# gisbi-kim/navtech-radar-slam

Measured on AMD Instinct MI355X. Metric: sc_loop_queries_per_sec_vs_10k_scan_db, higher is better.
Workload: dtype f16 filter + f64 exact

## Files before the change

navtech-radar-slam_amd/csrc/sc_api.cpp:

```cpp
#include <cmath>
#include <cstdio>
#include <cstdlib>
#include <cstring>
#include <mutex>
#include <new>
#include <string>
#include <vector>

#include "rsx_common.h"
#include "sc_kernels.h"
#include "sc_plan.h"
#include "sc_kdtree.h"
#include "loopverify.h"
#include "radarsc.h"
#include "voxelgrid.h"

namespace rsx {
std::string &last_error() {
  static thread_local std::string e;
  return e;
}
}

using namespace rsx;
using namespace rsx::sc;

struct rsx_sc {
  rsx_sc_params p;
  std::mutex mu;
  Stream stream;
  int64_t n_global = 0, n_local = 0, cap = 0;
  DevBuf desc, vkey, norm, rkey;
  DevBuf hn, cmask;
  DevBuf sp, sp_aux;
  DevBuf hnr, vk16, vk_n;
  int tree_counter = 0;
  int64_t tree_size = 0;
  bool batch_made = false;
  int64_t batch_size = 0;
  struct KdTreeDev {
    DevBuf nodes, vind;
    float low[KD_DIM], high[KD_DIM];
    int64_t n = 0;
    int32_t n_nodes = 0;
    int depth = 0;
  } tree, tree_batch;
  DevBuf pts_ws, q_desc, topk, knn_ws, small, pair_out, q_elig;
  struct QueryWs {
    DevBuf q_vkey, q_norm, q_rkey, partial;
    DevBuf f_qimg, f_lb, f_cand, f_cnt, f_thr, f_plan;
    DevBuf f_wimg, f_win;
  } ws[2];
  QueryWs *w = &ws[0];
  PairProfiler prof;
  const char *prof_kernel = "sc_pair_kernel";
  struct {
    bool valid = false, filtered = false;
    int32_t nq = 0, k = 0;
    int64_t n_items = 0, n_eligible = 0;
    const int64_t *q_elig = nullptr;
    QueryView qv{};
  } st;
  DevBuf st_partial;
  DevBuf q1_ws, q1_ticket;
  DevBuf helper_ws;
  DevBuf stats;
  PinnedBuf pinned;
  static constexpr int kMaxPieces = 8;
  static constexpr int kInsSlots = 8;
  struct InsSlot {
    PinnedBuf host;
    Event done;
    bool used = false;
  } ins[kInsSlots];
  int ins_next = 0;
  hipEvent_t last_insert = nullptr;
  StreamOrder order;
  Event legacy_ev;
  Stream up_stream, stream_b;
  Event up_ev[kMaxPieces], lane_ev;
};

namespace {

constexpr size_t kStatBytes = (size_t)RESCORE_STAT_COPIES * RESCORE_STAT_WORDS * sizeof(unsigned long long);

int set_device(rsx_sc *h) {
  RSX_HIP(hipSetDevice(h->p.device));
  return RSX_OK;
}

int use_stream(rsx_sc *h, void *stream, hipStream_t *s) {
  *s = stream ? static_cast<hipStream_t>(stream) : h->stream;
  if (!stream) {
    if (!h->legacy_ev) RSX_HIP(h->legacy_ev.create());
    RSX_HIP(hipEventRecord(h->legacy_ev, nullptr));
    RSX_HIP(hipStreamWaitEvent(h->stream, h->legacy_ev, 0));
  }
  if (*s != h->stream && h->last_insert) RSX_HIP(hipStreamWaitEvent(*s, h->last_insert, 0));
  return h->order.enter(*s);
}

int own_stream(rsx_sc *h) {
  RSX_TRY(set_device(h));
  return h->order.enter(h->stream);
}

int insert_cloud(rsx_sc *h, const void *d_pts, int64_t n_pts, int64_t stride, int64_t slot, hipStream_t s) {
  return launch_insert(d_pts, nullptr, n_pts, 1, stride, h->p.lidar_height, h->p.max_radius, slot, h->desc.as<float>(),
                       h->vkey.as<double>(), h->norm.as<double>(), h->rkey.as<float>(), h->hn.p, h->hnr.p,
                       h->cmask.as<uint64_t>(), h->sp.p, h->sp_aux.as<float>(), h->vk16.p, h->vk_n.as<float>(), s, h->p.sum_order);
}

int ensure_capacity(rsx_sc *h, int64_t want_local) {
  if (want_local <= h->cap) return RSX_OK;
  int64_t nc = h->cap ? h->cap : 1024;
  while (nc < want_local) nc *= 2;
  RSX_TRY(h->desc.reserve((size_t)nc * DS * sizeof(float), h->stream, true));
  RSX_TRY(h->vkey.reserve((size_t)nc * NS * sizeof(double), h->stream, true));
  RSX_TRY(h->norm.reserve((size_t)nc * NS * sizeof(double), h->stream, true));
  RSX_TRY(h->rkey.reserve((size_t)nc * NR * sizeof(float), h->stream, true));
  RSX_TRY(h->hn.reserve((size_t)nc * FILTER_DB_BYTES_PER_ENTRY, h->stream, true));
  RSX_TRY(h->cmask.reserve((size_t)nc * sizeof(uint64_t), h->stream, true));
  RSX_TRY(h->sp.reserve((size_t)nc * SPEC_DB_BYTES_PER_ENTRY, h->stream, true));
  RSX_TRY(h->sp_aux.reserve((size_t)nc * sizeof(float), h->stream, true));
  RSX_TRY(h->hnr.reserve((size_t)nc * FILTER_DB_BYTES_PER_ENTRY, h->stream, true));
  RSX_TRY(h->vk16.reserve((size_t)nc * 256, h->stream, true));
  RSX_TRY(h->vk_n.reserve((size_t)nc * 2 * sizeof(float), h->stream, true));
  h->cap = nc;
  return RSX_OK;
}

DbView db_view(const rsx_sc *h) {
  DbView v;
  v.desc = h->desc.as<float>();
  v.vkey = h->vkey.as<double>();
  v.norm = h->norm.as<double>();
  v.rkey = h->rkey.as<float>();
  v.hnT = h->hn.p;
  v.cmask = h->cmask.as<uint64_t>();
  v.spT = h->sp.p;
  v.sp_aux = h->sp_aux.as<float>();
  v.hnR = h->hnr.p;
  v.vk16 = h->vk16.p;
  v.vk_n = h->vk_n.as<float>();
  v.n_local = h->n_local;
  v.idx_base = h->p.shard_rank;
  v.idx_stride = h->p.shard_world;
  v.sum_order = h->p.sum_order;
  return v;
}

int build_db_images(rsx_sc *h, int64_t slot, int64_t count, hipStream_t s) {
  RSX_TRY(launch_db_images(h->desc.as<float>(), h->norm.as<double>(), slot, count, h->hn.p, h->hnr.p, h->cmask.as<uint64_t>(), s));
  RSX_TRY(launch_window_db_keys(h->vkey.as<double>(), slot, count, h->vk16.p, h->vk_n.as<float>(), s));
  RSX_TRY(launch_spec_db_images(h->desc.as<float>(), h->norm.as<double>(), slot, count, h->sp.p, h->sp_aux.as<float>(), s));
  RSX_HIP(hipStreamSynchronize(s));
  return RSX_OK;
}

bool owns(const rsx_sc *h, int64_t g) { return (g % h->p.shard_world) == h->p.shard_rank; }

int64_t local_count_below(const rsx_sc *h, int64_t n_eligible) {
  if (n_eligible < 0 || n_eligible > h->n_global) n_eligible = h->n_global;
  const int64_t w = h->p.shard_world, r = h->p.shard_rank;
  if (n_eligible <= r) return 0;
  int64_t c = (n_eligible - r + w - 1) / w;
  return c < h->n_local ? c : h->n_local;
}

float yaw_from_shift(int shift) {
  const double unit = 360.0 / (double)NS;
  const float deg = (float)(shift * unit);
  return (float)((double)deg * M_PI / 180.0);
}

int ensure_pinned(rsx_sc *h, size_t bytes) {
  if (bytes <= h->pinned.bytes) return RSX_OK;
  size_t nb = 4096;
  while (nb < bytes) nb *= 2;
  return h->pinned.reserve(nb);
}

int prepare_queries(rsx_sc *h, const float *d_q, int32_t nq, hipStream_t s, QueryView *qv) {
  h->st.valid = false;
  RSX_TRY(h->w->q_vkey.reserve((size_t)nq * NS * sizeof(double), s, false));
  RSX_TRY(h->w->q_norm.reserve((size_t)nq * NS * sizeof(double), s, false));
  RSX_TRY(h->w->q_rkey.reserve((size_t)nq * NR * sizeof(float), s, false));
  RSX_TRY(launch_keys(d_q, nq, h->w->q_vkey.as<double>(), h->w->q_norm.as<double>(), h->w->q_rkey.as<float>(), s, h->p.sum_order));
  qv->desc = d_q;
  qv->vkey = h->w->q_vkey.as<double>();
  qv->norm = h->w->q_norm.as<double>();
  qv->nq = nq;
  return RSX_OK;
}

int filter_mode_of(const rsx_sc *h) {
  static const int env = [] {
    const char *e = rsx::exp_env("RSX_SC_FILTER");
    if (!e || !*e) return -1;
    return atoi(e) ? 2 : 1;
  }();
  if (h->p.filter_mode) return h->p.filter_mode;
  return env >= 0 ? env : 0;
}

bool use_filter(const rsx_sc *h, int32_t nq, int64_t n_items) {
  const int m = filter_mode_of(h);
  if (m == 1 || n_items <= 0) return false;
  if (m == 2) return true;
  if (n_items >= 50000) return true;
  return (int64_t)nq * n_items >= (1ll << 17);
}

struct ProfScope {
  PairProfiler *pp;
  hipStream_t s;
  bool armed = false;
  ProfScope(PairProfiler *p, hipStream_t st) : pp(p), s(st) {
    if (pp && pp->on && pp->ev && pp->used < PairProfiler::kMax) armed = hipEventRecord(pp->ev[2 * pp->used], s) == hipSuccess;
  }
  void stop() {
    if (armed && hipEventRecord(pp->ev[2 * pp->used + 1], s) == hipSuccess) pp->used++;
    armed = false;
  }
};

constexpr int kDefaultFilterKind = 2;
int filter_kind_of(const rsx_sc *h) {
  static const int env = [] {
    const char *e = rsx::exp_env("RSX_SC_FILTER_KIND");
    if (!e || !*e) return -1;
    if (e[0] == '2' || (e[0] == 's' && std::strstr(e, "2"))) return 2;
    return (e[0] == 's' || e[0] == '1') ? 1 : 0;
  }();
  if (h->p.filter_kind) return h->p.filter_kind - 1;
  return env >= 0 ? env : kDefaultFilterKind;
}

size_t any_qimg_bytes(int32_t nq) {
  const size_t a = filter_qimg_bytes(nq), b = spec_qimg_bytes(nq);
  return a > b ? a : b;
}

int run_filter(rsx_sc *h, const QueryView &q, int64_t n_items, lb_t *lb, int64_t ld, const FilterPlanInput *plan,
               hipStream_t s, int64_t first = 0) {
  DbView db = db_view(h);
  if (first) {
    db.hnT = static_cast<const char *>(db.hnT) + first * FILTER_DB_BYTES_PER_ENTRY;
    db.spT = static_cast<const char *>(db.spT) + first * SPEC_DB_BYTES_PER_ENTRY;
    db.cmask += first;
    db.sp_aux += first;
  }
  if (plan) RSX_TRY(h->w->f_plan.reserve(filter_plan_bytes(n_items), s, false));
  if (filter_kind_of(h) >= 1) {
    const bool two_waves = filter_kind_of(h) == 2;
    h->prof_kernel = two_waves ? spec2_filter_kernel_name() : spec_filter_kernel_name();
    RSX_TRY(launch_spec_query_images(q.desc, q.norm, q.nq, h->w->f_qimg.p, s));
    const int32_t *qmin = nullptr;
    const int64_t *cum = nullptr;
    if (plan) RSX_TRY(launch_filter_plan(db, *plan, q.nq, n_items, 4, h->w->f_plan.p, &qmin, &cum, s));
    ProfScope ps(&h->prof, s);
    RSX_TRY(launch_spec_filter(db, h->w->f_qimg.p, q.nq, n_items, lb, ld, qmin, cum, s, two_waves));
    ps.stop();
    return RSX_OK;
  }
  h->prof_kernel = filter_kernel_name();
  RSX_TRY(launch_query_images(q.desc, q.norm, q.nq, h->w->f_qimg.p, s));
  ProfScope ps(&h->prof, s);
  RSX_TRY(launch_filter(db, h->w->f_qimg.p, q.nq, n_items, lb, ld, plan, plan ? h->w->f_plan.p : nullptr, s));
  ps.stop();
  return RSX_OK;
}

int64_t filter_batch(int64_t n_items, int64_t nq) { return plan::filter_batch(n_items, nq); }

int filter_reserve(rsx_sc *h, int64_t n_items, int64_t qb, hipStream_t s) {
  h->st.valid = false;
  const int64_t ld = (n_items + 31) / 32 * 32;
  RSX_TRY(h->w->f_qimg.reserve(any_qimg_bytes((int32_t)qb), s, false));
  RSX_TRY(h->w->f_lb.reserve((size_t)qb * ld * sizeof(lb_t), s, false));
  RSX_TRY(h->w->f_cand.reserve((size_t)qb * RESCORE_SHORTLIST_CAP * sizeof(RescoreEntry), s, false));
  RSX_TRY(h->w->f_cnt.reserve((size_t)qb * sizeof(int32_t), s, false));
  RSX_TRY(h->w->f_thr.reserve((size_t)qb * RESCORE_THR_STRIDE * sizeof(float), s, false));
  RSX_TRY(h->w->f_wimg.reserve(window_qimg_bytes((int32_t)qb), s, false));
  RSX_TRY(h->w->f_win.reserve((size_t)qb * WINDOW_P * sizeof(WindowPreview), s, false));
  return RSX_OK;
}

int filter_and_select(rsx_sc *h, const QueryView &q, int64_t n_items, int64_t n_eligible, const int64_t *elig,
                      int32_t first_target, int32_t k, hipStream_t s, bool elig_monotone = false) {
  const DbView db = db_view(h);
  const int64_t ld = (n_items + 31) / 32 * 32;
  lb_t *lb = h->w->f_lb.as<lb_t>();
  {
    FilterPlanInput plan{n_eligible, elig};
    const bool planned = elig_monotone && elig != nullptr;
    RSX_TRY(run_filter(h, q, n_items, lb, ld, planned ? &plan : nullptr, s));
  }
  RSX_TRY(launch_select(db, lb, ld, n_items, q.nq, n_eligible, elig, first_target, h->w->f_cand.as<RescoreEntry>(),
                        h->w->f_cnt.as<int32_t>(), h->w->f_thr.as<float>(), s));
  return launch_window(db, q, h->w->f_wimg.p, h->w->f_cand.as<RescoreEntry>(), h->w->f_cnt.as<int32_t>(), k, filter_eps(),
                       h->w->f_win.as<WindowPreview>(), s);
}

int rescore(rsx_sc *h, const QueryView &q, int64_t n_items, int64_t n_eligible, const int64_t *elig, int32_t round_begin,
            int32_t round_end, const rsx_sc_hit *tau_src, const rsx_sc_hit *seed, int32_t k, rsx_sc_hit *d_out,
            hipStream_t s) {
  const int64_t ld = (n_items + 31) / 32 * 32;
  return launch_rescore(db_view(h), q, h->w->f_lb.as<lb_t>(), ld, n_items, n_eligible, elig, h->w->f_cand.as<RescoreEntry>(),
                        h->w->f_cnt.as<int32_t>(), h->w->f_thr.as<float>(), filter_eps(), round_begin, round_end, tau_src,
                        seed, d_out, k, s, (h->prof.on && h->stats.p) ? h->stats.as<unsigned long long>() : nullptr,
                        h->w->f_win.as<WindowPreview>());
}

int32_t first_round_target() {
  static const int32_t v = [] {
    const char *e = rsx::exp_env("RSX_SC_FIRST_TARGET");
    const int x = e ? atoi(e) : 0;
    return (x >= 1 && x <= 128) ? x : 128;
  }();
  return v;
}

int run_topk_filtered(rsx_sc *h, const QueryView &qv, int64_t n_items, int64_t n_eligible, const int64_t *d_q_elig,
                      int32_t k, rsx_sc_hit *d_out, hipStream_t s, bool elig_monotone) {
  const int64_t qb = filter_batch(n_items, qv.nq);
  RSX_TRY(filter_reserve(h, n_items, qb, s));
  for (int64_t b0 = 0; b0 < qv.nq; b0 += qb) {
    const int32_t bn = (int32_t)((qv.nq - b0 < qb) ? (qv.nq - b0) : qb);
    QueryView q = qv;
    q.desc = qv.desc + b0 * DS;
    q.vkey = qv.vkey + b0 * NS;
    q.norm = qv.norm + b0 * NS;
    q.nq = bn;
    const int64_t *elig = d_q_elig ? d_q_elig + b0 : nullptr;
    RSX_TRY(filter_and_select(h, q, n_items, n_eligible, elig, first_round_target(), k, s, elig_monotone));
    RSX_TRY(rescore(h, q, n_items, n_eligible, elig, 0, RESCORE_ALL_ROUNDS, nullptr, nullptr, k, d_out + b0 * k, s));
  }
  return RSX_OK;
}

bool use_q1(const rsx_sc *h, int32_t nq, int64_t n_items) {
  static const bool off = [] {
    const char *e = rsx::exp_env("RSX_SC_Q1");
    return e && e[0] == '0';
  }();
  const int m = filter_mode_of(h);
  if (off || nq < 1 || nq > Q1_MAX_NQ || !(m == 0 || m == 3)) return false;
  return m == 3 || nq == 1 || (int64_t)nq * n_items <= (nq <= 8 ? 800000 : 400000);
}

int run_q1(rsx_sc *h, const float *d_q, int32_t nq, int64_t n_items, int64_t n_eligible, const int64_t *d_q_elig, int32_t k,
           rsx_sc_hit *d_out, hipStream_t s) {
  if (n_items < 0) n_items = 0;
  if (!h->q1_ticket.p) {
    RSX_TRY(h->q1_ticket.reserve(q1_ticket_bytes(), s, false));
    RSX_HIP(hipMemsetAsync(h->q1_ticket.p, 0, q1_ticket_bytes(), s));
  }
  RSX_TRY(h->q1_ws.reserve(q1_workspace_bytes(n_items, nq, k), s, false));
  h->prof_kernel = q1_kernel_name();
  ProfScope ps(&h->prof, s);
  RSX_TRY(launch_q1(db_view(h), d_q, nq, n_items, n_eligible, d_q_elig, k, d_out, h->q1_ws.p, h->q1_ticket.as<unsigned>(),
                    (h->prof.on && h->stats.p) ? h->stats.as<unsigned long long>() : nullptr, s));
  ps.stop();
  return RSX_OK;
}

int run_topk(rsx_sc *h, const QueryView &qv, int64_t n_items, int64_t n_eligible, const int64_t *d_q_elig,
             int32_t k, rsx_sc_hit *d_out, hipStream_t s, bool elig_monotone = false) {
  if (use_q1(h, qv.nq, n_items)) return run_q1(h, qv.desc, qv.nq, n_items, n_eligible, d_q_elig, k, d_out, s);
  if (use_filter(h, qv.nq, n_items)) return run_topk_filtered(h, qv, n_items, n_eligible, d_q_elig, k, d_out, s, elig_monotone);
  h->prof_kernel = pair_kernel_name();
  RSX_TRY(h->w->partial.reserve(pair_partial_bytes(n_items > 0 ? n_items : 1, qv.nq, k), s, false));
  struct Hook {
    explicit Hook(PairProfiler *p) { set_pair_profiler(p); }
    ~Hook() { set_pair_profiler(nullptr); }
  } hook(&h->prof);
  return launch_pairs(db_view(h), qv, nullptr, 0, n_items, n_eligible, d_q_elig, nullptr, nullptr,
                      h->w->partial.as<rsx_sc_hit>(), d_out, k, s);
}

struct PreparedTree {
  int64_t n = 0;
  std::vector<KdNode16> n16;
  std::vector<int32_t> vind;
  float low[KD_DIM], high[KD_DIM];
  int depth = 0;
};

int prepare_tree_host(const float *keys, int64_t n, PreparedTree *out) {
  KdTreeHost host;
  RSX_TRY(kdtree_build_host(keys, n, &host));
  std::vector<KdNode16> &n16 = out->n16;
  n16.resize(host.nodes.size());
  for (size_t i = 0; i < host.nodes.size(); i++) {
    const KdNode &nd = host.nodes[i];
    if (nd.child1 < 0) {
      n16[i] = KdNode16{nd.left, -1 - (nd.right - nd.left), 0.0f, 0.0f};
    } else {
      if (nd.child1 != (int32_t)i + 1) return fail(RSX_ERR_RANGE, "kd-tree nodes are not in preorder");
      n16[i] = KdNode16{nd.child2, nd.divfeat, nd.divlow, nd.divhigh};
    }
  }
  {
    std::vector<int32_t> lo(host.nodes.size());
    for (size_t i = host.nodes.size(); i-- > 0;) {
      const KdNode &nd = host.nodes[i];
      lo[i] = nd.child1 < 0 ? nd.left : lo[(size_t)nd.child1];
      if (nd.child1 >= 0) {
        if (lo[(size_t)nd.child2] >= (1 << 26)) return fail(RSX_ERR_RANGE, "ring-key tree over more than 2^26 keys");
        n16[i].b |= lo[(size_t)nd.child2] << 5;
      }
    }
  }
  out->vind.swap(host.vind);
  std::memcpy(out->low, host.low, sizeof(out->low));
  std::memcpy(out->high, host.high, sizeof(out->high));
  out->depth = host.depth;
  out->n = n;
  return RSX_OK;
}

int upload_tree(rsx_sc *h, rsx_sc::KdTreeDev *t, const PreparedTree &p) {
  hipStream_t s = h->stream;
  t->n = 0;
  t->n_nodes = (int32_t)p.n16.size();
  RSX_TRY(t->nodes.reserve(p.n16.size() * sizeof(KdNode16), s, false));
  RSX_TRY(t->vind.reserve(p.vind.size() * sizeof(int32_t), s, false));
  RSX_HIP(hipMemcpyAsync(t->nodes.p, p.n16.data(), p.n16.size() * sizeof(KdNode16), hipMemcpyHostToDevice, s));
  RSX_HIP(hipMemcpyAsync(t->vind.p, p.vind.data(), p.vind.size() * sizeof(int32_t), hipMemcpyHostToDevice, s));
  RSX_HIP(hipStreamSynchronize(s));
  std::memcpy(t->low, p.low, sizeof(t->low));
  std::memcpy(t->high, p.high, sizeof(t->high));
  t->depth = p.depth;
  t->n = p.n;
  return RSX_OK;
}

int ensure_tree(rsx_sc *h, rsx_sc::KdTreeDev *t, int64_t n, std::unique_lock<std::mutex> &lk) {
  if (t->n == n) return RSX_OK;
  hipStream_t s = h->stream;
  std::vector<float> keys((size_t)n * NR);
  RSX_HIP(hipMemcpyAsync(keys.data(), h->rkey.p, keys.size() * sizeof(float), hipMemcpyDeviceToHost, s));
  RSX_HIP(hipStreamSynchronize(s));
  PreparedTree p;
  lk.unlock();
  const int st = prepare_tree_host(keys.data(), n, &p);
  const std::string err = st == RSX_OK ? std::string() : last_error();
  lk.lock();
  if (st != RSX_OK) {
    last_error() = err;
    return st;
  }
  RSX_TRY(set_device(h));
  if (t->n == n) return RSX_OK;
  if (n > h->n_local) return fail(RSX_ERR_RANGE, "the database shrank while the ring-key tree was being built");
  return upload_tree(h, t, p);
}

int score_candidates_and_finish(rsx_sc *h, const QueryView &qv, const float *d_qkey, int64_t n_search, rsx_sc::KdTreeDev *tree,
                                int mode, int32_t *loop_id, float *yaw, double *min_dist, int32_t *nn_idx) {
  hipStream_t s = h->stream;
  const int k = h->p.num_candidates;
  double best_d = 10000000;
  int best_align = 0, best_idx = 0;
  if (mode == RSX_SC_MODE_CANDIDATE) {
    RSX_TRY(h->small.reserve(4096, s, false));
    int32_t *d_idx = h->small.as<int32_t>();
    float *d_kd = reinterpret_cast<float *>(d_idx + 64);
    int32_t *d_found = d_idx + 128;
    if (n_search > 0) {
      if (tree->n != n_search) return fail(RSX_ERR_INTERNAL, "ring-key tree over %lld keys was not prepared", (long long)n_search);
      int32_t *b_idx = d_idx + 192;
      float *b_kd = reinterpret_cast<float *>(d_idx + 256);
      int32_t *b_found = d_idx + 320;
      RSX_TRY(h->knn_ws.reserve((size_t)n_search * 2 * sizeof(float), s, false));
      float *dist_all = h->knn_ws.as<float>(), *dist_tree = dist_all + n_search;
      RSX_TRY(launch_knn(h->rkey.as<float>(), n_search, d_qkey, k, dist_all, b_idx, b_kd, b_found, s));
      int32_t *cand_pos = d_idx + 384, *cand_count = d_idx + 384 + 64;
      RSX_TRY(launch_knn_tree_order(dist_all, tree->vind.as<int32_t>(), n_search, dist_tree, k, b_kd, b_found, cand_pos, cand_count, s));
      KdSearchArgs ka;
      ka.bound_dist = b_kd;
      ka.bound_found = b_found;
      ka.dist_tree = dist_tree;
      ka.cand_pos = cand_pos;
      ka.cand_count = cand_count;
      ka.nodes = tree->nodes.as<KdNode16>();
      ka.n_nodes = tree->n_nodes;
      ka.n = n_search;
      ka.vind = tree->vind.as<int32_t>();
      ka.keys = h->rkey.as<float>();
      ka.qkey = d_qkey;
      std::memcpy(ka.low, tree->low, sizeof(ka.low));
      std::memcpy(ka.high, tree->high, sizeof(ka.high));
      ka.k = k;
      ka.out_idx = d_idx;
      ka.out_dist = d_kd;
      ka.out_found = d_found;
      RSX_TRY(launch_knn_tree(ka, s));
    } else {
      RSX_TRY(h->knn_ws.reserve(sizeof(float), s, false));
      RSX_TRY(launch_knn(h->rkey.as<float>(), 0, d_qkey, k, h->knn_ws.as<float>(), d_idx, d_kd, d_found, s));
    }
    double *d_dist = reinterpret_cast<double *>(h->small.as<char>() + 1024);
    int32_t *d_shift = reinterpret_cast<int32_t *>(h->small.as<char>() + 2048);
    RSX_TRY(launch_pairs(db_view(h), qv, d_idx, 0, k, -1, nullptr, d_dist, d_shift, nullptr, nullptr, 0, s));
    RSX_TRY(ensure_pinned(h, 4096));
    char *hp = static_cast<char *>(h->pinned.p);
    RSX_HIP(hipMemcpyAsync(hp, h->small.p, 2048 + 256, hipMemcpyDeviceToHost, s));
    RSX_HIP(hipStreamSynchronize(s));
    const int32_t *ci = reinterpret_cast<const int32_t *>(hp);
    const double *cd = reinterpret_cast<const double *>(hp + 1024);
    const int32_t *cs = reinterpret_cast<const int32_t *>(hp + 2048);
    for (int c = 0; c < k; c++) {
      if (cd[c] < best_d) {
        best_d = cd[c];
        best_align = cs[c];
        best_idx = ci[c];
      }
    }
  } else {
    RSX_TRY(ensure_pinned(h, 4096));
    RSX_TRY(run_topk(h, qv, n_search, n_search, nullptr, 1, static_cast<rsx_sc_hit *>(h->pinned.p), s));
    RSX_HIP(hipStreamSynchronize(s));
    const rsx_sc_hit *r = static_cast<const rsx_sc_hit *>(h->pinned.p);
    if (r->dist < best_d) {
      best_d = r->dist;
      best_align = r->shift;
      best_idx = r->index;
    }
  }
  int lid = -1;
  if (best_d < h->p.dist_thres) lid = best_idx;
  if (loop_id) *loop_id = lid;
  if (yaw) *yaw = yaw_from_shift(best_align);
  if (min_dist) *min_dist = best_d;
  if (nn_idx) *nn_idx = best_idx;
  return RSX_OK;
}

}

extern "C" {

const char *rsx_last_error_string(void) { return rsx::last_error().c_str(); }

const char *rsx_version(void) {
#ifdef RSX_EXPERIMENTS
  return "rsx 0.3 (gfx950, HIP; ScanContext + ORORA hot path) +experiments";
#else
  return "rsx 0.3 (gfx950, HIP; ScanContext + ORORA hot path)";
#endif
}

int rsx_device_count(void) try {
  int n = 0;
  if (hipGetDeviceCount(&n) != hipSuccess) return 0;
  return n;
} RSX_CATCH_ALL

const char *rsx_sc_dominant_kernel_name(void) { return pair_kernel_name(); }

const char *rsx_sc_profiled_kernel_name(rsx_sc *h) {
  if (!h) return "";
  std::lock_guard<std::mutex> lk(h->mu);
  return h->prof_kernel;
}

int rsx_sc_default_params(rsx_sc_params *p) try {
  if (!p) return fail(RSX_ERR_BAD_ARG, "null params");
  p->lidar_height = 2.0;
  p->max_radius = 80.0;
  p->num_exclude_recent = 30;
  p->num_candidates = 3;
  p->search_ratio = 0.1;
  p->dist_thres = 0.2;
  p->tree_making_period = 30;
  p->device = 0;
  p->shard_rank = 0;
  p->shard_world = 1;
  p->capacity_hint = 1024;
  p->filter_mode = 0;
  p->filter_kind = 0;
  p->sum_order = RSX_SC_SUM_EIGEN_SSE2;
  return RSX_OK;
} RSX_CATCH_ALL

int rsx_sc_create(const rsx_sc_params *p, rsx_sc **out) try {
  if (!out) return fail(RSX_ERR_BAD_ARG, "null out");
  *out = nullptr;
  rsx_sc_params d;
  rsx_sc_default_params(&d);
  if (p) d = *p;
  if (d.shard_world < 1 || d.shard_rank < 0 || d.shard_rank >= d.shard_world)
    return fail(RSX_ERR_BAD_ARG, "bad shard %d/%d", d.shard_rank, d.shard_world);
  if (d.num_candidates < 1 || d.num_candidates > RSX_SC_MAX_TOPK)
    return fail(RSX_ERR_BAD_ARG, "num_candidates must be in [1,%d]", RSX_SC_MAX_TOPK);
  if ((int)std::lround(0.5 * d.search_ratio * NS) != 3)
    return fail(RSX_ERR_BAD_ARG, "kernels are specialised for SEARCH_RADIUS 3 (search_ratio 0.1, SC.h:96)");
  if (d.tree_making_period < 1 || d.num_exclude_recent < 0) return fail(RSX_ERR_BAD_ARG, "bad detector params");
  if (d.filter_mode < 0 || d.filter_mode > 3) return fail(RSX_ERR_BAD_ARG, "filter_mode must be 0 (auto), 1 (off), 2 (force) or 3 (single-query path)");
  if (d.sum_order < 0 || d.sum_order > RSX_SC_SUM_EIGEN34_AVX_FMA) return fail(RSX_ERR_BAD_ARG, "sum_order must be RSX_SC_SUM_EIGEN_SSE2, _SEQ, _EIGEN_AVX_FMA or _EIGEN34_AVX_FMA");
  if (d.filter_kind < 0 || d.filter_kind > 3)
    return fail(RSX_ERR_BAD_ARG, "filter_kind must be 0 (auto), 1 (direct), 2 (spectral) or 3 (spectral, two waves per SIMD)");
  RSX_TRY(check_device(d.device));
  std::unique_ptr<rsx_sc> h(new (std::nothrow) rsx_sc());
  if (!h) return fail(RSX_ERR_OOM, "host alloc");
  h->p = d;
  RSX_TRY(set_device(h.get()));
  hipError_t e = h->stream.create();
  if (e != hipSuccess) return fail(RSX_ERR_HIP, "hipStreamCreate: %s", hipGetErrorString(e));
  RSX_TRY(ensure_capacity(h.get(), d.capacity_hint > 0 ? d.capacity_hint : 1024));
  *out = h.release();
  return RSX_OK;
} RSX_CATCH_ALL

int rsx_sc_destroy(rsx_sc *h) try {
  if (!h) return RSX_OK;
  (void)hipSetDevice(h->p.device);
  for (hipStream_t s : {h->stream.s, h->up_stream.s, h->stream_b.s})
    if (s) (void)hipStreamSynchronize(s);
  delete h;
  return RSX_OK;
} RSX_CATCH_ALL

int rsx_sc_set_dist_thres(rsx_sc *h, double thres) try {
  if (!h) return fail(RSX_ERR_BAD_ARG, "null handle");
  std::lock_guard<std::mutex> lk(h->mu);
  h->p.dist_thres = thres;
  return RSX_OK;
} RSX_CATCH_ALL

int rsx_sc_size(rsx_sc *h, int64_t *n) try {
  if (!h || !n) return fail(RSX_ERR_BAD_ARG, "null arg");
  std::lock_guard<std::mutex> lk(h->mu);
  *n = h->n_global;
  return RSX_OK;
} RSX_CATCH_ALL

int rsx_sc_local_size(rsx_sc *h, int64_t *n) try {
  if (!h || !n) return fail(RSX_ERR_BAD_ARG, "null arg");
  std::lock_guard<std::mutex> lk(h->mu);
  *n = h->n_local;
  return RSX_OK;
} RSX_CATCH_ALL

int rsx_sc_ringkey_tree_layout(const float *keys20, int64_t n, int32_t *out_vind, int32_t *out_n_nodes, int32_t *out_depth) try {
  if (!keys20 || !out_vind || n < 1) return fail(RSX_ERR_BAD_ARG, "bad arg");
  KdTreeHost host;
  RSX_TRY(kdtree_build_host(keys20, n, &host));
  std::memcpy(out_vind, host.vind.data(), host.vind.size() * sizeof(int32_t));
  if (out_n_nodes) *out_n_nodes = (int32_t)host.nodes.size();
  if (out_depth) *out_depth = host.depth;
  return RSX_OK;
} RSX_CATCH_ALL

int rsx_sc_tree_size(rsx_sc *h, int64_t *n) try {
  if (!h || !n) return fail(RSX_ERR_BAD_ARG, "null arg");
  std::lock_guard<std::mutex> lk(h->mu);
  *n = h->tree_size;
  return RSX_OK;
} RSX_CATCH_ALL

int rsx_sc_add_points(rsx_sc *h, const void *pts, size_t n, size_t stride_bytes, int32_t *out_index) try {
  if (!h || (!pts && n)) return fail(RSX_ERR_BAD_ARG, "null arg");
  if (stride_bytes < 12 || (stride_bytes & 3)) return fail(RSX_ERR_BAD_ARG, "stride_bytes must be >= 12 and a multiple of 4");
  std::lock_guard<std::mutex> lk(h->mu);
  RSX_TRY(own_stream(h));
  const int64_t g = h->n_global;
  if (owns(h, g)) {
    const int64_t slot = h->n_local;
    RSX_TRY(ensure_capacity(h, slot + 1));
    const size_t bytes = n * stride_bytes;
    rsx_sc::InsSlot &sl = h->ins[h->ins_next];
    h->ins_next = (h->ins_next + 1) % rsx_sc::kInsSlots;
    if (sl.used) RSX_HIP(hipEventSynchronize(sl.done));
    if (bytes > sl.host.bytes) {
      size_t cap = 32768;
      while (cap < bytes) cap *= 2;
      RSX_TRY(sl.host.reserve(cap));
    }
    if (!sl.done) RSX_HIP(sl.done.create());
    if (bytes) std::memcpy(sl.host.p, pts, bytes);
    RSX_TRY(insert_cloud(h, sl.host.p, (int64_t)n, (int64_t)stride_bytes, slot, h->stream));
    RSX_HIP(hipEventRecord(sl.done, h->stream));
    sl.used = true;
    h->last_insert = sl.done;
    h->n_local = slot + 1;
  }
  h->n_global = g + 1;
  if (out_index) *out_index = (int32_t)g;
  return RSX_OK;
} RSX_CATCH_ALL

int rsx_sc_add_points_downsampled(rsx_sc *h, rsx_voxelgrid *vg, const void *pts, size_t n, size_t stride_bytes, float leaf,
                                  int32_t *out_index) try {
  if (!h || !vg || (!pts && n)) return fail(RSX_ERR_BAD_ARG, "null arg");
  if (stride_bytes < 12 || (stride_bytes & 3)) return fail(RSX_ERR_BAD_ARG, "stride_bytes must be >= 12 and a multiple of 4");
  if (!(leaf > 0.0f)) return fail(RSX_ERR_BAD_ARG, "leaf must be positive");
  if (rsx::vg::device_of(vg) != h->p.device) return fail(RSX_ERR_BAD_ARG, "voxel grid and ScanContext handles are on different devices");
  std::lock_guard<std::mutex> lk(h->mu);
  std::lock_guard<std::mutex> lkv(rsx::vg::mutex_of(vg));
  RSX_TRY(own_stream(h));
  const int64_t g = h->n_global;
  if (owns(h, g)) {
    const float *d_ds = nullptr;
    int64_t nds = 0;
    RSX_TRY(rsx::vg::upload_and_filter(vg, pts, (int64_t)n, (int64_t)stride_bytes, -1, leaf, (int64_t)(n ? n : 1), &d_ds, &nds));
    const int64_t slot = h->n_local;
    RSX_TRY(ensure_capacity(h, slot + 1));
    RSX_TRY(insert_cloud(h, d_ds ? static_cast<const void *>(d_ds) : h->desc.p, nds, 16, slot, h->stream));
    RSX_HIP(hipStreamSynchronize(h->stream));
    h->n_local = slot + 1;
  }
  h->n_global = g + 1;
  if (out_index) *out_index = (int32_t)g;
  return RSX_OK;
} RSX_CATCH_ALL

int rsx_sc_add_keyframe(rsx_sc *h, rsx_voxelgrid *vg, rsx_kfstore *kf, const void *pts, size_t n, size_t stride_bytes,
                        int32_t intensity_offset, float leaf, int32_t *out_index) try {
  if (!h || !vg || !kf || (!pts && n)) return fail(RSX_ERR_BAD_ARG, "null arg");
  if (stride_bytes < 12 || (stride_bytes & 3)) return fail(RSX_ERR_BAD_ARG, "stride_bytes must be >= 12 and a multiple of 4");
  if (intensity_offset >= 0 && ((intensity_offset & 3) || (size_t)intensity_offset + 4 > stride_bytes))
    return fail(RSX_ERR_BAD_ARG, "intensity_offset outside the point");
  if (!(leaf > 0.0f)) return fail(RSX_ERR_BAD_ARG, "leaf must be positive");
  if (rsx::vg::device_of(vg) != h->p.device || rsx::kf::device_of(kf) != h->p.device)
    return fail(RSX_ERR_BAD_ARG, "voxel grid, keyframe store and ScanContext handles are on different devices");
  std::lock_guard<std::mutex> lk(h->mu);
  std::lock_guard<std::mutex> lkv(rsx::vg::mutex_of(vg));
  std::lock_guard<std::mutex> lkk(rsx::kf::mutex_of(kf));
  RSX_TRY(own_stream(h));
  const int64_t g = h->n_global;
  const float *d_ds = nullptr;
  int64_t nds = 0;
  RSX_TRY(rsx::vg::upload_and_filter(vg, pts, (int64_t)n, (int64_t)stride_bytes, intensity_offset, leaf, (int64_t)(n ? n : 1), &d_ds, &nds));
  const bool mine = owns(h, g);
  if (mine) {
    const int64_t slot = h->n_local;
    RSX_TRY(ensure_capacity(h, slot + 1));
    RSX_TRY(insert_cloud(h, d_ds ? static_cast<const void *>(d_ds) : h->desc.p, nds, 16, slot, h->stream));
    RSX_HIP(hipStreamSynchronize(h->stream));
  }
  int32_t kf_index = -1;
  RSX_TRY(rsx::kf::append_device_locked(kf, d_ds, nds, &kf_index));
  if (mine) h->n_local = h->n_local + 1;
  h->n_global = g + 1;
  if (out_index) *out_index = (int32_t)g;
  return RSX_OK;
} RSX_CATCH_ALL

static int add_f32_locked(rsx_sc *h, const float *src, int64_t n, bool src_is_device, hipStream_t s) {
  const int64_t g0 = h->n_global;
  const int64_t w = h->p.shard_world, r = h->p.shard_rank;
  int64_t first = g0 + (((r - g0) % w) + w) % w;
  int64_t count = first < g0 + n ? (g0 + n - first + w - 1) / w : 0;
  if (count > 0) {
    const int64_t slot = h->n_local;
    RSX_TRY(ensure_capacity(h, slot + count));
    float *dst = h->desc.as<float>() + slot * DS;
    RSX_HIP(hipMemcpy2DAsync(dst, DS * sizeof(float), src + (first - g0) * DS, (size_t)w * DS * sizeof(float),
                             DS * sizeof(float), (size_t)count,
                             src_is_device ? hipMemcpyDeviceToDevice : hipMemcpyHostToDevice, s));
    RSX_TRY(launch_keys(dst, count, h->vkey.as<double>() + slot * NS, h->norm.as<double>() + slot * NS,
                        h->rkey.as<float>() + slot * NR, s, h->p.sum_order));
    RSX_TRY(build_db_images(h, slot, count, s));
    h->n_local = slot + count;
  }
  h->n_global = g0 + n;
  return RSX_OK;
}

static int add_descriptor_f64(rsx_sc *h, const double *desc, bool allow_rounding, int32_t *out_index, double *max_err) {
  if (!h || !desc) return fail(RSX_ERR_BAD_ARG, "null arg");
  float f[DS];
  double worst = 0.0;
  for (int i = 0; i < DS; i++) {
    f[i] = (float)desc[i];
    if (!((double)f[i] == desc[i])) {
      if (!allow_rounding || !(desc[i] == desc[i]))
        return fail(RSX_ERR_NOT_FP32_EXACT, "descriptor element %d (%.17g) is not exactly representable in fp32", i, desc[i]);
      const double e = std::fabs((double)f[i] - desc[i]);
      if (e > worst) worst = e;
    }
  }
  if (max_err) *max_err = worst;
  std::lock_guard<std::mutex> lk(h->mu);
  RSX_TRY(own_stream(h));
  const int64_t g = h->n_global;
  RSX_TRY(add_f32_locked(h, f, 1, false, h->stream));
  if (out_index) *out_index = (int32_t)g;
  return RSX_OK;
}

int rsx_sc_add_descriptor(rsx_sc *h, const double *desc, int32_t *out_index) try {
  return add_descriptor_f64(h, desc, false, out_index, nullptr);
} RSX_CATCH_ALL

int rsx_sc_add_descriptor_rounded(rsx_sc *h, const double *desc, int32_t *out_index, double *max_abs_rounding) try {
  return add_descriptor_f64(h, desc, true, out_index, max_abs_rounding);
} RSX_CATCH_ALL

int rsx_sc_add_descriptors_f32(rsx_sc *h, const float *descs, int64_t n) try {
  if (!h || (!descs && n) || n < 0) return fail(RSX_ERR_BAD_ARG, "bad arg");
  if (n == 0) return RSX_OK;
  std::lock_guard<std::mutex> lk(h->mu);
  RSX_TRY(own_stream(h));
  return add_f32_locked(h, descs, n, false, h->stream);
} RSX_CATCH_ALL

int rsx_sc_add_descriptors_f32_device(rsx_sc *h, const float *d_descs, int64_t n, void *stream) try {
  if (!h || (!d_descs && n) || n < 0) return fail(RSX_ERR_BAD_ARG, "bad arg");
  if (n == 0) return RSX_OK;
  std::lock_guard<std::mutex> lk(h->mu);
  RSX_TRY(set_device(h));
  hipStream_t s;
  RSX_TRY(use_stream(h, stream, &s));
  return add_f32_locked(h, d_descs, n, true, s);
} RSX_CATCH_ALL

int rsx_sc_add_polar_batch_device(rsx_sc *h, rsx_radarsc *rc, const uint8_t *d_imgs, int32_t n_images, int64_t image_stride_bytes,
                                  int32_t row_stride, int32_t col_offset, const float *d_azimuths, int32_t azimuths_per_image, void *stream) try {
  if (!h || !rc || n_images < 0 || (n_images && (!d_imgs || !d_azimuths))) return fail(RSX_ERR_BAD_ARG, "bad arg");
  if (rsx::rc::device_of(rc) != h->p.device) return fail(RSX_ERR_BAD_ARG, "radar scan-context and ScanContext handles are on different devices");
  if (n_images == 0) return RSX_OK;
  std::lock_guard<std::mutex> lk(h->mu);
  std::lock_guard<std::mutex> lkr(rsx::rc::mutex_of(rc));
  RSX_TRY(set_device(h));
  hipStream_t s;
  RSX_TRY(use_stream(h, stream, &s));
  const float *d_descs = nullptr;
  RSX_TRY(rsx::rc::build_scratch_device(rc, d_imgs, n_images, image_stride_bytes, row_stride, col_offset, d_azimuths, azimuths_per_image, s, &d_descs));
  return add_f32_locked(h, d_descs, n_images, true, s);
} RSX_CATCH_ALL

int rsx_sc_add_polar(rsx_sc *h, rsx_radarsc *rc, const uint8_t *img, int32_t row_stride, int32_t col_offset, const float *azimuths,
                     int32_t *out_index) try {
  if (!h || !rc || !img || !azimuths) return fail(RSX_ERR_BAD_ARG, "null arg");
  if (rsx::rc::device_of(rc) != h->p.device) return fail(RSX_ERR_BAD_ARG, "radar scan-context and ScanContext handles are on different devices");
  std::lock_guard<std::mutex> lk(h->mu);
  std::lock_guard<std::mutex> lkr(rsx::rc::mutex_of(rc));
  RSX_TRY(own_stream(h));
  const int64_t g = h->n_global;
  if (owns(h, g)) {
    const float *d_desc = nullptr;
    RSX_TRY(rsx::rc::upload_and_build(rc, img, row_stride, col_offset, azimuths, h->stream, &d_desc));
    RSX_TRY(add_f32_locked(h, d_desc, 1, true, h->stream));
  } else {
    h->n_global = g + 1;
  }
  if (out_index) *out_index = (int32_t)g;
  return RSX_OK;
} RSX_CATCH_ALL

int rsx_sc_export_descriptors_f32(rsx_sc *h, int64_t first_slot, int64_t count, float *out) try {
  if (!h || (!out && count)) return fail(RSX_ERR_BAD_ARG, "null arg");
  std::lock_guard<std::mutex> lk(h->mu);
  if (first_slot < 0 || count < 0 || first_slot + count > h->n_local) return fail(RSX_ERR_RANGE, "slot range out of bounds");
  if (count == 0) return RSX_OK;
  RSX_TRY(own_stream(h));
  RSX_HIP(hipMemcpyAsync(out, h->desc.as<float>() + first_slot * DS, (size_t)count * DS * sizeof(float), hipMemcpyDeviceToHost,
                         h->stream));
  RSX_HIP(hipStreamSynchronize(h->stream));
  return RSX_OK;
} RSX_CATCH_ALL

namespace {
struct DbFileHeader {
  char magic[8];
  uint32_t version;
  uint32_t num_ring;
  uint32_t num_sector;
  uint32_t dtype;
  int64_t n_global;
  int64_t n_local;
  int32_t shard_rank, shard_world;
  uint8_t reserved[16];
};
static_assert(sizeof(DbFileHeader) == 64, "header layout");
}

int rsx_sc_save(rsx_sc *h, const char *path) try {
  if (!h || !path) return fail(RSX_ERR_BAD_ARG, "null arg");
  std::lock_guard<std::mutex> lk(h->mu);
  RSX_TRY(own_stream(h));
  std::vector<float> buf((size_t)h->n_local * DS);
  if (h->n_local) {
    RSX_HIP(hipMemcpyAsync(buf.data(), h->desc.p, buf.size() * sizeof(float), hipMemcpyDeviceToHost, h->stream));
    RSX_HIP(hipStreamSynchronize(h->stream));
  }
  DbFileHeader hd{};
  std::memcpy(hd.magic, "RSXSCDB1", 8);
  hd.version = 1;
  hd.num_ring = NR;
  hd.num_sector = NS;
  hd.dtype = 0;
  hd.n_global = h->n_global;
  hd.n_local = h->n_local;
  hd.shard_rank = h->p.shard_rank;
  hd.shard_world = h->p.shard_world;
  FILE *f = std::fopen(path, "wb");
  if (!f) return fail(RSX_ERR_BAD_ARG, "cannot open %s for writing", path);
  bool ok = std::fwrite(&hd, sizeof(hd), 1, f) == 1;
  ok = ok && (buf.empty() || std::fwrite(buf.data(), sizeof(float), buf.size(), f) == buf.size());
  ok = (std::fclose(f) == 0) && ok;
  if (!ok) return fail(RSX_ERR_INTERNAL, "short write to %s", path);
  return RSX_OK;
} RSX_CATCH_ALL

int rsx_sc_load(rsx_sc *h, const char *path, int64_t *n_loaded) try {
  if (!h || !path) return fail(RSX_ERR_BAD_ARG, "null arg");
  FILE *f = std::fopen(path, "rb");
  if (!f) return fail(RSX_ERR_BAD_ARG, "cannot open %s", path);
  DbFileHeader hd{};
  std::vector<float> buf;
  bool ok = std::fread(&hd, sizeof(hd), 1, f) == 1 && std::memcmp(hd.magic, "RSXSCDB1", 8) == 0 && hd.version == 1 &&
            hd.num_ring == (uint32_t)NR && hd.num_sector == (uint32_t)NS && hd.dtype == 0 && hd.n_local >= 0 && hd.n_global >= 0 &&
            hd.n_local <= hd.n_global && hd.shard_world >= 1 && hd.shard_rank >= 0 && hd.shard_rank < hd.shard_world;
  if (ok) {
    const int64_t expect = hd.n_global > hd.shard_rank ? (hd.n_global - hd.shard_rank + hd.shard_world - 1) / hd.shard_world : 0;
    ok = hd.n_local == expect;
  }
  if (ok) {
    const long here = std::ftell(f);
    ok = here == (long)sizeof(hd) && std::fseek(f, 0, SEEK_END) == 0;
    const long end = ok ? std::ftell(f) : -1;
    ok = ok && end >= 0 && (uint64_t)end == (uint64_t)sizeof(hd) + (uint64_t)hd.n_local * DS * sizeof(float) &&
         std::fseek(f, here, SEEK_SET) == 0;
  }
  if (ok) {
    try {
      buf.resize((size_t)hd.n_local * DS);
    } catch (const std::bad_alloc &) {
      std::fclose(f);
      return fail(RSX_ERR_OOM, "%s: %lld descriptors do not fit in host memory", path, (long long)hd.n_local);
    }
    ok = buf.empty() || std::fread(buf.data(), sizeof(float), buf.size(), f) == buf.size();
  }
  std::fclose(f);
  if (!ok) return fail(RSX_ERR_BAD_ARG, "%s is not a complete, consistent RSXSCDB1 file for 20 x 60 fp32 descriptors", path);
  std::lock_guard<std::mutex> lk(h->mu);
  if (hd.shard_world != 1) {
    if (hd.shard_world != h->p.shard_world || hd.shard_rank != h->p.shard_rank || h->n_global != 0)
      return fail(RSX_ERR_BAD_ARG, "%s holds shard %d/%d: load it into an empty handle of the same shard", path, hd.shard_rank,
                  hd.shard_world);
    RSX_TRY(own_stream(h));
    if (hd.n_local) {
      RSX_TRY(ensure_capacity(h, hd.n_local));
      RSX_HIP(hipMemcpyAsync(h->desc.p, buf.data(), buf.size() * sizeof(float), hipMemcpyHostToDevice, h->stream));
      RSX_TRY(launch_keys(h->desc.as<float>(), hd.n_local, h->vkey.as<double>(), h->norm.as<double>(), h->rkey.as<float>(), h->stream, h->p.sum_order));
      RSX_TRY(build_db_images(h, 0, hd.n_local, h->stream));
    }
    h->n_local = hd.n_local;
    h->n_global = hd.n_global;
  } else {
    RSX_TRY(own_stream(h));
    if (hd.n_local) RSX_TRY(add_f32_locked(h, buf.data(), hd.n_local, false, h->stream));
  }
  if (n_loaded) *n_loaded = hd.n_local;
  return RSX_OK;
} RSX_CATCH_ALL

static int local_slot_of(rsx_sc *h, int64_t index, int64_t *slot) {
  if (index < 0 || index >= h->n_global) return fail(RSX_ERR_RANGE, "index %lld out of range [0,%lld)", (long long)index, (long long)h->n_global);
  if (!owns(h, index)) return fail(RSX_ERR_RANGE, "index %lld is not stored on shard %d/%d", (long long)index, h->p.shard_rank, h->p.shard_world);
  *slot = index / h->p.shard_world;
  if (*slot >= h->n_local) return fail(RSX_ERR_INTERNAL, "index %lld maps to slot %lld but the shard holds %lld", (long long)index, (long long)*slot, (long long)h->n_local);
  return RSX_OK;
}

int rsx_sc_get_descriptor(rsx_sc *h, int64_t index, double *out) try {
  if (!h || !out) return fail(RSX_ERR_BAD_ARG, "null arg");
  std::lock_guard<std::mutex> lk(h->mu);
  RSX_TRY(own_stream(h));
  int64_t slot;
  RSX_TRY(local_slot_of(h, index, &slot));
  float f[DS];
  RSX_HIP(hipMemcpyAsync(f, h->desc.as<float>() + slot * DS, sizeof(f), hipMemcpyDeviceToHost, h->stream));
  RSX_HIP(hipStreamSynchronize(h->stream));
  for (int i = 0; i < DS; i++) out[i] = (double)f[i];
  return RSX_OK;
} RSX_CATCH_ALL

int rsx_sc_get_ringkey(rsx_sc *h, int64_t index, float *out20) try {
  if (!h || !out20) return fail(RSX_ERR_BAD_ARG, "null arg");
  std::lock_guard<std::mutex> lk(h->mu);
  RSX_TRY(own_stream(h));
  int64_t slot;
  RSX_TRY(local_slot_of(h, index, &slot));
  RSX_HIP(hipMemcpyAsync(out20, h->rkey.as<float>() + slot * NR, NR * sizeof(float), hipMemcpyDeviceToHost, h->stream));
  RSX_HIP(hipStreamSynchronize(h->stream));
  return RSX_OK;
} RSX_CATCH_ALL

int rsx_sc_get_sectorkey(rsx_sc *h, int64_t index, double *out60) try {
  if (!h || !out60) return fail(RSX_ERR_BAD_ARG, "null arg");
  std::lock_guard<std::mutex> lk(h->mu);
  RSX_TRY(own_stream(h));
  int64_t slot;
  RSX_TRY(local_slot_of(h, index, &slot));
  RSX_HIP(hipMemcpyAsync(out60, h->vkey.as<double>() + slot * NS, NS * sizeof(double), hipMemcpyDeviceToHost, h->stream));
  RSX_HIP(hipStreamSynchronize(h->stream));
  return RSX_OK;
} RSX_CATCH_ALL

int rsx_sc_detect_loop_closure_ex(rsx_sc *h, int mode, rsx_sc_detection *out) try {
  if (!h || !out) return fail(RSX_ERR_BAD_ARG, "null arg");
  if (mode != RSX_SC_MODE_CANDIDATE && mode != RSX_SC_MODE_EXHAUSTIVE) return fail(RSX_ERR_BAD_ARG, "bad mode %d", mode);
  std::unique_lock<std::mutex> lk(h->mu);
  if (h->p.shard_world != 1) return fail(RSX_ERR_BAD_ARG, "detect_loop_closure needs an unsharded handle; use rsx_scs_* or rsx_sc_query_device + merge");
  RSX_TRY(own_stream(h));
  const int64_t N = h->n_global;
  out->loop_id = -1;
  out->yaw_diff_rad = 0.0f;
  out->min_dist = 10000000;
  out->nn_idx = 0;
  out->query_idx = (int32_t)(N - 1);
  out->searched = 0;
  out->reserved = 0;
  out->dist_thres = h->p.dist_thres;
  if (N == 0 || N < h->p.num_exclude_recent + 1) return RSX_OK;
  int64_t n_search = h->tree_size;
  if (h->tree_counter % h->p.tree_making_period == 0)
    n_search = N - h->p.num_exclude_recent;
  if (mode == RSX_SC_MODE_CANDIDATE && n_search >= 1) RSX_TRY(ensure_tree(h, &h->tree, n_search, lk));
  if (N > h->n_global || n_search > h->n_global)
    return fail(RSX_ERR_RANGE, "the database was replaced while the ring-key tree was being built");
  h->tree_size = n_search;
  h->tree_counter = h->tree_counter + 1;
  QueryView qv;
  qv.desc = h->desc.as<float>() + (N - 1) * DS;
  qv.vkey = h->vkey.as<double>() + (N - 1) * NS;
  qv.norm = h->norm.as<double>() + (N - 1) * NS;
  qv.nq = 1;
  out->searched = 1;
  return score_candidates_and_finish(h, qv, h->rkey.as<float>() + (N - 1) * NR , n_search, &h->tree, mode,
                                     &out->loop_id, &out->yaw_diff_rad, &out->min_dist, &out->nn_idx);
} RSX_CATCH_ALL

int rsx_sc_detect_loop_closure(rsx_sc *h, int mode, int32_t *loop_id, float *yaw, double *min_dist, int32_t *nn_idx) try {
  rsx_sc_detection d;
  RSX_TRY(rsx_sc_detect_loop_closure_ex(h, mode, &d));
  if (loop_id) *loop_id = d.loop_id;
  if (yaw) *yaw = d.yaw_diff_rad;
  if (min_dist) *min_dist = d.min_dist;
  if (nn_idx) *nn_idx = d.nn_idx;
  return RSX_OK;
} RSX_CATCH_ALL

static int helper_call(rsx_sc *h, int op, const double *a, size_t na, const double *b, size_t nb, double *out_d, size_t nd,
                       int32_t *out_i) {
  std::lock_guard<std::mutex> lk(h->mu);
  RSX_TRY(own_stream(h));
  hipStream_t s = h->stream;
  RSX_TRY(h->helper_ws.reserve((2 * DS + 128) * sizeof(double), s, false));
  double *d_a = h->helper_ws.as<double>(), *d_b = d_a + DS, *d_o = d_b + DS;
  int32_t *d_i = reinterpret_cast<int32_t *>(d_o + 96);
  RSX_HIP(hipMemcpyAsync(d_a, a, na * sizeof(double), hipMemcpyHostToDevice, s));
  if (b) RSX_HIP(hipMemcpyAsync(d_b, b, nb * sizeof(double), hipMemcpyHostToDevice, s));
  RSX_TRY(launch_helper(op, d_a, b ? d_b : nullptr, d_o, d_i, s, h->p.sum_order));
  if (out_d) RSX_HIP(hipMemcpyAsync(out_d, d_o, nd * sizeof(double), hipMemcpyDeviceToHost, s));
  if (out_i) RSX_HIP(hipMemcpyAsync(out_i, d_i, sizeof(int32_t), hipMemcpyDeviceToHost, s));
  RSX_HIP(hipStreamSynchronize(s));
  return RSX_OK;
}

int rsx_sc_make_keys(rsx_sc *h, const double *desc, double *out_ringkey20, double *out_sectorkey60) try {
  if (!h || !desc) return fail(RSX_ERR_BAD_ARG, "null arg");
  double o[NR + NS];
  RSX_TRY(helper_call(h, 0, desc, DS, nullptr, 0, o, NR + NS, nullptr));
  if (out_ringkey20) std::memcpy(out_ringkey20, o, NR * sizeof(double));
  if (out_sectorkey60) std::memcpy(out_sectorkey60, o + NR, NS * sizeof(double));
  return RSX_OK;
} RSX_CATCH_ALL

int rsx_sc_dist_direct(rsx_sc *h, const double *sc1, const double *sc2, double *out_dist) try {
  if (!h || !sc1 || !sc2 || !out_dist) return fail(RSX_ERR_BAD_ARG, "null arg");
  return helper_call(h, 1, sc1, DS, sc2, DS, out_dist, 1, nullptr);
} RSX_CATCH_ALL

int rsx_sc_fast_align(rsx_sc *h, const double *vkey1, const double *vkey2, int32_t *out_shift) try {
  if (!h || !vkey1 || !vkey2 || !out_shift) return fail(RSX_ERR_BAD_ARG, "null arg");
  return helper_call(h, 2, vkey1, NS, vkey2, NS, nullptr, 0, out_shift);
} RSX_CATCH_ALL

int rsx_sc_distance(rsx_sc *h, const double *sc1, const double *sc2, double *out_dist, int32_t *out_shift) try {
  if (!h || !sc1 || !sc2 || !out_dist || !out_shift) return fail(RSX_ERR_BAD_ARG, "null arg");
  return helper_call(h, 3, sc1, DS, sc2, DS, out_dist, 1, out_shift);
} RSX_CATCH_ALL

int rsx_sc_make_scancontext(rsx_sc *h, const void *pts, size_t n, size_t stride_bytes, double *out_desc) try {
  if (!h || (!pts && n) || !out_desc) return fail(RSX_ERR_BAD_ARG, "null arg");
  if (stride_bytes < 12 || (stride_bytes & 3)) return fail(RSX_ERR_BAD_ARG, "stride_bytes must be >= 12 and a multiple of 4");
  std::lock_guard<std::mutex> lk(h->mu);
  RSX_TRY(own_stream(h));
  hipStream_t s = h->stream;
  const size_t bytes = n * stride_bytes;
  RSX_TRY(h->pts_ws.reserve(bytes ? bytes : 16, s, false));
  if (bytes) RSX_HIP(hipMemcpyAsync(h->pts_ws.p, pts, bytes, hipMemcpyHostToDevice, s));
  RSX_TRY(h->helper_ws.reserve((2 * DS + 128) * sizeof(double), s, false));
  float *d_desc = h->helper_ws.as<float>();
  double *d_vk = reinterpret_cast<double *>(d_desc + DS);
  RSX_TRY(launch_build(h->pts_ws.p, (int64_t)n, (int64_t)stride_bytes, h->p.lidar_height, h->p.max_radius, d_desc, d_vk,
                       d_vk + NS, reinterpret_cast<float *>(d_vk + 2 * NS), s, h->p.sum_order));
  float f[DS];
  RSX_HIP(hipMemcpyAsync(f, d_desc, sizeof(f), hipMemcpyDeviceToHost, s));
  RSX_HIP(hipStreamSynchronize(s));
  for (int i = 0; i < DS; i++) out_desc[i] = (double)f[i];
  return RSX_OK;
} RSX_CATCH_ALL

int rsx_sc_detect_between_session(rsx_sc *h, const float *curr_key20, const double *curr_desc, int32_t *loop_id,
                                  float *yaw, double *min_dist, int32_t *nn_idx) try {
  if (!h || !curr_key20 || !curr_desc) return fail(RSX_ERR_BAD_ARG, "null arg");
  float f[DS];
  for (int i = 0; i < DS; i++) {
    f[i] = (float)curr_desc[i];
    if (!((double)f[i] == curr_desc[i])) return fail(RSX_ERR_NOT_FP32_EXACT, "query descriptor element %d is not fp32-exact", i);
  }
  std::unique_lock<std::mutex> lk(h->mu);
  if (h->p.shard_world != 1) return fail(RSX_ERR_BAD_ARG, "unsharded handles only");
  if (h->n_global == 0) return fail(RSX_ERR_RANGE, "empty database");
  RSX_TRY(own_stream(h));
  const int64_t batch = h->batch_made ? h->batch_size : h->n_global;
  RSX_TRY(ensure_tree(h, &h->tree_batch, batch, lk));
  if (batch > h->n_global) return fail(RSX_ERR_RANGE, "the database was replaced while the ring-key tree was being built");
  if (!h->batch_made) {
    h->batch_size = batch;
    h->batch_made = true;
  }
  hipStream_t s = h->stream;
  RSX_TRY(h->q_desc.reserve(sizeof(f) + 128, s, false));
  RSX_HIP(hipMemcpyAsync(h->q_desc.p, f, sizeof(f), hipMemcpyHostToDevice, s));
  float *d_key = reinterpret_cast<float *>(static_cast<char *>(h->q_desc.p) + sizeof(f));
  RSX_HIP(hipMemcpyAsync(d_key, curr_key20, NR * sizeof(float), hipMemcpyHostToDevice, s));
  QueryView qv;
  RSX_TRY(prepare_queries(h, h->q_desc.as<float>(), 1, s, &qv));
  return score_candidates_and_finish(h, qv, d_key, h->batch_size, &h->tree_batch, RSX_SC_MODE_CANDIDATE, loop_id, yaw, min_dist, nn_idx);
} RSX_CATCH_ALL

static int query_device_locked(rsx_sc *h, const float *d_q, int32_t nq, int32_t k, int64_t n_eligible, rsx_sc_hit *d_out,
                               hipStream_t s) {
  const int64_t items = local_count_below(h, n_eligible);
  if (use_q1(h, nq, items))
    return run_q1(h, d_q, nq, items, n_eligible < 0 ? h->n_global : n_eligible, nullptr, k, d_out, s);
  QueryView qv;
  RSX_TRY(prepare_queries(h, d_q, nq, s, &qv));
  return run_topk(h, qv, items, n_eligible < 0 ? h->n_global : n_eligible, nullptr, k, d_out, s);
}

int rsx_sc_query_device(rsx_sc *h, const float *d_q, int32_t nq, int32_t k, int64_t n_eligible, rsx_sc_hit *d_out, void *stream) try {
  if (!h || !d_q || !d_out || nq < 1) return fail(RSX_ERR_BAD_ARG, "bad arg");
  if (k < 1 || k > RSX_SC_MAX_TOPK) return fail(RSX_ERR_BAD_ARG, "k must be in [1,%d]", RSX_SC_MAX_TOPK);
  std::lock_guard<std::mutex> lk(h->mu);
  RSX_TRY(set_device(h));
  hipStream_t s;
  RSX_TRY(use_stream(h, stream, &s));
  return query_device_locked(h, d_q, nq, k, n_eligible, d_out, s);
} RSX_CATCH_ALL

int host_pieces(int32_t nq, int32_t *sizes) {
  static const std::pair<int, int> cfg = [] {
    const char *e = rsx::exp_env("RSX_SC_HOST_PIECES");
    std::pair<int, int> r{512, 25};
    if (e && *e) {
      r.first = atoi(e);
      const char *c = strchr(e, ':');
      if (c) r.second = atoi(c + 1);
    }
    return r;
  }();
  return plan::host_pieces(nq, cfg.first, cfg.second, rsx_sc::kMaxPieces, sizes);
}

int rsx_sc_query(rsx_sc *h, const float *q, int32_t nq, int32_t k, int64_t n_eligible, rsx_sc_hit *out) try {
  if (!h || !q || !out || nq < 1) return fail(RSX_ERR_BAD_ARG, "bad arg");
  if (k < 1 || k > RSX_SC_MAX_TOPK) return fail(RSX_ERR_BAD_ARG, "k must be in [1,%d]", RSX_SC_MAX_TOPK);
  std::lock_guard<std::mutex> lk(h->mu);
  RSX_TRY(own_stream(h));
  RSX_TRY(h->q_desc.reserve((size_t)nq * DS * sizeof(float), h->stream, false));
  RSX_TRY(h->topk.reserve((size_t)nq * k * sizeof(rsx_sc_hit), h->stream, false));
  int32_t sizes[rsx_sc::kMaxPieces];
  const int np = host_pieces(nq, sizes);
  static const bool two_lanes = [] {
    const char *e = rsx::exp_env("RSX_SC_HOST_LANES");
    return !(e && e[0] == '1');
  }();
  const size_t out_bytes = (size_t)nq * k * sizeof(rsx_sc_hit);
  if (np == 1 && out_bytes <= 4096) {
    const size_t q_bytes = (size_t)nq * DS * sizeof(float);
    const bool small_q = q_bytes <= 8 * DS * sizeof(float);
    RSX_TRY(ensure_pinned(h, 4096 + (small_q ? q_bytes : 0)));
    const void *src = q;
    if (small_q) {
      std::memcpy(static_cast<char *>(h->pinned.p) + 4096, q, q_bytes);
      src = static_cast<char *>(h->pinned.p) + 4096;
    }
    RSX_HIP(hipMemcpyAsync(h->q_desc.p, src, q_bytes, hipMemcpyHostToDevice, h->stream));
    RSX_TRY(query_device_locked(h, h->q_desc.as<float>(), nq, k, n_eligible, static_cast<rsx_sc_hit *>(h->pinned.p), h->stream));
    RSX_HIP(hipStreamSynchronize(h->stream));
    std::memcpy(out, h->pinned.p, out_bytes);
    return RSX_OK;
  }
  if (np == 1) {
    RSX_HIP(hipMemcpyAsync(h->q_desc.p, q, (size_t)nq * DS * sizeof(float), hipMemcpyHostToDevice, h->stream));
    RSX_TRY(query_device_locked(h, h->q_desc.as<float>(), nq, k, n_eligible, h->topk.as<rsx_sc_hit>(), h->stream));
  } else {
    if (!h->up_stream) {
      RSX_HIP(h->up_stream.create());
      RSX_HIP(h->stream_b.create());
      for (Event &e : h->up_ev) RSX_HIP(e.create());
      RSX_HIP(h->lane_ev.create());
    }
    auto upload = [&](int c, int64_t q0) -> int {
      RSX_HIP(hipMemcpyAsync(h->q_desc.as<float>() + q0 * DS, q + q0 * DS, (size_t)sizes[c] * DS * sizeof(float),
                             hipMemcpyHostToDevice, h->up_stream));
      RSX_HIP(hipEventRecord(h->up_ev[c], h->up_stream));
      return RSX_OK;
    };
    const int64_t items = local_count_below(h, n_eligible), elig_all = n_eligible < 0 ? h->n_global : n_eligible;
    const bool one_tail = !use_q1(h, nq, items) && use_filter(h, nq, items) && filter_batch(items, nq) >= nq;
    auto filter_pieces_one_tail = [&]() -> int {
      hipStream_t s = h->stream;
      h->w = &h->ws[0];
      RSX_TRY(filter_reserve(h, items, nq, s));
      QueryView all;
      {
        h->st.valid = false;
        RSX_TRY(h->w->q_vkey.reserve((size_t)nq * NS * sizeof(double), s, false));
        RSX_TRY(h->w->q_norm.reserve((size_t)nq * NS * sizeof(double), s, false));
        RSX_TRY(h->w->q_rkey.reserve((size_t)nq * NR * sizeof(float), s, false));
        all.desc = h->q_desc.as<float>();
        all.vkey = h->w->q_vkey.as<double>();
        all.norm = h->w->q_norm.as<double>();
        all.nq = nq;
      }
      const int64_t ld = (items + 31) / 32 * 32;
      lb_t *lb = h->w->f_lb.as<lb_t>();
      RSX_TRY(upload(0, 0));
      int64_t q0 = 0;
      for (int c = 0; c < np; c++) {
        RSX_HIP(hipStreamWaitEvent(s, h->up_ev[c], 0));
        RSX_TRY(launch_keys(all.desc + q0 * DS, sizes[c], h->w->q_vkey.as<double>() + q0 * NS, h->w->q_norm.as<double>() + q0 * NS,
                            h->w->q_rkey.as<float>() + q0 * NR, s, h->p.sum_order));
        QueryView piece = all;
        piece.desc = all.desc + q0 * DS;
        piece.vkey = all.vkey + q0 * NS;
        piece.norm = all.norm + q0 * NS;
        piece.nq = sizes[c];
        RSX_TRY(run_filter(h, piece, items, lb + q0 * ld, ld, nullptr, s));
        q0 += sizes[c];
        if (c + 1 < np) RSX_TRY(upload(c + 1, q0));
      }
      const DbView db = db_view(h);
      RSX_TRY(launch_select(db, lb, ld, items, nq, elig_all, nullptr, first_round_target(), h->w->f_cand.as<RescoreEntry>(),
                            h->w->f_cnt.as<int32_t>(), h->w->f_thr.as<float>(), s));
      RSX_TRY(launch_window(db, all, h->w->f_wimg.p, h->w->f_cand.as<RescoreEntry>(), h->w->f_cnt.as<int32_t>(), k, filter_eps(),
                            h->w->f_win.as<WindowPreview>(), s));
      return rescore(h, all, items, elig_all, nullptr, 0, RESCORE_ALL_ROUNDS, nullptr, nullptr, k, h->topk.as<rsx_sc_hit>(), s);
    };
    auto all_pieces = [&]() -> int {
      if (one_tail) return filter_pieces_one_tail();
      RSX_HIP(hipEventRecord(h->lane_ev, h->stream));
      RSX_HIP(hipStreamWaitEvent(h->stream_b, h->lane_ev, 0));
      RSX_TRY(upload(0, 0));
      int64_t q0 = 0;
      for (int c = 0; c < np; c++) {
        hipStream_t lane = two_lanes && (c & 1) ? h->stream_b : h->stream;
        h->w = &h->ws[two_lanes ? (c & 1) : 0];
        RSX_HIP(hipStreamWaitEvent(lane, h->up_ev[c], 0));
        RSX_TRY(query_device_locked(h, h->q_desc.as<float>() + q0 * DS, sizes[c], k, n_eligible,
                                    h->topk.as<rsx_sc_hit>() + q0 * k, lane));
        q0 += sizes[c];
        if (c + 1 < np) RSX_TRY(upload(c + 1, q0));
      }
      RSX_HIP(hipEventRecord(h->lane_ev, h->stream_b));
      RSX_HIP(hipStreamWaitEvent(h->stream, h->lane_ev, 0));
      return RSX_OK;
    };
    struct BackToSetZero {
      rsx_sc *h;
      ~BackToSetZero() { h->w = &h->ws[0]; }
    } back{h};
    const int st = all_pieces();
    h->w = &h->ws[0];
    if (st != RSX_OK) {
      (void)hipStreamSynchronize(h->up_stream);
      (void)hipStreamSynchronize(h->stream_b);
      (void)hipStreamSynchronize(h->stream);
      return st;
    }
  }
  RSX_HIP(hipMemcpyAsync(out, h->topk.p, (size_t)nq * k * sizeof(rsx_sc_hit), hipMemcpyDeviceToHost, h->stream));
  RSX_HIP(hipStreamSynchronize(h->stream));
  return RSX_OK;
} RSX_CATCH_ALL

int rsx_sc_filter_range_device(rsx_sc *h, const float *d_q, int32_t nq, int64_t first_slot, int64_t n_slots, rsx_f16 *d_lb,
                               int64_t ld, void *stream) try {
  if (!h || !d_q || !d_lb || nq < 1) return fail(RSX_ERR_BAD_ARG, "bad arg");
  if (first_slot < 0 || first_slot % 32 || n_slots < 0) return fail(RSX_ERR_BAD_ARG, "the range must start at a multiple of 32 slots");
  if (ld < (n_slots + 31) / 32 * 32 || ld % 8) return fail(RSX_ERR_BAD_ARG, "ld must cover the range rounded up to 32 slots");
  if ((reinterpret_cast<uintptr_t>(d_lb) & 15u) != 0) return fail(RSX_ERR_BAD_ARG, "d_lb must be 16-byte aligned");
  if (n_slots == 0) return RSX_OK;
  std::lock_guard<std::mutex> lk(h->mu);
  RSX_TRY(set_device(h));
  if (first_slot + n_slots > h->n_local) return fail(RSX_ERR_RANGE, "slots [%lld, %lld) of %lld", (long long)first_slot,
                                                     (long long)(first_slot + n_slots), (long long)h->n_local);
  hipStream_t s;
  RSX_TRY(use_stream(h, stream, &s));
  QueryView qv;
  RSX_TRY(prepare_queries(h, d_q, nq, s, &qv));
  RSX_TRY(h->w->f_qimg.reserve(any_qimg_bytes(nq), s, false));
  return run_filter(h, qv, n_slots, reinterpret_cast<lb_t *>(d_lb), ld, nullptr, s, first_slot);
} RSX_CATCH_ALL

int rsx_sc_query_bounds_device(rsx_sc *h, const float *d_q, int32_t nq, int32_t k, int64_t n_eligible, const rsx_f16 *d_lb_blocks,
                               int32_t n_blocks, int64_t block_ld, int64_t block_stride, rsx_sc_hit *d_out, void *stream) try {
  if (!h || !d_q || !d_lb_blocks || !d_out || nq < 1 || n_blocks < 1) return fail(RSX_ERR_BAD_ARG, "bad arg");
  if (k < 1 || k > RSX_SC_MAX_TOPK) return fail(RSX_ERR_BAD_ARG, "k must be in [1,%d]", RSX_SC_MAX_TOPK);
  if ((reinterpret_cast<uintptr_t>(d_lb_blocks) & 15u) != 0)
    return fail(RSX_ERR_BAD_ARG, "d_lb_blocks must be 16-byte aligned");
  std::lock_guard<std::mutex> lk(h->mu);
  RSX_TRY(set_device(h));
  if (h->p.shard_world != 1) return fail(RSX_ERR_BAD_ARG, "bounds from filter shards need the whole database in this handle (shard_world 1)");
  hipStream_t s;
  RSX_TRY(use_stream(h, stream, &s));
  QueryView qv;
  RSX_TRY(prepare_queries(h, d_q, nq, s, &qv));
  const int64_t n_elig = n_eligible < 0 ? h->n_global : n_eligible;
  const int64_t n_items = local_count_below(h, n_eligible);
  if (n_items <= 0) return launch_pairs(db_view(h), qv, nullptr, 0, 0, n_elig, nullptr, nullptr, nullptr, nullptr, d_out, k, s);
  const int64_t ld = (n_items + 31) / 32 * 32;
  if (block_ld < 32 || block_ld % 32 || (int64_t)n_blocks * block_ld < ld || block_stride < (int64_t)nq * block_ld || block_stride % 8)
    return fail(RSX_ERR_BAD_ARG, "%d blocks of %lld columns do not cover %lld eligible entries", n_blocks, (long long)block_ld,
                (long long)n_items);
  const int64_t qb = filter_batch(n_items, nq);
  RSX_TRY(filter_reserve(h, n_items, qb, s));
  const DbView db = db_view(h);
  for (int64_t b0 = 0; b0 < nq; b0 += qb) {
    QueryView q = qv;
    q.desc = qv.desc + b0 * DS;
    q.vkey = qv.vkey + b0 * NS;
    q.norm = qv.norm + b0 * NS;
    q.nq = (int32_t)((nq - b0 < qb) ? (nq - b0) : qb);
    RSX_TRY(launch_gather_bounds(reinterpret_cast<const lb_t *>(d_lb_blocks), block_ld, block_stride, b0, q.nq, h->w->f_lb.as<lb_t>(), ld, s));
    RSX_TRY(launch_select(db, h->w->f_lb.as<lb_t>(), ld, n_items, q.nq, n_elig, nullptr, first_round_target(), h->w->f_cand.as<RescoreEntry>(),
                          h->w->f_cnt.as<int32_t>(), h->w->f_thr.as<float>(), s));
    RSX_TRY(launch_window(db, q, h->w->f_wimg.p, h->w->f_cand.as<RescoreEntry>(), h->w->f_cnt.as<int32_t>(), k, filter_eps(),
                          h->w->f_win.as<WindowPreview>(), s));
    RSX_TRY(rescore(h, q, n_items, n_elig, nullptr, 0, RESCORE_ALL_ROUNDS, nullptr, nullptr, k, d_out + b0 * k, s));
  }
  return RSX_OK;
} RSX_CATCH_ALL

int rsx_sc_query_stage1_device(rsx_sc *h, const float *d_q, int32_t nq, int32_t k, int64_t n_eligible,
                               rsx_sc_hit *d_partial, void *stream) try {
  return rsx_sc_query_stage1_elig_device(h, d_q, nq, k, n_eligible, nullptr, 0, d_partial, stream);
} RSX_CATCH_ALL

int rsx_sc_query_stage1_elig_device(rsx_sc *h, const float *d_q, int32_t nq, int32_t k, int64_t n_eligible,
                                    const int64_t *d_q_elig, int32_t elig_monotone, rsx_sc_hit *d_partial, void *stream) try {
  if (!h || !d_q || !d_partial || nq < 1) return fail(RSX_ERR_BAD_ARG, "bad arg");
  if (k < 1 || k > RSX_SC_MAX_TOPK) return fail(RSX_ERR_BAD_ARG, "k must be in [1,%d]", RSX_SC_MAX_TOPK);
  std::lock_guard<std::mutex> lk(h->mu);
  RSX_TRY(set_device(h));
  hipStream_t s;
  RSX_TRY(use_stream(h, stream, &s));
  h->st.valid = false;
  QueryView qv;
  RSX_TRY(prepare_queries(h, d_q, nq, s, &qv));
  const int64_t items = local_count_below(h, n_eligible);
  const int64_t n_elig = n_eligible < 0 ? h->n_global : n_eligible;
  RSX_TRY(h->st_partial.reserve((size_t)nq * k * sizeof(rsx_sc_hit), s, false));
  const bool filtered = use_filter(h, nq, items) && filter_batch(items, nq) >= nq;
  if (filtered) {
    static const int stage1_total = [] {
      const char *e = rsx::exp_env("RSX_SC_STAGE1_TOTAL");
      const int v = (e && *e) ? atoi(e) : 0;
      return v > 0 ? v : 160;
    }();
    int32_t first = (stage1_total + h->p.shard_world - 1) / h->p.shard_world;
    if (first < 8) first = 8;
    if (first > 128) first = 128;
    RSX_TRY(filter_reserve(h, items, nq, s));
    RSX_TRY(filter_and_select(h, qv, items, n_elig, d_q_elig, first, k, s, elig_monotone != 0));
    RSX_TRY(rescore(h, qv, items, n_elig, d_q_elig, 0, 1, nullptr, nullptr, k, h->st_partial.as<rsx_sc_hit>(), s));
  } else {
    RSX_TRY(run_topk(h, qv, items, n_elig, d_q_elig, k, h->st_partial.as<rsx_sc_hit>(), s, elig_monotone != 0));
  }
  RSX_HIP(hipMemcpyAsync(d_partial, h->st_partial.p, (size_t)nq * k * sizeof(rsx_sc_hit), hipMemcpyDeviceToDevice, s));
  h->st.valid = true;
  h->st.filtered = filtered;
  h->st.nq = nq;
  h->st.k = k;
  h->st.n_items = items;
  h->st.n_eligible = n_elig;
  h->st.q_elig = d_q_elig;
  h->st.qv = qv;
  return RSX_OK;
} RSX_CATCH_ALL

int rsx_sc_query_stage2_device(rsx_sc *h, int32_t nq, int32_t k, const rsx_sc_hit *d_global, rsx_sc_hit *d_out,
                               void *stream) try {
  if (!h || !d_global || !d_out) return fail(RSX_ERR_BAD_ARG, "null arg");
  std::lock_guard<std::mutex> lk(h->mu);
  if (!h->st.valid || h->st.nq != nq || h->st.k != k)
    return fail(RSX_ERR_BAD_ARG, "stage 2 without a matching stage 1 (nq=%d k=%d)", nq, k);
  RSX_TRY(set_device(h));
  hipStream_t s;
  RSX_TRY(use_stream(h, stream, &s));
  h->st.valid = false;
  if (h->st.filtered)
    return rescore(h, h->st.qv, h->st.n_items, h->st.n_eligible, h->st.q_elig, 1, RESCORE_ALL_ROUNDS, d_global,
                   h->st_partial.as<rsx_sc_hit>(), k, d_out, s);
  RSX_HIP(hipMemcpyAsync(d_out, h->st_partial.p, (size_t)nq * k * sizeof(rsx_sc_hit), hipMemcpyDeviceToDevice, s));
  return RSX_OK;
} RSX_CATCH_ALL

int rsx_sc_query_self_device(rsx_sc *h, int64_t q_first, int32_t nq, int32_t k, int64_t n_eligible, int32_t exclude_recent,
                             rsx_sc_hit *d_out, void *stream) try {
  if (!h || !d_out || nq < 1) return fail(RSX_ERR_BAD_ARG, "bad arg");
  if (k < 1 || k > RSX_SC_MAX_TOPK) return fail(RSX_ERR_BAD_ARG, "k must be in [1,%d]", RSX_SC_MAX_TOPK);
  std::lock_guard<std::mutex> lk(h->mu);
  if (h->p.shard_world != 1) return fail(RSX_ERR_BAD_ARG, "query_self needs an unsharded handle (queries must be local)");
  if (q_first < 0 || q_first + nq > h->n_global) return fail(RSX_ERR_RANGE, "query range out of bounds");
  RSX_TRY(set_device(h));
  hipStream_t s;
  RSX_TRY(use_stream(h, stream, &s));
  QueryView qv;
  qv.desc = h->desc.as<float>() + q_first * DS;
  qv.vkey = h->vkey.as<double>() + q_first * NS;
  qv.norm = h->norm.as<double>() + q_first * NS;
  qv.nq = nq;
  if (n_eligible < 0 || n_eligible > h->n_global) n_eligible = h->n_global;
  const int64_t *d_elig = nullptr;
  if (exclude_recent >= 0) {
    std::vector<int64_t> e((size_t)nq);
    for (int i = 0; i < nq; i++) {
      int64_t v = q_first + i - exclude_recent;
      e[(size_t)i] = v < 0 ? 0 : v;
    }
    RSX_TRY(h->q_elig.reserve((size_t)nq * sizeof(int64_t), s, false));
    RSX_HIP(hipMemcpyAsync(h->q_elig.p, e.data(), (size_t)nq * sizeof(int64_t), hipMemcpyHostToDevice, s));
    RSX_HIP(hipStreamSynchronize(s));
    d_elig = h->q_elig.as<int64_t>();
  }
  return run_topk(h, qv, local_count_below(h, n_eligible), n_eligible, d_elig, k, d_out, s, true);
} RSX_CATCH_ALL

int rsx_sc_pair_distances(rsx_sc *h, const float *q_desc, int64_t first, int64_t count, double *out_dist, int32_t *out_shift) try {
  if (!h || !q_desc || !out_dist || !out_shift) return fail(RSX_ERR_BAD_ARG, "null arg");
  std::lock_guard<std::mutex> lk(h->mu);
  if (first < 0 || count < 0 || first + count > h->n_local) return fail(RSX_ERR_RANGE, "range out of bounds");
  if (count == 0) return RSX_OK;
  RSX_TRY(own_stream(h));
  hipStream_t s = h->stream;
  RSX_TRY(h->q_desc.reserve(DS * sizeof(float), s, false));
  RSX_HIP(hipMemcpyAsync(h->q_desc.p, q_desc, DS * sizeof(float), hipMemcpyHostToDevice, s));
  QueryView qv;
  RSX_TRY(prepare_queries(h, h->q_desc.as<float>(), 1, s, &qv));
  RSX_TRY(h->pair_out.reserve((size_t)count * (sizeof(double) + sizeof(int32_t)), s, false));
  double *d_dist = h->pair_out.as<double>();
  int32_t *d_shift = reinterpret_cast<int32_t *>(d_dist + count);
  RSX_TRY(launch_pairs(db_view(h), qv, nullptr, first, count, -1, nullptr, d_dist, d_shift, nullptr, nullptr, 0, s));
  RSX_HIP(hipMemcpyAsync(out_dist, d_dist, (size_t)count * sizeof(double), hipMemcpyDeviceToHost, s));
  RSX_HIP(hipMemcpyAsync(out_shift, d_shift, (size_t)count * sizeof(int32_t), hipMemcpyDeviceToHost, s));
  RSX_HIP(hipStreamSynchronize(s));
  return RSX_OK;
} RSX_CATCH_ALL

int rsx_sc_filter_bounds(rsx_sc *h, const float *q_descs, int32_t nq, float *out_lb) try {
  if (!h || !q_descs || !out_lb || nq < 1) return fail(RSX_ERR_BAD_ARG, "bad arg");
  std::lock_guard<std::mutex> lk(h->mu);
  RSX_TRY(own_stream(h));
  hipStream_t s = h->stream;
  const int64_t n = h->n_local;
  if (n == 0) return RSX_OK;
  const int64_t ld = (n + 31) / 32 * 32;
  RSX_TRY(h->q_desc.reserve((size_t)nq * DS * sizeof(float), s, false));
  RSX_HIP(hipMemcpyAsync(h->q_desc.p, q_descs, (size_t)nq * DS * sizeof(float), hipMemcpyHostToDevice, s));
  QueryView qv;
  RSX_TRY(prepare_queries(h, h->q_desc.as<float>(), nq, s, &qv));
  RSX_TRY(h->w->f_qimg.reserve(any_qimg_bytes(nq), s, false));
  RSX_TRY(h->w->f_lb.reserve((size_t)nq * ld * sizeof(lb_t), s, false));
  RSX_TRY(run_filter(h, qv, n, h->w->f_lb.as<lb_t>(), ld, nullptr, s));
  std::vector<lb_t> host((size_t)nq * (size_t)n);
  RSX_HIP(hipMemcpy2DAsync(host.data(), (size_t)n * sizeof(lb_t), h->w->f_lb.p, (size_t)ld * sizeof(lb_t), (size_t)n * sizeof(lb_t),
                           (size_t)nq, hipMemcpyDeviceToHost, s));
  RSX_HIP(hipStreamSynchronize(s));
  for (size_t i = 0; i < host.size(); i++) out_lb[i] = (float)host[i];
  return RSX_OK;
} RSX_CATCH_ALL

double rsx_sc_filter_eps(void) { return filter_eps(); }

int rsx_sc_window_previews(rsx_sc *h, const float *q_descs, int32_t nq, int32_t k, int32_t *out_slots, float *out_pv,
                           int32_t *out_kstar, int32_t *out_shift_mask, int32_t *out_counts) try {
  if (!h || !q_descs || !out_slots || !out_pv || !out_kstar || !out_shift_mask || !out_counts || nq < 1)
    return fail(RSX_ERR_BAD_ARG, "bad arg");
  if (k < 1 || k > RSX_SC_MAX_TOPK) return fail(RSX_ERR_BAD_ARG, "k=%d out of range [1,%d]", k, RSX_SC_MAX_TOPK);
  std::lock_guard<std::mutex> lk(h->mu);
  RSX_TRY(own_stream(h));
  hipStream_t s = h->stream;
  const int64_t n = h->n_local;
  for (int32_t q = 0; q < nq; q++) out_counts[q] = 0;
  if (n == 0) return RSX_OK;
  RSX_TRY(h->q_desc.reserve((size_t)nq * DS * sizeof(float), s, false));
  RSX_HIP(hipMemcpyAsync(h->q_desc.p, q_descs, (size_t)nq * DS * sizeof(float), hipMemcpyHostToDevice, s));
  QueryView qv;
  RSX_TRY(prepare_queries(h, h->q_desc.as<float>(), nq, s, &qv));
  RSX_TRY(filter_reserve(h, n, nq, s));
  RSX_HIP(hipMemsetAsync(h->w->f_win.p, 0xff, (size_t)nq * WINDOW_P * sizeof(WindowPreview), s));
  RSX_TRY(filter_and_select(h, qv, n, h->n_global, nullptr, 128, k, s));
  std::vector<RescoreEntry> sl((size_t)nq * RESCORE_SHORTLIST_CAP);
  std::vector<WindowPreview> wp((size_t)nq * WINDOW_P);
  std::vector<int32_t> cnt((size_t)nq);
  RSX_HIP(hipMemcpyAsync(sl.data(), h->w->f_cand.p, sl.size() * sizeof(RescoreEntry), hipMemcpyDeviceToHost, s));
  RSX_HIP(hipMemcpyAsync(wp.data(), h->w->f_win.p, wp.size() * sizeof(WindowPreview), hipMemcpyDeviceToHost, s));
  RSX_HIP(hipMemcpyAsync(cnt.data(), h->w->f_cnt.p, cnt.size() * sizeof(int32_t), hipMemcpyDeviceToHost, s));
  RSX_HIP(hipStreamSynchronize(s));
  for (int32_t q = 0; q < nq; q++) {
    const int32_t c = cnt[(size_t)q] < WINDOW_P ? cnt[(size_t)q] : WINDOW_P;
    out_counts[q] = c;
    for (int32_t i = 0; i < WINDOW_P; i++) {
      const size_t o = (size_t)q * WINDOW_P + i;
      out_slots[o] = i < c ? sl[(size_t)q * RESCORE_SHORTLIST_CAP + i].slot : -1;
      out_pv[o] = wp[o].pv;
      out_kstar[o] = wp[o].ks >= 0 ? (wp[o].ks & 63) : wp[o].ks;
      out_shift_mask[o] = wp[o].ks >= 0 ? ((wp[o].ks >> 8) & 0x7f) : 0;
    }
  }
  return RSX_OK;
} RSX_CATCH_ALL

int rsx_selftest_firewall(int kind) try {
  if (kind == 0) {
    std::vector<double> v;
    v.reserve(v.max_size() + 1);
  } else if (kind == 1) {
    throw std::bad_alloc();
  } else if (kind == 2) {
    throw std::runtime_error("KDTreeSingleIndexAdaptor: selftest");
  } else if (kind == 3) {
    throw 42;
  }
  return RSX_OK;
} RSX_CATCH_ALL

int rsx_sc_merge_topk(const rsx_sc_hit *parts, int32_t nparts, int32_t nq, int32_t k, rsx_sc_hit *out) try {
  if (!parts || !out || nparts < 1 || nq < 1 || k < 1) return fail(RSX_ERR_BAD_ARG, "bad arg");
  for (int q = 0; q < nq; q++) {
    rsx_sc_hit *o = out + (size_t)q * k;
    int count = 0;
    for (int p = 0; p < nparts; p++)
      for (int i = 0; i < k; i++) {
        const rsx_sc_hit &r = parts[((size_t)p * nq + q) * k + i];
        if (!(r.dist < 10000000)) continue;
        int pos = count < k ? count : k;
        while (pos > 0 && ((r.dist < o[pos - 1].dist) || (r.dist == o[pos - 1].dist && r.index < o[pos - 1].index))) pos--;
        if (pos >= k) continue;
        int last = count < k ? count : k - 1;
        for (int j = last; j > pos; j--) o[j] = o[j - 1];
        o[pos] = r;
        if (count < k) count++;
      }
    for (int i = count; i < k; i++) {
      o[i].dist = 10000000;
      o[i].index = 0;
      o[i].shift = 0;
    }
  }
  return RSX_OK;
} RSX_CATCH_ALL

int rsx_sc_merge_topk_device(rsx_sc *h, const rsx_sc_hit *d_parts, int32_t nparts, int32_t nq, int32_t k,
                             rsx_sc_hit *d_out, void *stream) try {
  if (!h || !d_parts || !d_out || nparts < 1 || nq < 1 || k < 1 || k > RSX_SC_MAX_TOPK) return fail(RSX_ERR_BAD_ARG, "bad arg");
  std::lock_guard<std::mutex> lk(h->mu);
  RSX_TRY(set_device(h));
  hipStream_t s;
  RSX_TRY(use_stream(h, stream, &s));
  return launch_merge(d_parts, nparts, nq, k, d_out, s);
} RSX_CATCH_ALL

int rsx_sc_profile_enable(rsx_sc *h, int on) try {
  if (!h) return fail(RSX_ERR_BAD_ARG, "null handle");
  std::lock_guard<std::mutex> lk(h->mu);
  RSX_TRY(own_stream(h));
  if (on && !h->prof.ev) {
    h->prof.ev.reset(new (std::nothrow) Event[2 * PairProfiler::kMax]);
    if (!h->prof.ev) return fail(RSX_ERR_OOM, "host alloc");
    for (int i = 0; i < 2 * PairProfiler::kMax; i++) RSX_HIP(h->prof.ev[i].create(true));
  }
  if (on) {
    RSX_TRY(h->stats.reserve(kStatBytes, h->stream, false));
    RSX_HIP(hipMemsetAsync(h->stats.p, 0, kStatBytes, h->stream));
    RSX_HIP(hipStreamSynchronize(h->stream));
  }
  h->prof.on = on != 0;
  h->prof.used = 0;
  return RSX_OK;
} RSX_CATCH_ALL

int rsx_sc_profile_read_rescoring(rsx_sc *h, rsx_sc_rescoring_stats *out) try {
  if (!h || !out || out->struct_size < offsetof(rsx_sc_rescoring_stats, candidates)) return fail(RSX_ERR_BAD_ARG, "null arg / struct_size not set");
  int64_t out6[8];
  int64_t *const out5 = out6;
  int64_t *candidates = out5, *exact_evals = out5 + 1, *queries_rescored = out5 + 2;
  struct Publish {
    rsx_sc_rescoring_stats *o;
    const int64_t *v;
    ~Publish() {
      int64_t *dst = &o->candidates;
      const size_t n = (o->struct_size - offsetof(rsx_sc_rescoring_stats, candidates)) / sizeof(int64_t);
      for (size_t i = 0; i < n && i < 8; i++) dst[i] = v[i];
    }
  } publish{out, out6};
  std::lock_guard<std::mutex> lk(h->mu);
  RSX_TRY(set_device(h));
  for (int i = 0; i < 8; i++) out6[i] = 0;
  if (!h->stats.p) return RSX_OK;
  RSX_HIP(hipDeviceSynchronize());
  unsigned long long v[RESCORE_STAT_WORDS] = {0};
  {
    std::vector<unsigned long long> all((size_t)RESCORE_STAT_COPIES * RESCORE_STAT_WORDS);
    RSX_HIP(hipMemcpy(all.data(), h->stats.p, kStatBytes, hipMemcpyDeviceToHost));
    RSX_HIP(hipMemset(h->stats.p, 0, kStatBytes));
    for (int c = 0; c < RESCORE_STAT_COPIES; c++)
      for (int i = 0; i < RESCORE_STAT_WORDS; i++) v[i] += all[(size_t)c * RESCORE_STAT_WORDS + i];
  }
  if (rsx::exp_env("RSX_RESCORE_PROF") && v[1])
    fprintf(stderr, "[sc_rescore prof] per query (cycles of wave 0): load %.0f  phaseA %.0f  mergeA %.0f  phaseB %.0f  mergeX %.0f  gather %.0f  total %.0f\n",
            (double)v[4] / v[1], (double)v[5] / v[1], (double)v[6] / v[1], (double)v[7] / v[1], (double)v[8] / v[1], (double)v[9] / v[1],
            (double)v[10] / v[1]);
  if (rsx::exp_env("RSX_RESCORE_PROF") && v[1] && v[13])
    fprintf(stderr, "[sc_rescore prof] wave kernel: header %.0f  records %.0f (then tau_ub = the 'phaseA' figure)\n", (double)v[13] / v[1], (double)v[14] / v[1]);
  *candidates = (int64_t)v[0];
  *exact_evals = v[2] ? (int64_t)v[2] : (int64_t)v[0];
  *queries_rescored = (int64_t)v[1];
  out5[3] = (int64_t)v[3];
  out5[4] = (int64_t)v[11];
  out6[5] = v[12] ? (int64_t)v[12] : 7 * *exact_evals;
  out6[6] = (int64_t)v[15];
  out6[7] = (int64_t)v[16];
  return RSX_OK;
} RSX_CATCH_ALL

int rsx_sc_profile_read(rsx_sc *h, int64_t *launches, double *total_ms) try {
  if (!h || !launches || !total_ms) return fail(RSX_ERR_BAD_ARG, "null arg");
  std::lock_guard<std::mutex> lk(h->mu);
  RSX_TRY(set_device(h));
  *launches = 0;
  *total_ms = 0.0;
  for (int i = 0; i < h->prof.used; i++) {
    RSX_HIP(hipEventSynchronize(h->prof.ev[2 * i + 1]));
    float ms = 0.f;
    RSX_HIP(hipEventElapsedTime(&ms, h->prof.ev[2 * i], h->prof.ev[2 * i + 1]));
    *total_ms += ms;
    (*launches)++;
  }
  h->prof.used = 0;
  return RSX_OK;
} RSX_CATCH_ALL

int rsx_sc_hit_to_loop(rsx_sc *h, const rsx_sc_hit *hit, int32_t *loop_id, float *yaw) try {
  if (!h || !hit) return fail(RSX_ERR_BAD_ARG, "null arg");
  std::lock_guard<std::mutex> lk(h->mu);
  if (loop_id) *loop_id = (hit->dist < h->p.dist_thres) ? hit->index : -1;
  if (yaw) *yaw = yaw_from_shift(hit->shift);
  return RSX_OK;
} RSX_CATCH_ALL

}
```

navtech-radar-slam_amd/csrc/sc_kernels.h:

```cpp
#pragma once
#include <hip/hip_runtime.h>

#include <cstdint>

#include "rsx_common.h"

namespace rsx {
namespace sc {

constexpr int NR = RSX_SC_NUM_RING;
constexpr int NS = RSX_SC_NUM_SECTOR;
constexpr int DS = RSX_SC_DESC_SIZE;

struct DbView {
  const float *desc;
  const double *vkey;
  const double *norm;
  const float *rkey;
  const void *hnT;
  const uint64_t *cmask;
  const void *spT;
  const float *sp_aux;
  const void *hnR;
  const void *vk16;
  const float *vk_n;
  int64_t n_local;
  int64_t idx_base;
  int64_t idx_stride;
  int32_t sum_order;
};

using lb_t = _Float16;
typedef _Float16 lb2_t __attribute__((ext_vector_type(2)));
constexpr int RESCORE_BINS = 2048;
#ifdef __HIPCC__
__device__ __forceinline__ lb_t lb_pack(float v) {
  return __builtin_bit_cast(lb2_t, __builtin_amdgcn_cvt_pkrtz(v, 0.0f))[0];
}
__device__ __forceinline__ int lb_bin(float d) {
  if (!(d > 0.0f)) return 0;
  const float x = d * (float)RESCORE_BINS;
  return x >= (float)(RESCORE_BINS - 1) ? RESCORE_BINS - 1 : (int)x;
}
__device__ __forceinline__ float lb_bin_edge(int b) {
  return b < 0 ? -INFINITY : (b >= RESCORE_BINS - 1 ? INFINITY : (float)(b + 1) / (float)RESCORE_BINS);
}
__device__ __forceinline__ int lb_edge_bin(float edge) {
  return edge == -INFINITY ? -1 : (edge == INFINITY ? RESCORE_BINS - 1 : (int)(edge * (float)RESCORE_BINS) - 1);
}
__device__ __forceinline__ float lb_bin_lo(int b) {
  return b <= 0 ? -INFINITY : (float)b / (float)RESCORE_BINS;
}
#endif

struct QueryView {
  const float *desc;
  const double *vkey;
  const double *norm;
  int32_t nq;
};

int launch_keys(const float *desc, int64_t n, double *vkey, double *norm, float *rkey, hipStream_t s, int sum_order);

int launch_build(const void *d_pts, int64_t n_pts, int64_t stride_bytes, double lidar_height,
                 double max_radius, float *out_desc, double *out_vkey, double *out_norm,
                 float *out_rkey, hipStream_t s, int sum_order);

int pair_num_slots(int64_t n_items, int32_t nq);
size_t pair_partial_bytes(int64_t n_items, int32_t nq, int32_t k);

int launch_pairs(const DbView &db, const QueryView &q, const int32_t *gather, int64_t first,
                 int64_t n_items, int64_t n_eligible, const int64_t *q_elig, double *out_dist,
                 int32_t *out_shift, rsx_sc_hit *d_partial, rsx_sc_hit *d_topk, int32_t k,
                 hipStream_t s);

int launch_insert(const void *d_pts, const int64_t *d_offs, int64_t n_pts, int64_t n_clouds, int64_t stride_bytes,
                  double lidar_height, double max_radius, int64_t first_slot, float *desc, double *vkey, double *norm,
                  float *rkey, void *hnT, void *hnR, uint64_t *cmask, void *spT, float *aux, void *vk16, float *vk_n,
                  hipStream_t s, int sum_order);

int launch_merge(const rsx_sc_hit *d_parts, int32_t nparts, int32_t nq, int32_t k, rsx_sc_hit *d_out,
                 hipStream_t s);

int launch_gather_bounds(const lb_t *d_blocks, int64_t block_ld, int64_t block_stride, int64_t q0, int32_t nq, lb_t *d_lb,
                         int64_t ld, hipStream_t s);

int launch_knn(const float *rkeys, int64_t n_search, const float *qkey, int32_t k, float *d_dist_ws,
               int32_t *out_idx, float *out_dist, int32_t *out_found, hipStream_t s);

constexpr int RESCORE_SHORTLIST_CAP = 2048;
constexpr int RESCORE_HEAD = 512;
static_assert(RESCORE_HEAD >= RSX_SC_WINDOW_P && RESCORE_HEAD <= RESCORE_SHORTLIST_CAP,
              "the head must cover every list position sc_window_kernel may read (WINDOW_P)");
constexpr int RESCORE_NUM_THR = 6;
constexpr int RESCORE_THR_HEAD_BIN = 2 * RESCORE_NUM_THR, RESCORE_THR_HEAD_END = 2 * RESCORE_NUM_THR + 1;
constexpr int RESCORE_THR_STRIDE = 16;
static_assert(RESCORE_THR_HEAD_END < RESCORE_THR_STRIDE, "layout");
constexpr int RESCORE_STAT_WORDS = 24, RESCORE_STAT_COPIES = 64;
struct WindowPreview;
struct RescoreEntry {
  float lb;
  int32_t slot;
};
int launch_select(const DbView &db, const lb_t *lb, int64_t ld_lb, int64_t n_items, int32_t nq, int64_t n_eligible,
                  const int64_t *q_elig, int32_t first_target, RescoreEntry *slist, int32_t *sl_cnt, float *thr,
                  hipStream_t s);
constexpr int RESCORE_ALL_ROUNDS = RESCORE_NUM_THR + 1;
int launch_rescore(const DbView &db, const QueryView &q, const lb_t *lb, int64_t ld_lb, int64_t n_items,
                   int64_t n_eligible, const int64_t *q_elig, const RescoreEntry *slist, const int32_t *sl_cnt,
                   const float *thr, double eps, int32_t round_begin, int32_t round_end, const rsx_sc_hit *tau_src,
                   const rsx_sc_hit *seed, rsx_sc_hit *d_out, int32_t k, hipStream_t s, unsigned long long *d_stats,
                   const WindowPreview *win);

constexpr int FILTER_QIMG_BYTES = 9984;
constexpr int FILTER_QIMG_ODD = 4960;
constexpr int FILTER_QIMG_MASK_OFF = 4928;
constexpr float FILTER_ACC_SCALE = 1073741824.0f;
constexpr int FILTER_DB_BYTES_PER_ENTRY = 2 * DS;
double filter_eps();
size_t filter_qimg_bytes(int32_t nq);
int launch_db_images(const float *desc, const double *norm, int64_t first, int64_t count, void *hnT, void *hnR,
                     uint64_t *cmask, hipStream_t s);
int launch_query_images(const float *desc, const double *norm, int32_t nq, void *qimg, hipStream_t s);
struct FilterPlanInput {
  int64_t n_eligible;
  const int64_t *q_elig;
};
size_t filter_plan_bytes(int64_t n_items);
int launch_filter_plan(const DbView &db, const FilterPlanInput &plan, int32_t nq, int64_t n_items, int32_t qgroup,
                       void *plan_ws, const int32_t **tb_qmin, const int64_t **tb_cum, hipStream_t s);
int launch_filter(const DbView &db, const void *qimg, int32_t nq, int64_t n_items, lb_t *lb, int64_t ld_lb,
                  const FilterPlanInput *plan, void *plan_ws, hipStream_t s);
const char *pair_kernel_name();
const char *filter_kernel_name();

constexpr int SPEC_QIMG_BYTES = 4736;
constexpr int SPEC_DB_BYTES_PER_ENTRY = 2432;
size_t spec_qimg_bytes(int32_t nq);
int launch_spec_db_images(const float *desc, const double *norm, int64_t first, int64_t count, void *spT, float *aux,
                          hipStream_t s);
int launch_spec_query_images(const float *desc, const double *norm, int32_t nq, void *qimg, hipStream_t s);
int launch_spec_filter(const DbView &db, const void *qimg, int32_t nq, int64_t n_items, lb_t *lb, int64_t ld_lb,
                       const int32_t *tb_qmin, const int64_t *tb_cum, hipStream_t s, bool two_waves);
const char *spec_filter_kernel_name();
const char *spec2_filter_kernel_name();

constexpr int WINDOW_P = RSX_SC_WINDOW_P;
constexpr int WINDOW_HEAD = 128;
constexpr float WINDOW_MARGIN = RSX_SC_WINDOW_MARGIN;
constexpr int WINDOW_QK_BYTES = 4624;
static_assert(WINDOW_P % 64 == 0 && WINDOW_HEAD == 128 && WINDOW_P > WINDOW_HEAD, "layout");
struct WindowPreview {
  float pv;
  int32_t ks;
};
size_t window_qimg_bytes(int32_t nq);
int launch_window_db_keys(const double *vkey, int64_t first, int64_t count, void *vk16, float *vk_n, hipStream_t s);
int launch_window(const DbView &db, const QueryView &q, void *qimg, const RescoreEntry *slist, const int32_t *sl_cnt,
                  int32_t k, double eps, WindowPreview *out, hipStream_t s);
const char *window_kernel_name();

constexpr int Q1_MAX_NQ = 16;
int q1_grid(int64_t n_items, int32_t k, int32_t nq);
size_t q1_workspace_bytes(int64_t n_items, int32_t nq, int32_t k);
size_t q1_ticket_bytes();
int launch_q1(const DbView &db, const float *d_q, int32_t nq, int64_t n_items, int64_t n_eligible, const int64_t *q_elig,
              int32_t k, rsx_sc_hit *d_out, void *ws, unsigned *d_ticket, unsigned long long *d_stats, hipStream_t s);
const char *q1_kernel_name();

int launch_helper(int op, const double *d_a, const double *d_b, double *d_out_d, int32_t *d_out_i, hipStream_t s, int sum_order);

struct PairProfiler {
  bool on = false;
  static constexpr int kMax = 4096;
  std::unique_ptr<Event[]> ev;
  int used = 0;
};
void set_pair_profiler(PairProfiler *p);

}
}
```

navtech-radar-slam_amd/csrc/sc_kernels.hip:

```cpp
#include <hip/hip_runtime.h>

#include <cmath>
#include <cstdint>
#include <cstdio>
#include <cstdlib>

#include "rsx_common.h"
#include "sc_kernels.h"
#include "sc_entry_dev.h"
#include "sc_exact_dev.h"

namespace rsx {
namespace sc {

namespace {

using dev::wave_keys;


template <int SO>
__global__ __launch_bounds__(256) void sc_keys_kernel(const float *__restrict__ desc, int64_t n,
                                                      double *__restrict__ vkey, double *__restrict__ norm,
                                                      float *__restrict__ rkey) {
  const int lane = threadIdx.x & 63;
  int64_t i = (int64_t)blockIdx.x * 4 + (threadIdx.x >> 6);
  if (i >= n) return;
  wave_keys<SO>(desc + i * DS, vkey + i * NS, norm + i * NS, rkey + i * NR, lane);
}

template <int SO>
__global__ __launch_bounds__(256) void sc_build_kernel(const char *__restrict__ pts, int64_t n_pts,
                                                       int64_t stride, double lidar_height,
                                                       double max_radius, float *__restrict__ out_desc,
                                                       double *__restrict__ out_vkey,
                                                       double *__restrict__ out_norm,
                                                       float *__restrict__ out_rkey) {
  __shared__ __attribute__((aligned(16))) unsigned bins[DS];
  dev::build_block<SO>(pts, n_pts, stride, lidar_height, max_radius, bins, out_desc, out_vkey, out_norm, out_rkey);
}

constexpr int Q_COL_STRIDE = 176;
constexpr int OFF_QIMG = 0;
constexpr int OFF_QN1 = 60 * Q_COL_STRIDE;
constexpr int OFF_QV1 = OFF_QN1 + 512;
constexpr int OFF_WAVES = OFF_QV1 + 512;
constexpr int QP_COL_STRIDE = NR * 4;
constexpr int QP_FLAG = NS * QP_COL_STRIDE;
constexpr int QP_MASK = QP_FLAG + 8;
constexpr int QP_V1F = QP_FLAG + 16;
constexpr int QP_SIZE = QP_V1F + NS * 4;

template <int B>
struct PairLds {
  static constexpr int WAVE_SIZE = B * ENT_SIZE;
  static constexpr int SIZE = OFF_WAVES + 4 * WAVE_SIZE;
};

struct PairArgs {
  DbView db;
  QueryView q;
  const int32_t *gather;
  int64_t first, n_items, n_eligible;
  const int64_t *q_elig;
  double *out_dist;
  int32_t *out_shift;
  rsx_sc_hit *partial;
  int32_t k, nslots;
};


template <int B>
constexpr int pair_waves_per_simd() {
  constexpr int blocks = (160 * 1024) / PairLds<B>::SIZE;
  return blocks < 1 ? 1 : (blocks > 4 ? 4 : blocks);
}


constexpr float kFastAlignEps = 1.6e-5f;
__host__ __device__ constexpr int fimg_base(int j) { return (j == 0 ? 0 : j == 1 ? 37 : j == 2 ? 73 : 109) * 16; }
typedef float float2p __attribute__((ext_vector_type(2)));

constexpr float kPreviewMargin = 1e-4f;


template <int B, int SO = dev::SO_SSE2>
__device__ __forceinline__ void pair_group(const DbView &db, const char *smem, char *wsm, int lane,
                                           const int64_t (&eslot)[B], double &bd_out, int &bk_out) {
  const int cl = lane < NS ? lane : 0;
  const int kk = lane < NS ? lane : NS - 1;
  const double *v1 = reinterpret_cast<const double *>(smem + OFF_QV1);
  const double *qn1 = reinterpret_cast<const double *>(smem + OFF_QN1);
  float4 ecol[B][5];
  double en2[B], ev[B];
    wave_lds_fence();
#pragma unroll
    for (int b = 0; b < B; b++) {
      ev[b] = db.vkey[eslot[b] * NS + cl];
      const float4 *src = reinterpret_cast<const float4 *>(db.desc + eslot[b] * DS + cl * NR);
#pragma unroll
      for (int i = 0; i < 5; i++) ecol[b][i] = src[i];
      en2[b] = db.norm[eslot[b] * NS + cl];
    }

    int kstar[B];
#pragma unroll
    for (int b = 0; b < B; b++) {
      const double v = ev[b];
      double *vka = reinterpret_cast<double *>(wsm + b * ENT_SIZE + ENT_VKEY_A);
      double *vkb = reinterpret_cast<double *>(wsm + b * ENT_SIZE + ENT_VKEY_B);
      if (lane < NS) {
        vka[lane] = v;
        vka[lane + NS] = v;
        vkb[lane + 1] = v;
        vkb[lane + NS + 1] = v;
      }
    }
    wave_lds_fence();

    double acc[B][4];
#pragma unroll
    for (int b = 0; b < B; b++)
#pragma unroll
      for (int l = 0; l < 4; l++) acc[b][l] = 0.0;
    {
      const double2 *v2[B];
      const int eoff = (kk & 1) ? (ENT_VKEY_B + (NS + 1 - kk) * 8) : (ENT_VKEY_A + (NS - kk) * 8);
#pragma unroll
      for (int b = 0; b < B; b++) v2[b] = reinterpret_cast<const double2 *>(wsm + b * ENT_SIZE + eoff);
      const double2 *v1p = reinterpret_cast<const double2 *>(v1);
#pragma unroll 1
      for (int c0 = 0; c0 < NS / 2; c0 += 6) {
#pragma unroll
        for (int cc = 0; cc < 6; cc++) {
          const double2 x = v1p[c0 + cc];
#pragma unroll
          for (int b = 0; b < B; b++) {
            const double2 y = v2[b][c0 + cc];
            double d0 = x.x - y.x;
            double dd0 = d0 * d0;
            acc[b][2 * (cc & 1)] = acc[b][2 * (cc & 1)] + dd0;
            double d1 = x.y - y.y;
            double dd1 = d1 * d1;
            acc[b][2 * (cc & 1) + 1] = acc[b][2 * (cc & 1) + 1] + dd1;
          }
        }
      }
    }
#pragma unroll
    for (int b = 0; b < B; b++) {
      double nrm = sqrt((acc[b][0] + acc[b][2]) + (acc[b][1] + acc[b][3]));
      if constexpr (SO != dev::SO_SSE2) {
        const int eoff = (kk & 1) ? (ENT_VKEY_B + (NS + 1 - kk) * 8) : (ENT_VKEY_A + (NS - kk) * 8);
        const double *v2d = reinterpret_cast<const double *>(wsm + b * ENT_SIZE + eoff);
        auto d = [&](int c) { return v1[c] - v2d[c]; };
        nrm = sqrt(dev::redux_prod<SO, NS>(d, d));
      }
      bool ok = (lane < NS) && (nrm < kBig);
      double m = ok ? nrm : INFINITY;
#pragma unroll
      for (int off = 32; off >= 1; off >>= 1) m = fmin(m, __shfl_xor(m, off));
      unsigned long long bal = __ballot(ok && nrm == m);
      kstar[b] = bal ? (__ffsll((long long)bal) - 1) : 0;
    }

    wave_lds_fence();
#pragma unroll
    for (int b = 0; b < B; b++) {
      const int ks = kstar[b];
      double e[NR];
#pragma unroll
      for (int i = 0; i < 5; i++) {
        e[4 * i + 0] = ecol[b][i].x; e[4 * i + 1] = ecol[b][i].y;
        e[4 * i + 2] = ecol[b][i].z; e[4 * i + 3] = ecol[b][i].w;
      }
      const double n2 = en2[b];
      double *simp = reinterpret_cast<double *>(wsm + b * ENT_SIZE + ENT_SIM);
      int *misc = reinterpret_cast<int *>(wsm + b * ENT_SIZE + ENT_MISC);
#pragma unroll
      for (int t = 0; t < 7; t++) {
        int k = ks + t - 3;
        k += (k < 0) ? NS : 0;
        k -= (k >= NS) ? NS : 0;
        int c = cl + k;
        c -= (c >= NS) ? NS : 0;
        const double2 *qp = reinterpret_cast<const double2 *>(smem + OFF_QIMG + c * Q_COL_STRIDE);
        double da[4] = {0.0, 0.0, 0.0, 0.0};
#pragma unroll
        for (int i = 0; i < 10; i++) {
          double2 q2 = qp[i];
          da[2 * (i & 1)] = fma(q2.x, e[2 * i + 0], da[2 * (i & 1)]);
          da[2 * (i & 1) + 1] = fma(q2.y, e[2 * i + 1], da[2 * (i & 1) + 1]);
        }
        double dot = (da[0] + da[2]) + (da[1] + da[3]);
        if constexpr (SO != dev::SO_SSE2) {
          const double *qd = reinterpret_cast<const double *>(qp);
          dot = dev::redux_prod<SO, NR>([&](int r) { return qd[r]; }, [&](int r) { return e[r]; });
        }
        const double n1 = qn1[c];
        const bool valid = (lane < NS) && !((n1 == 0.0) | (n2 == 0.0));
        const double s = dot / (n1 * n2);
        if (lane < NS) simp[t * NS + c] = valid ? s : 0.0;
        const int ne = __popcll(__ballot(valid));
        if (lane == 0) misc[t] = ne;
      }
      if (lane == 0) misc[7] = ks;
    }
    wave_lds_fence();

    const int bb = lane >> 3, tt = lane & 7;
    double bd = INFINITY;
    int bk = 0x7fffffff;
    if (bb < B && tt < 7) {
      const double2 *sp = reinterpret_cast<const double2 *>(wsm + bb * ENT_SIZE + ENT_SIM + tt * (NS * 8));
      const int *misc = reinterpret_cast<const int *>(wsm + bb * ENT_SIZE + ENT_MISC);
      double s = 0.0;
#pragma unroll 1
      for (int c0 = 0; c0 < NS / 2; c0 += 6) {
#pragma unroll
        for (int cc = 0; cc < 6; cc++) {
          const double2 v = sp[c0 + cc];
          s = s + v.x;
          s = s + v.y;
        }
      }
      const int ne = misc[tt];
      const double d = 1.0 - s / (double)ne;
      int k = misc[7] + tt - 3;
      k += (k < 0) ? NS : 0;
      k -= (k >= NS) ? NS : 0;
      if (d < kBig) {
        bd = d;
        bk = k;
      }
    }
#pragma unroll
    for (int off = 1; off <= 4; off <<= 1) {
      double od = __shfl_xor(bd, off);
      int ok = __shfl_xor(bk, off);
      if (hit_before(od, ok, bd, bk)) {
        bd = od;
        bk = ok;
      }
    }
    if (bd == INFINITY) {
      bd = kBig;
      bk = 0;
    }

    bd_out = bd;
    bk_out = bk;
}


template <int SO = dev::SO_SSE2>
__device__ __forceinline__ int phase_a(const char *smem, char *wsm, int lane, const EntryRegs &er, int off_preview,
                                       float e1, float &pv) {
  const int cl = lane < NS ? lane : 0;
  const int kk = lane < NS ? lane : NS - 1;
  const double *v1 = reinterpret_cast<const double *>(smem + OFF_QV1);
  wave_lds_fence();
  const double ev = er.v;
  const float4 (&ecol)[5] = er.ecol;
  const double n2 = er.n2;
  int kstar = 0;
  bool need_exact = true;
  {
    const float vf = (float)ev;
    if (lane < NS) {
#pragma unroll
      for (int j = 0; j < 4; j++) {
        float *img = reinterpret_cast<float *>(wsm + fimg_base(j));
        if (lane >= j) img[lane - j] = vf;
        img[lane + NS - j] = vf;
        if (lane < j) img[lane + 2 * NS - j] = vf;
      }
    }
    const float e2 = wave_sum_f32(lane < NS ? vf * vf : 0.0f);
    wave_lds_fence();
    const int j = (-kk) & 3;
    const float4 *yp = reinterpret_cast<const float4 *>(wsm + fimg_base(j) + (NS - kk - j) * 4);
    const float4 *xp = reinterpret_cast<const float4 *>(smem + off_preview + QP_V1F);
    float2p a0 = {0.0f, 0.0f}, a1 = {0.0f, 0.0f};
#pragma unroll 5
    for (int i = 0; i < NS / 4; i++) {
      const float4 x = xp[i], y = yp[i];
      const float2p d0 = float2p{x.x, x.y} - float2p{y.x, y.y}, d1 = float2p{x.z, x.w} - float2p{y.z, y.w};
      a0 = __builtin_elementwise_fma(d0, d0, a0);
      a1 = __builtin_elementwise_fma(d1, d1, a1);
    }
    const float D = (a0[0] + a0[1]) + (a1[0] + a1[1]);
    const float dmin = wave_min_f32(lane < NS ? D : INFINITY);
    const float thr = dmin + 2.0f * kFastAlignEps * (e1 + e2);
    const unsigned long long nan_bal = __ballot(lane < NS && !(D == D));
    const unsigned long long cand = __ballot(lane < NS && D <= thr);
    if (!nan_bal && dmin < 1e12f && thr < 3.0e38f && __popcll(cand) == 1) {
      kstar = __ffsll((long long)cand) - 1;
      need_exact = false;
    }
    wave_lds_fence();
  }
  if (need_exact) kstar = align_exact<SO>(v1, wsm, lane, ev);
  pv = __builtin_nanf("");
  if (*reinterpret_cast<const int *>(smem + off_preview + QP_FLAG)) {
    const bool n2_ok = (n2 == 0.0) || (n2 >= 1e-15 && n2 <= 1e15);
    if (!__ballot(!n2_ok && lane < NS)) {
      const float r2 = (n2 == 0.0 || lane >= NS) ? 0.0f : (float)(1.0 / n2);
      const unsigned long long me = __ballot(lane < NS && n2 != 0.0);
      const unsigned long long mq = *reinterpret_cast<const unsigned long long *>(smem + off_preview + QP_MASK);
      float p[8];
      int k0 = kstar - 3;
      k0 += (k0 < 0) ? NS : 0;
      int k = k0;
      int c = cl + k;
      c -= (c >= NS) ? NS : 0;
#pragma unroll
      for (int t = 0; t < 7; t++) {
        const float4 *qp = reinterpret_cast<const float4 *>(smem + off_preview + c * QP_COL_STRIDE);
        float2p d0 = {0.0f, 0.0f}, d1 = {0.0f, 0.0f};
#pragma unroll
        for (int i = 0; i < 5; i++) {
          const float4 q4 = qp[i];
          d0 = __builtin_elementwise_fma(float2p{q4.x, q4.y}, float2p{ecol[i].x, ecol[i].y}, d0);
          d1 = __builtin_elementwise_fma(float2p{q4.z, q4.w}, float2p{ecol[i].z, ecol[i].w}, d1);
        }
        p[t] = ((d0[0] + d0[1]) + (d1[0] + d1[1])) * r2;
        c = (c + 1 == NS) ? 0 : c + 1;
      }
      p[7] = 0.0f;
      const bool b0 = lane & 1, b1 = lane & 2, b2 = lane & 4;
      float q4v[4];
#pragma unroll
      for (int i = 0; i < 4; i++) {
        const float keep = b0 ? p[2 * i + 1] : p[2 * i], send = b0 ? p[2 * i] : p[2 * i + 1];
        q4v[i] = keep + __shfl_xor(send, 1);
      }
      float q2v[2];
#pragma unroll
      for (int i = 0; i < 2; i++) {
        const float keep = b1 ? q4v[2 * i + 1] : q4v[2 * i], send = b1 ? q4v[2 * i] : q4v[2 * i + 1];
        q2v[i] = keep + __shfl_xor(send, 2);
      }
      float sv;
      {
        const float keep = b2 ? q2v[1] : q2v[0], send = b2 ? q2v[0] : q2v[1];
        sv = keep + __shfl_xor(send, 4);
      }
      sv += __shfl_xor(sv, 8);
      sv += __shfl_xor(sv, 16);
      sv += __shfl_xor(sv, 32);
      float best = INFINITY;
      bool broken = false;
      k = k0;
#pragma unroll
      for (int t = 0; t < 7; t++) {
        const float st = __builtin_bit_cast(float, __builtin_amdgcn_readlane(__builtin_bit_cast(int, sv), t));
        const unsigned long long rq = ((mq >> k) | (mq << (NS - k))) & ((1ull << NS) - 1ull);
        const int ne = __popcll(rq & me);
        k = (k + 1 == NS) ? 0 : k + 1;
        if (ne != 0) {
          const float d = 1.0f - st * __builtin_amdgcn_rcpf((float)ne);
          if (!(d == d)) broken = true;
          best = fminf(best, d);
        }
      }
      if (!broken) pv = best;
    }
  }
  return kstar;
}

template <int SO = dev::SO_SSE2>
__device__ __forceinline__ void phase_b(const char *smem, char *wsm, int lane, const EntryRegs &er, int ks, double &bd_out,
                                        int &bk_out) {
  const int cl = lane < NS ? lane : 0;
  const double *qn1 = reinterpret_cast<const double *>(smem + OFF_QN1);
  wave_lds_fence();
  double e[NR];
#pragma unroll
  for (int i = 0; i < 5; i++) {
    const float4 v = er.ecol[i];
    e[4 * i + 0] = v.x; e[4 * i + 1] = v.y; e[4 * i + 2] = v.z; e[4 * i + 3] = v.w;
  }
  const double n2 = er.n2;
  double *simp = reinterpret_cast<double *>(wsm + ENT_SIM);
  int *misc = reinterpret_cast<int *>(wsm + ENT_MISC);
#pragma unroll
  for (int t = 0; t < 7; t++) {
    int k = ks + t - 3;
    k += (k < 0) ? NS : 0;
    k -= (k >= NS) ? NS : 0;
    int c = cl + k;
    c -= (c >= NS) ? NS : 0;
    const double2 *qp = reinterpret_cast<const double2 *>(smem + OFF_QIMG + c * Q_COL_STRIDE);
    double da[4] = {0.0, 0.0, 0.0, 0.0};
#pragma unroll
    for (int i = 0; i < 10; i++) {
      const double2 q2 = qp[i];
      da[2 * (i & 1)] = fma(q2.x, e[2 * i + 0], da[2 * (i & 1)]);
      da[2 * (i & 1) + 1] = fma(q2.y, e[2 * i + 1], da[2 * (i & 1) + 1]);
    }
    double dot = (da[0] + da[2]) + (da[1] + da[3]);
    if constexpr (SO != dev::SO_SSE2) {
      const double *qd = reinterpret_cast<const double *>(qp);
      dot = dev::redux_prod<SO, NR>([&](int r) { return qd[r]; }, [&](int r) { return e[r]; });
    }
    const double n1 = qn1[c];
    const bool valid = (lane < NS) && !((n1 == 0.0) | (n2 == 0.0));
    const double s = dot / (n1 * n2);
    if (lane < NS) simp[t * NS + c] = valid ? s : 0.0;
    const int ne = __popcll(__ballot(valid));
    if (lane == 0) misc[t] = ne;
  }
  wave_lds_fence();
  const int tt = lane & 7;
  double bd = INFINITY;
  int bk = 0x7fffffff;
  if (lane < 8 && tt < 7) {
    const double2 *sp = reinterpret_cast<const double2 *>(wsm + ENT_SIM + tt * (NS * 8));
    double s = 0.0;
#pragma unroll 1
    for (int c0 = 0; c0 < NS / 2; c0 += 6) {
#pragma unroll
      for (int cc = 0; cc < 6; cc++) {
        const double2 v = sp[c0 + cc];
        s = s + v.x;
        s = s + v.y;
      }
    }
    const int ne = misc[tt];
    const double d = 1.0 - s / (double)ne;
    int k = ks + tt - 3;
    k += (k < 0) ? NS : 0;
    k -= (k >= NS) ? NS : 0;
    if (d < kBig) {
      bd = d;
      bk = k;
    }
  }
#pragma unroll
  for (int off = 1; off <= 4; off <<= 1) {
    const double od = __shfl_xor(bd, off);
    const int ok = __shfl_xor(bk, off);
    if (hit_before(od, ok, bd, bk)) {
      bd = od;
      bk = ok;
    }
  }
  bd = __shfl(bd, 0);
  bk = __shfl(bk, 0);
  if (bd == INFINITY) {
    bd = kBig;
    bk = 0;
  }
  bd_out = bd;
  bk_out = bk;
}

__device__ __forceinline__ void load_query_to_lds(const QueryView &q, int qi, char *smem, int tid, int nthreads,
                                                  int off_preview = -1) {
  const float4 *qd4 = reinterpret_cast<const float4 *>(q.desc + (int64_t)qi * DS);
  const double *qn = q.norm + (int64_t)qi * NS, *qv = q.vkey + (int64_t)qi * NS;
  double kn = 0.0, kv = 0.0;
  if (tid < NS) {
    kn = qn[tid];
    kv = qv[tid];
  }
  for (int t = tid; t < DS / 4; t += nthreads) {
    const int c = t / (NR / 4), r0 = (t - c * (NR / 4)) * 4;
    const float4 x = qd4[t];
    const double n1 = off_preview >= 0 ? qn[c] : 1.0;
    const float xe[4] = {x.x, x.y, x.z, x.w};
    double *img = reinterpret_cast<double *>(smem + OFF_QIMG + c * Q_COL_STRIDE + r0 * 8);
#pragma unroll
    for (int e = 0; e < 4; e++) img[e] = (double)xe[e];
    if (off_preview >= 0) {
      float4 u;
      u.x = (n1 == 0.0) ? 0.0f : (float)((double)xe[0] / n1);
      u.y = (n1 == 0.0) ? 0.0f : (float)((double)xe[1] / n1);
      u.z = (n1 == 0.0) ? 0.0f : (float)((double)xe[2] / n1);
      u.w = (n1 == 0.0) ? 0.0f : (float)((double)xe[3] / n1);
      *reinterpret_cast<float4 *>(smem + off_preview + (c * NR + r0) * 4) = u;
    }
  }
  if (off_preview >= 0) {
    const bool bad = tid < NS && (kn != 0.0) && !(kn >= 1e-15 && kn <= 1e15);
    if (__ballot(bad)) *reinterpret_cast<int *>(smem + off_preview + QP_FLAG) = 0;
    if (tid < NS) reinterpret_cast<float *>(smem + off_preview + QP_V1F)[tid] = (float)kv;
    if (tid < 64) {
      const unsigned long long m = __ballot(tid < NS && kn != 0.0);
      if (tid == 0) *reinterpret_cast<unsigned long long *>(smem + off_preview + QP_MASK) = m;
    }
  }
  if (tid < NS) {
    reinterpret_cast<double *>(smem + OFF_QN1)[tid] = kn;
    reinterpret_cast<double *>(smem + OFF_QV1)[tid] = kv;
  }
}


template <int B, int W, int SO>
__global__ __launch_bounds__(256, W) void sc_pair_kernel(PairArgs a) {
  extern __shared__ __attribute__((aligned(16))) char smem[];
  const int lane = threadIdx.x & 63;
  const int wave = threadIdx.x >> 6;
  char *wsm = smem + OFF_WAVES + wave * PairLds<B>::WAVE_SIZE;
  const int qi = blockIdx.y;
  const int slot = blockIdx.x * 4 + wave;
  const int nwaves = gridDim.x * 4;

  load_query_to_lds(a.q, qi, smem, threadIdx.x, 256);
  __syncthreads();

  int64_t n_elig = a.n_eligible;
  if (a.q_elig) {
    int64_t e = a.q_elig[qi];
    n_elig = e < n_elig ? e : n_elig;
  }

  double ld = INFINITY;
  int li = 0x7fffffff, ls = 0;

  const int32_t *gath = a.gather;
  const int64_t n_items = a.n_items;
  const int64_t ngroups = (n_items + B - 1) / B;
  for (int64_t g = slot; g < ngroups; g += nwaves) {
    int64_t eslot[B];
    bool evalid[B];
#pragma unroll
    for (int b = 0; b < B; b++) {
      int64_t item = g * B + b;
      evalid[b] = item < n_items;
      int64_t it = evalid[b] ? item : (n_items - 1);
      eslot[b] = gath ? (int64_t)gath[it] : (a.first + it);
    }
    double bd;
    int bk;
    pair_group<B, SO>(a.db, smem, wsm, lane, eslot, bd, bk);

#pragma unroll
    for (int b = 0; b < B; b++) {
      const double dist = __shfl(bd, b * 8);
      const int shift = __shfl(bk, b * 8);
      if (!evalid[b]) continue;
      const int64_t item = g * B + b;
      if (a.out_dist && lane == 0) {
        a.out_dist[(int64_t)qi * n_items + item] = dist;
        a.out_shift[(int64_t)qi * n_items + item] = shift;
      }
      if (a.partial) {
        const int64_t gidx = a.db.idx_base + eslot[b] * a.db.idx_stride;
        if (gidx < n_elig && dist < kBig) {
          topk_insert(ld, li, ls, lane, a.k, dist, (int)gidx, shift);
        }
      }
    }
  }

  if (a.partial && lane < a.k) {
    rsx_sc_hit h;
    h.dist = ld;
    h.index = li;
    h.shift = ls;
    a.partial[((int64_t)qi * a.nslots + slot) * a.k + lane] = h;
  }
}

constexpr int PAIR2_OFF_QP32 = OFF_WAVES + 4 * ENT_SIZE;
constexpr int PAIR2_LDS = PAIR2_OFF_QP32 + QP_SIZE;

template <int W, int SO>
__global__ __launch_bounds__(256, W) void sc_pair2_kernel(PairArgs a) {
  extern __shared__ __attribute__((aligned(16))) char smem[];
  const int lane = threadIdx.x & 63;
  const int wave = threadIdx.x >> 6;
  char *wsm = smem + OFF_WAVES + wave * ENT_SIZE;
  const int qi = blockIdx.y;
  const int slot = blockIdx.x * 4 + wave;
  const int nwaves = gridDim.x * 4;

  if (threadIdx.x == 0) *reinterpret_cast<int *>(smem + PAIR2_OFF_QP32 + QP_FLAG) = 1;
  __syncthreads();
  load_query_to_lds(a.q, qi, smem, threadIdx.x, 256, PAIR2_OFF_QP32);
  __syncthreads();
  const float v1f = lane < NS ? reinterpret_cast<const float *>(smem + PAIR2_OFF_QP32 + QP_V1F)[lane] : 0.0f;
  const float e1 = wave_sum_f32(v1f * v1f);

  int64_t n_elig = a.n_eligible;
  if (a.q_elig) {
    const int64_t e = a.q_elig[qi];
    n_elig = e < n_elig ? e : n_elig;
  }
  double ld = INFINITY;
  int li = 0x7fffffff, ls = 0;
  const int32_t *gath = a.gather;
  EntryRegs cur;
  Touch tch;
  for (int64_t g = slot; g < a.n_items; g += nwaves) {
    const int64_t eslot = gath ? (int64_t)gath[g] : (a.first + g);
    const int64_t gidx = a.db.idx_base + eslot * a.db.idx_stride;
    if (gidx >= n_elig) continue;
    if (g + nwaves < a.n_items) touch_entry(a.db, gath ? (int64_t)gath[g + nwaves] : (a.first + g + nwaves), lane, tch);
    load_entry(a.db, eslot, lane, cur);
    float pv;
    const int ks = phase_a<SO>(smem, wsm, lane, cur, PAIR2_OFF_QP32, e1, pv);
    touch_keep(tch);
    const double kth = __shfl(ld, a.k - 1);
    if ((pv == pv) && (double)pv - (double)kPreviewMargin > kth) continue;
    double bd;
    int bk;
    phase_b<SO>(smem, wsm, lane, cur, ks, bd, bk);
    if (bd < kBig) topk_insert(ld, li, ls, lane, a.k, bd, (int)gidx, bk);
  }
  if (lane < a.k) {
    rsx_sc_hit h;
    h.dist = ld;
    h.index = li;
    h.shift = ls;
    a.partial[((int64_t)qi * a.nslots + slot) * a.k + lane] = h;
  }
}

__global__ __launch_bounds__(256) void sc_gather_bounds_kernel(const lb_t *__restrict__ blocks, int64_t block_ld,
                                                               int64_t block_stride, int64_t q0, lb_t *__restrict__ lb,
                                                               int64_t ld) {
  const int64_t c = ((int64_t)blockIdx.x * 256 + threadIdx.x) * 8;
  if (c >= ld) return;
  const int64_t q = blockIdx.y, b = c / block_ld, j = c - b * block_ld;
  const uint4 v = *reinterpret_cast<const uint4 *>(blocks + b * block_stride + (q0 + q) * block_ld + j);
  *reinterpret_cast<uint4 *>(lb + q * ld + c) = v;
}

__global__ __launch_bounds__(64) void sc_merge_kernel(const rsx_sc_hit *__restrict__ parts, int32_t nparts,
                                                      int64_t part_stride, int64_t q_stride, int32_t per_part,
                                                      int32_t k, rsx_sc_hit *__restrict__ out) {
  const int q = blockIdx.x;
  const int lane = threadIdx.x;
  double pd = -INFINITY;
  int pi = -1;
  const int64_t total = (int64_t)nparts * per_part;
  for (int r = 0; r < k; r++) {
    double bd = INFINITY;
    int bi = 0x7fffffff, bs = 0;
    for (int64_t t = lane; t < total; t += 64) {
      const int p = (int)(t / per_part), i = (int)(t % per_part);
      rsx_sc_hit h = parts[(int64_t)p * part_stride + (int64_t)q * q_stride + i];
      const bool pad = !(h.dist < kBig);
      if (pad) continue;
      if (hit_before(pd, pi, h.dist, h.index) && hit_before(h.dist, h.index, bd, bi)) {
        bd = h.dist; bi = h.index; bs = h.shift;
      }
    }
#pragma unroll
    for (int off = 32; off >= 1; off >>= 1) {
      double od = __shfl_xor(bd, off);
      int oi = __shfl_xor(bi, off), os = __shfl_xor(bs, off);
      if (hit_before(od, oi, bd, bi)) {
        bd = od; bi = oi; bs = os;
      }
    }
    if (lane == 0) {
      rsx_sc_hit h;
      if (bd == INFINITY) {
        h.dist = kBig; h.index = 0; h.shift = 0;
      } else {
        h.dist = bd; h.index = bi; h.shift = bs;
      }
      out[(int64_t)q * k + r] = h;
    }
    pd = bd;
    pi = bi;
  }
}

__global__ __launch_bounds__(1024) void sc_knn_kernel(const float *__restrict__ rkeys, int64_t n,
                                                      const float *__restrict__ qkey, int32_t k,
                                                      float *__restrict__ dist_ws, int32_t *__restrict__ out_idx,
                                                      float *__restrict__ out_dist, int32_t *__restrict__ out_found) {
  __shared__ float sq[NR];
  __shared__ float rd[16];
  __shared__ int ri[16];
  __shared__ float pick_d;
  __shared__ int pick_i;
  if (threadIdx.x < NR) sq[threadIdx.x] = qkey[threadIdx.x];
  __syncthreads();
  for (int64_t i = threadIdx.x; i < n; i += 1024) {
    const float4 *p = reinterpret_cast<const float4 *>(rkeys + i * NR);
    float result = 0.0f;
#pragma unroll
    for (int g = 0; g < 5; g++) {
      float4 v = p[g];
      float d0 = __fsub_rn(sq[4 * g + 0], v.x), d1 = __fsub_rn(sq[4 * g + 1], v.y);
      float d2 = __fsub_rn(sq[4 * g + 2], v.z), d3 = __fsub_rn(sq[4 * g + 3], v.w);
      float t = __fadd_rn(__fadd_rn(__fadd_rn(__fmul_rn(d0, d0), __fmul_rn(d1, d1)), __fmul_rn(d2, d2)),
                          __fmul_rn(d3, d3));
      result = __fadd_rn(result, t);
    }
    dist_ws[i] = result;
  }
  __syncthreads();
  float pd = -1.0f;
  int pi = -1;
  int found = 0;
  for (int r = 0; r < k; r++) {
    float bd = INFINITY;
    int bi = 0x7fffffff;
    for (int64_t i = threadIdx.x; i < n; i += 1024) {
      float d = dist_ws[i];
      bool after = (d > pd) || (d == pd && (int)i > pi);
      if (after && ((d < bd) || (d == bd && (int)i < bi))) {
        bd = d;
        bi = (int)i;
      }
    }
#pragma unroll
    for (int off = 32; off >= 1; off >>= 1) {
      float od = __shfl_xor(bd, off);
      int oi = __shfl_xor(bi, off);
      if ((od < bd) || (od == bd && oi < bi)) {
        bd = od; bi = oi;
      }
    }
    if ((threadIdx.x & 63) == 0) {
      rd[threadIdx.x >> 6] = bd;
      ri[threadIdx.x >> 6] = bi;
    }
    __syncthreads();
    if (threadIdx.x == 0) {
      float d = rd[0];
      int ix = ri[0];
      for (int w = 1; w < 16; w++)
        if ((rd[w] < d) || (rd[w] == d && ri[w] < ix)) {
          d = rd[w]; ix = ri[w];
        }
      pick_d = d;
      pick_i = ix;
    }
    __syncthreads();
    pd = pick_d;
    pi = pick_i;
    if (pi != 0x7fffffff) found++;
    if (threadIdx.x == 0) {
      out_idx[r] = (pi == 0x7fffffff) ? 0 : pi;
      out_dist[r] = pd;
    }
    __syncthreads();
  }
  if (threadIdx.x == 0) out_found[0] = found;
}


struct RescoreArgs {
  DbView db;
  QueryView q;
  const lb_t *lb;
  int64_t ld_lb, n_items, n_eligible;
  const int64_t *q_elig;
  const RescoreEntry *slist;
  const int32_t *sl_cnt;
  const float *thr;
  rsx_sc_hit *out;
  const rsx_sc_hit *tau_src;
  const rsx_sc_hit *seed;
  double eps;
  int32_t k;
  int32_t round_begin, round_end;
  unsigned long long *stats;
  const WindowPreview *win;
};

template <int B, int W, int SO>
int launch_pairs_t(const PairArgs &a, int gx, hipStream_t s) {
  static_assert(W <= pair_waves_per_simd<B>(), "LDS footprint does not allow this occupancy");
  static bool attr_set = false;
  const int lds = PairLds<B>::SIZE;
  if (!attr_set) {
    RSX_HIP(hipFuncSetAttribute(reinterpret_cast<const void *>(&sc_pair_kernel<B, W, SO>),
                                hipFuncAttributeMaxDynamicSharedMemorySize, lds));
    attr_set = true;
  }
  dim3 grid(gx, a.q.nq);
  hipLaunchKernelGGL((sc_pair_kernel<B, W, SO>), grid, dim3(256), lds, s, a);
  RSX_HIP(hipGetLastError());
  return RSX_OK;
}

constexpr int kPairB = 2, kPairW = 4;

int choose_gx(int64_t n_items, int32_t nq) {
  const int kB = kPairB;
  const int64_t ngroups = (n_items + kB - 1) / kB;
  int64_t max_gx = (ngroups + 3) / 4;
  if (max_gx < 1) max_gx = 1;
  int64_t want = (2048 + 4 * (int64_t)nq - 1) / (4 * (int64_t)nq);
  if (want < 1) want = 1;
  return (int)(want < max_gx ? want : max_gx);
}

}

const char *pair_kernel_name() { return "sc_pair_kernel"; }

static thread_local PairProfiler *g_prof = nullptr;
void set_pair_profiler(PairProfiler *p) { g_prof = p; }

int pair_num_slots(int64_t n_items, int32_t nq) { return choose_gx(n_items, nq) * 4; }

size_t pair_partial_bytes(int64_t n_items, int32_t nq, int32_t k) {
  return (size_t)pair_num_slots(n_items, nq) * (size_t)nq * (size_t)k * sizeof(rsx_sc_hit);
}

int launch_keys(const float *desc, int64_t n, double *vkey, double *norm, float *rkey, hipStream_t s, int sum_order) {
  if (n <= 0) return RSX_OK;
  RSX_SO_DISPATCH(sum_order, hipLaunchKernelGGL(sc_keys_kernel<SO>, dim3((unsigned)((n + 3) / 4)), dim3(256), 0, s, desc, n, vkey, norm, rkey));
  RSX_HIP(hipGetLastError());
  return RSX_OK;
}

int launch_build(const void *d_pts, int64_t n_pts, int64_t stride_bytes, double lidar_height,
                 double max_radius, float *out_desc, double *out_vkey, double *out_norm,
                 float *out_rkey, hipStream_t s, int sum_order) {
  RSX_SO_DISPATCH(sum_order, hipLaunchKernelGGL(sc_build_kernel<SO>, dim3(1), dim3(256), 0, s, static_cast<const char *>(d_pts), n_pts,
                                                stride_bytes, lidar_height, max_radius, out_desc, out_vkey, out_norm, out_rkey));
  RSX_HIP(hipGetLastError());
  return RSX_OK;
}

int launch_merge(const rsx_sc_hit *d_parts, int32_t nparts, int32_t nq, int32_t k, rsx_sc_hit *d_out,
                 hipStream_t s) {
  if (nq <= 0) return RSX_OK;
  hipLaunchKernelGGL(sc_merge_kernel, dim3(nq), dim3(64), 0, s, d_parts, nparts, (int64_t)nq * k, (int64_t)k, k, k, d_out);
  RSX_HIP(hipGetLastError());
  return RSX_OK;
}

int launch_gather_bounds(const lb_t *d_blocks, int64_t block_ld, int64_t block_stride, int64_t q0, int32_t nq, lb_t *d_lb,
                         int64_t ld, hipStream_t s) {
  if (nq <= 0 || ld <= 0) return RSX_OK;
  if (block_ld < 32 || block_ld % 32 || ld % 8 || block_stride % 8) return fail(RSX_ERR_BAD_ARG, "bound blocks must be a multiple of 32 columns wide");
  for (int32_t r0 = 0; r0 < nq; r0 += 65535) {
    const int32_t rows = nq - r0 < 65535 ? nq - r0 : 65535;
    hipLaunchKernelGGL(sc_gather_bounds_kernel, dim3((unsigned)((ld / 8 + 255) / 256), (unsigned)rows), dim3(256), 0, s, d_blocks,
                       block_ld, block_stride, q0 + r0, d_lb + (int64_t)r0 * ld, ld);
    RSX_HIP(hipGetLastError());
  }
  return RSX_OK;
}

int launch_pairs(const DbView &db, const QueryView &q, const int32_t *gather, int64_t first,
                 int64_t n_items, int64_t n_eligible, const int64_t *q_elig, double *out_dist,
                 int32_t *out_shift, rsx_sc_hit *d_partial, rsx_sc_hit *d_topk, int32_t k,
                 hipStream_t s) {
  if (q.nq <= 0) return RSX_OK;
  if (k < 0 || k > RSX_SC_MAX_TOPK) return fail(RSX_ERR_BAD_ARG, "k=%d out of range [0,%d]", k, RSX_SC_MAX_TOPK);
  if (n_items <= 0) {
    if (d_topk && k > 0) {
      hipLaunchKernelGGL(sc_merge_kernel, dim3(q.nq), dim3(64), 0, s, (const rsx_sc_hit *)nullptr, 0,
                         (int64_t)0, (int64_t)k, k, k, d_topk);
      RSX_HIP(hipGetLastError());
    }
    return RSX_OK;
  }
  PairArgs a;
  a.db = db;
  a.q = q;
  a.gather = gather;
  a.first = first;
  a.n_items = n_items;
  a.n_eligible = n_eligible < 0 ? INT64_MAX : n_eligible;
  a.q_elig = q_elig;
  a.out_dist = out_dist;
  a.out_shift = out_shift;
  const int gx = choose_gx(n_items, q.nq);
  a.partial = (d_topk && k > 0) ? d_partial : nullptr;
  a.k = k;
  a.nslots = gx * 4;
  PairProfiler *pp = (g_prof && g_prof->on && g_prof->ev && g_prof->used < PairProfiler::kMax) ? g_prof : nullptr;
  if (pp) RSX_HIP(hipEventRecord(pp->ev[2 * pp->used], s));
  if (a.partial && !out_dist) {
    static_assert(PAIR2_LDS <= 48 * 1024, "within the default dynamic LDS limit: no per-device opt-in needed");
    RSX_SO_DISPATCH(db.sum_order, hipLaunchKernelGGL((sc_pair2_kernel<4, SO>), dim3(gx, q.nq), dim3(256), PAIR2_LDS, s, a));
    RSX_HIP(hipGetLastError());
  } else {
    int st = RSX_OK;
    RSX_SO_DISPATCH(db.sum_order, st = (launch_pairs_t<kPairB, kPairW, SO>(a, gx, s)));
    RSX_TRY(st);
  }
  if (pp) {
    RSX_HIP(hipEventRecord(pp->ev[2 * pp->used + 1], s));
    pp->used++;
  }
  if (a.partial) {
    hipLaunchKernelGGL(sc_merge_kernel, dim3(q.nq), dim3(64), 0, s, (const rsx_sc_hit *)d_partial, 1,
                       (int64_t)0, (int64_t)a.nslots * k, a.nslots * k, k, d_topk);
    RSX_HIP(hipGetLastError());
  }
  return RSX_OK;
}


constexpr int RW_CH = (WINDOW_P + 63) / 64;


#ifndef RW_OCC
#define RW_OCC 3
#endif
template <int SO>
__global__ __launch_bounds__(64, RW_OCC) void sc_rescore_wave_kernel(RescoreArgs a) {
  extern __shared__ __attribute__((aligned(16))) char smem[];
  if (a.stats) a.stats += (blockIdx.x % RESCORE_STAT_COPIES) * RESCORE_STAT_WORDS;
  const int lane = threadIdx.x;
  const int qi = blockIdx.x;
  char *wsm = smem + WaveLds::OFF_ENT;

  int64_t n_elig = a.n_eligible;
  if (a.q_elig) {
    const int64_t e = a.q_elig[qi];
    n_elig = e < n_elig ? e : n_elig;
  }
  int64_t n_rows = 0;
  if (n_elig > a.db.idx_base) {
    n_rows = (n_elig - a.db.idx_base + a.db.idx_stride - 1) / a.db.idx_stride;
    n_rows = n_rows < a.n_items ? n_rows : a.n_items;
  }

  double ld = INFINITY;
  int li = 0x7fffffff, ls = 0;
  double tau_init = INFINITY;
  if (a.tau_src) {
    const double d = a.tau_src[(int64_t)qi * a.k + (a.k - 1)].dist;
    if (d < kBig) tau_init = d;
  }
  if (a.seed && lane < a.k) {
    const rsx_sc_hit h = a.seed[(int64_t)qi * a.k + lane];
    if (h.dist < kBig) {
      ld = h.dist; li = h.index; ls = h.shift;
    }
  }
  auto kth_of = [&](double list) {
    const double t = __shfl(list, a.k - 1);
    return t < tau_init ? t : tau_init;
  };
  double tau = kth_of(ld);
  bool query_loaded = false;
  unsigned n_exact = 0, n_looked = 0, n_aligned = 0, n_shifts = 0, n_tail = 0;
  unsigned nl_lane = 0, n_windowed = 0;
  bool walked_tail = false;

#ifdef RSX_EXPERIMENTS
  const bool timing = a.stats != nullptr;
#else
  constexpr bool timing = false;
#endif
  long long tacc[9] = {0, 0, 0, 0, 0, 0, 0, 0, 0};
  long long t_mark = timing ? clock64() : 0;
  const long long t_begin = t_mark;
  auto lap = [&](int slot_) {
    if (!timing) return;
    const long long t = clock64();
    tacc[slot_] += t - t_mark;
    t_mark = t;
  };
  auto eval = [&](int64_t slot, int ksm, const EntryRegs &er) {
    if (timing) {
      lap(2);
      asm volatile("s_waitcnt vmcnt(0)" ::: "memory");
      lap(5);
    }
    int ks = ksm;
    unsigned tmask = 0x7fu;
    if (ksm >= 0) {
      ks = ksm & 63;
      const unsigned m7 = ((unsigned)ksm >> 8) & 0x7fu;
      if (m7) tmask = m7;
    }
    if (!query_loaded) {
      const float4 *src = reinterpret_cast<const float4 *>(a.q.desc + (int64_t)qi * DS);
      float4 *dst = reinterpret_cast<float4 *>(smem + WaveLds::OFF_QF32);
      float4 x[5];
#pragma unroll
      for (int i = 0; i < 5; i++) x[i] = (lane + 64 * i < DS / 4) ? src[lane + 64 * i] : float4{0.f, 0.f, 0.f, 0.f};
      const double kn = lane < NS ? a.q.norm[(int64_t)qi * NS + lane] : 0.0;
      const double kv = lane < NS ? a.q.vkey[(int64_t)qi * NS + lane] : 0.0;
#pragma unroll
      for (int i = 0; i < 5; i++)
        if (lane + 64 * i < DS / 4) dst[lane + 64 * i] = x[i];
      if (lane < NS) {
        reinterpret_cast<double *>(smem + WaveLds::OFF_QN1)[lane] = kn;
        reinterpret_cast<double *>(smem + WaveLds::OFF_QV1)[lane] = kv;
      }
      query_loaded = true;
      wave_lds_fence();
      lap(0);
    }
    if (ks < 0) {
      ks = align_exact<SO>(reinterpret_cast<const double *>(smem + WaveLds::OFF_QV1), wsm, lane, er.v);
      n_aligned++;
      lap(4);
    }
    double bd;
    int bk;
    phase_b32<SO>(smem, wsm, lane, er, ks, tmask, bd, bk);
    if (timing) {
      asm volatile("" : "+v"(bd));
      lap(3);
    }
    n_exact++;
    n_shifts += (unsigned)__builtin_popcount(tmask);
    const int64_t gidx = a.db.idx_base + slot * a.db.idx_stride;
    if (gidx < n_elig && bd < kBig) {
      topk_insert(ld, li, ls, lane, a.k, bd, (int)gidx, bk);
      tau = kth_of(ld);
    }
  };

  const int sl_cnt = a.sl_cnt[qi];
  const RescoreEntry *sl = a.slist + (int64_t)qi * RESCORE_SHORTLIST_CAP;
  const float *thr = a.thr + (int64_t)qi * RESCORE_THR_STRIDE;
  const int32_t *rcnt = reinterpret_cast<const int32_t *>(thr) + RESCORE_NUM_THR;
  const float t_cap = thr[RESCORE_NUM_THR - 1];
  const int r_end = a.round_end < RESCORE_NUM_THR ? a.round_end : RESCORE_NUM_THR;
  auto upto = [&](int r) {
    if (r <= 0) return 0;
    const int c = rcnt[r - 1];
    return c < sl_cnt ? c : sl_cnt;
  };
  const int i0 = upto(a.round_begin), i1 = upto(r_end);
  if (timing) {
    int keep = i0 + i1;
    asm volatile("" : "+s"(keep));
    lap(7);
  }
  bool done = false;

  int pos_next = i0;
  if (a.win && i0 < WINDOW_P && i0 < i1) {
    const WindowPreview *wp = a.win + (int64_t)qi * WINDOW_P;
    const int pw = i1 < WINDOW_P ? i1 : WINDOW_P;
    float lo[RW_CH], ub[RW_CH], flb[RW_CH];
#pragma unroll
    for (int j = 0; j < RW_CH; j++) {
      const int pos = i0 + lane + 64 * j;
      lo[j] = INFINITY;
      ub[j] = INFINITY;
      flb[j] = INFINITY;
      if (pos < pw) {
        const RescoreEntry e = sl[pos];
        const WindowPreview w = wp[pos];
        const int64_t gidx = a.db.idx_base + (int64_t)e.slot * a.db.idx_stride;
        if (gidx < n_elig && !((double)e.lb - a.eps > tau)) {
          flb[j] = e.lb;
          if (!(w.pv == w.pv)) {
            lo[j] = -INFINITY;
          } else {
            lo[j] = w.pv - WINDOW_MARGIN;
            if (w.ks >= 0 && w.pv < 3.0e38f) ub[j] = w.pv + WINDOW_MARGIN;
          }
        }
      }
    }
    if (timing) {
      asm volatile("" : "+v"(lo[0]), "+v"(ub[0]));
      lap(8);
    }
    double ud = ld;
    int ui = li, us = ls;
    for (int it = 0; it < a.k; it++) {
      float m = ub[0];
#pragma unroll
      for (int j = 1; j < RW_CH; j++) m = fminf(m, ub[j]);
      const float wm = wave_min_f32(m);
      if (!((double)wm < __shfl(ud, a.k - 1))) break;
      const unsigned long long bal = __ballot(m == wm);
      const int src = __ffsll((long long)bal) - 1;
      if (lane == src) {
        bool gone = false;
#pragma unroll
        for (int j = 0; j < RW_CH; j++)
          if (!gone && ub[j] == wm) {
            ub[j] = INFINITY;
            gone = true;
          }
      }
      topk_insert(ud, ui, us, lane, a.k, (double)wm, 0x40000000 + it, 0);
    }
    const double tau_ub = kth_of(ud);
    lap(1);
#pragma unroll
    for (int j = 0; j < RW_CH; j++)
      if ((double)flb[j] - a.eps > tau_ub) lo[j] = INFINITY;
#pragma unroll
    for (int j = 0; j < RW_CH; j++) {
      nl_lane += (lo[j] < INFINITY) ? 1u : 0u;
      n_windowed += (lo[j] > -INFINITY && lo[j] < INFINITY) ? 1u : 0u;
    }
    struct Packed {
      float lo;
      int pos;
    };
    Packed *cbuf = reinterpret_cast<Packed *>(wsm);
    for (;;) {
      const double t_now = tau < tau_ub ? tau : tau_ub;
      int nsurv = 0;
#pragma unroll
      for (int j = 0; j < RW_CH; j++) {
        const bool sv = lo[j] < INFINITY && !((double)lo[j] > t_now);
        const unsigned long long bal = __ballot(sv);
        const int rank = nsurv + __popcll(bal & ((1ull << lane) - 1ull));
        if (sv && rank < 64) {
          cbuf[rank] = Packed{lo[j], i0 + lane + 64 * j};
          lo[j] = INFINITY;
        }
        nsurv += __popcll(bal);
      }
      if (nsurv == 0) break;
      nsurv = nsurv < 64 ? nsurv : 64;
      wave_lds_fence();
      float mylo = INFINITY;
      int32_t myslot = 0;
      int myks = -1;
      if (lane < nsurv) {
        const Packed c = cbuf[lane];
        mylo = c.lo;
        myslot = sl[c.pos].slot;
        const int k_ = wp[c.pos].ks;
        myks = k_ >= 0 ? k_ : -1;
      }
      wave_lds_fence();
      {
        Touch tch;
        for (int i = 0; i < nsurv; i++) touch_entry(a.db, __shfl(myslot, i), lane, tch);
        touch_wait(tch);
      }
      auto pick = [&](int32_t &slot, int &ks) -> float {
        const float wm = wave_min_f32(mylo);
        if (wm == INFINITY) return wm;
        const int src = __ffsll((long long)__ballot(mylo == wm)) - 1;
        slot = __shfl(myslot, src);
        ks = __shfl(myks, src);
        if (lane == src) mylo = INFINITY;
        return wm;
      };
      EntryRegs cur, nxt;
      int32_t cur_slot = 0, nxt_slot = 0;
      int cur_ks = -1, nxt_ks = -1;
      float cur_lo = pick(cur_slot, cur_ks);
      if (cur_lo < INFINITY) load_entry(a.db, cur_slot, lane, cur);
      while (cur_lo < INFINITY) {
        const double t_eff = tau < tau_ub ? tau : tau_ub;
        if ((double)cur_lo > t_eff) break;
        const float nxt_lo = pick(nxt_slot, nxt_ks);
        if (nxt_lo < INFINITY && !((double)nxt_lo > t_eff)) load_entry(a.db, nxt_slot, lane, nxt);
        eval(cur_slot, cur_ks, cur);
        cur_lo = nxt_lo;
        cur_slot = nxt_slot;
        cur_ks = nxt_ks;
        cur = nxt;
      }
    }
    pos_next = pw > i0 ? pw : i0;
  }

  const int head_bin = rcnt[RESCORE_THR_HEAD_BIN - RESCORE_NUM_THR], head_end = rcnt[RESCORE_THR_HEAD_END - RESCORE_NUM_THR];
  const int i1h = i1 < head_end ? i1 : head_end;
  for (int base = pos_next; base < i1h && !done; base += 64) {
    const int n_here = (i1h - base < 64) ? (i1h - base) : 64;
    RescoreEntry mine;
    mine.lb = INFINITY;
    mine.slot = 0;
    if (lane < n_here) mine = sl[base + lane];
    for (int i = 0; i < n_here; i++) {
      const float lb = __shfl(mine.lb, i);
      const int32_t slot = __shfl(mine.slot, i);
      if ((double)lb_bin_lo(lb_bin(lb)) - a.eps > tau) {
        done = true;
        break;
      }
      if ((double)lb - a.eps > tau) continue;
      const int64_t gidx = a.db.idx_base + (int64_t)slot * a.db.idx_stride;
      if (!(gidx < n_elig)) continue;
      EntryRegs er;
      load_entry(a.db, slot, lane, er);
      n_looked++;
      eval(slot, -1, er);
    }
  }

  if (!done && i1 > head_end) {
    const lb_t *row = a.lb + (int64_t)qi * a.ld_lb;
    const int b_to = lb_edge_bin(thr[r_end - 1]);
    int b = head_bin;
    if (a.round_begin > 0) {
      const int b0 = lb_edge_bin(thr[(a.round_begin < RESCORE_NUM_THR ? a.round_begin : RESCORE_NUM_THR) - 1]);
      b = b0 > b ? b0 : b;
    }
    bool take = false;
    walked_tail = b < b_to;
    while (!done && walked_tail) {
      int next = RESCORE_BINS;
      constexpr int U = 4;
      for (int64_t pos = 0; pos < n_rows && !done; pos += 64 * U) {
        float d[U];
#pragma unroll
        for (int u = 0; u < U; u++) {
          const int64_t i = pos + 64 * u + lane;
          d[u] = (i < n_rows) ? (float)row[i] : INFINITY;
        }
#pragma unroll
        for (int u = 0; u < U; u++) {
          const int bin = (d[u] != INFINITY) ? lb_bin(d[u]) : RESCORE_BINS;
          if (bin > b && bin < next) next = bin;
          unsigned long long bal = __ballot(take && bin == b);
          while (bal && !done) {
            const int l = __ffsll((long long)bal) - 1;
            bal &= bal - 1;
            if ((double)lb_bin_lo(b) - a.eps > tau) {
              done = true;
              break;
            }
            const float dl = __shfl(d[u], l);
            if ((double)dl - a.eps > tau) continue;
            const int64_t slot = pos + 64 * u + l;
            EntryRegs er;
            load_entry(a.db, slot, lane, er);
            n_looked++;
            n_tail++;
            eval(slot, -1, er);
          }
        }
      }
      if (done) break;
#pragma unroll
      for (int off = 32; off >= 1; off >>= 1) {
        const int o = __shfl_xor(next, off);
        next = o < next ? o : next;
      }
      if (next > b_to) break;
      b = next;
      take = true;
      if ((double)lb_bin_lo(b) - a.eps > tau) done = true;
    }
  }

  if (!done && a.round_end > RESCORE_NUM_THR && t_cap < INFINITY && !((double)t_cap - a.eps > tau)) {
    const lb_t *row = a.lb + (int64_t)qi * a.ld_lb;
    const bool take_all = (t_cap == -INFINITY);
    for (int64_t pos = 0; pos < n_rows; pos += 64) {
      const int64_t i = pos + lane;
      const float d = (i < n_rows) ? (float)row[i] : INFINITY;
      const bool beyond = take_all ? true : (d >= t_cap);
      unsigned long long bal = __ballot((i < n_rows) && beyond && (d != INFINITY));
      while (bal) {
        const int l = __ffsll((long long)bal) - 1;
        bal &= bal - 1;
        const float dl = __shfl(d, l);
        if ((double)dl - a.eps > tau) continue;
        EntryRegs er;
        load_entry(a.db, pos + l, lane, er);
        n_looked++;
        eval(pos + l, -1, er);
      }
    }
  }

  if (lane < a.k) {
    rsx_sc_hit h;
    if (ld == INFINITY) {
      h.dist = kBig; h.index = 0; h.shift = 0;
    } else {
      h.dist = ld; h.index = li; h.shift = ls;
    }
    a.out[(int64_t)qi * a.k + lane] = h;
  }
  if (a.stats) {
    unsigned lk = nl_lane, wd = n_windowed;
#pragma unroll
    for (int off = 32; off >= 1; off >>= 1) {
      lk += __shfl_xor(lk, off);
      wd += __shfl_xor(wd, off);
    }
    if (lane == 0) {
      atomicAdd(a.stats, (unsigned long long)(lk + n_looked));
      atomicAdd(a.stats + 3, (unsigned long long)wd);
      atomicAdd(a.stats + 2, (unsigned long long)n_exact);
      atomicAdd(a.stats + 11, (unsigned long long)n_aligned);
      atomicAdd(a.stats + 12, (unsigned long long)n_shifts);
      atomicAdd(a.stats + 15, (unsigned long long)n_tail);
      if (walked_tail) atomicAdd(a.stats + 16, 1ull);
      if (timing) {
        for (int i = 0; i < 6; i++) atomicAdd(a.stats + 4 + i, (unsigned long long)tacc[i]);
        atomicAdd(a.stats + 13, (unsigned long long)tacc[7]);
        atomicAdd(a.stats + 14, (unsigned long long)tacc[8]);
        atomicAdd(a.stats + 10, (unsigned long long)(clock64() - t_begin));
      }
      if (n_exact) atomicAdd(a.stats + 1, 1ull);
    }
  }
}

int launch_rescore(const DbView &db, const QueryView &q, const lb_t *lb, int64_t ld_lb, int64_t n_items,
                   int64_t n_eligible, const int64_t *q_elig, const RescoreEntry *slist, const int32_t *sl_cnt,
                   const float *thr, double eps, int32_t round_begin, int32_t round_end, const rsx_sc_hit *tau_src,
                   const rsx_sc_hit *seed, rsx_sc_hit *d_out, int32_t k, hipStream_t s, unsigned long long *d_stats,
                   const WindowPreview *win) {
  if (q.nq <= 0) return RSX_OK;
  if (k < 1 || k > RSX_SC_MAX_TOPK) return fail(RSX_ERR_BAD_ARG, "k=%d out of range [1,%d]", k, RSX_SC_MAX_TOPK);
  RescoreArgs a;
  a.db = db;
  a.q = q;
  a.lb = lb;
  a.ld_lb = ld_lb;
  a.n_items = n_items;
  a.n_eligible = n_eligible < 0 ? INT64_MAX : n_eligible;
  a.q_elig = q_elig;
  a.slist = slist;
  a.sl_cnt = sl_cnt;
  a.thr = thr;
  a.out = d_out;
  a.tau_src = tau_src;
  a.seed = seed;
  a.eps = eps;
  a.k = k;
  a.round_begin = round_begin;
  a.round_end = round_end;
  a.stats = d_stats;
  a.win = win;
  RSX_SO_DISPATCH(db.sum_order, hipLaunchKernelGGL(sc_rescore_wave_kernel<SO>, dim3(q.nq), dim3(64), WaveLds::SIZE, s, a));
  RSX_HIP(hipGetLastError());
  return RSX_OK;
}

int launch_knn(const float *rkeys, int64_t n_search, const float *qkey, int32_t k, float *d_dist_ws,
               int32_t *out_idx, float *out_dist, int32_t *out_found, hipStream_t s) {
  hipLaunchKernelGGL(sc_knn_kernel, dim3(1), dim3(1024), 0, s, rkeys, n_search, qkey, k, d_dist_ws, out_idx,
                     out_dist, out_found);
  RSX_HIP(hipGetLastError());
  return RSX_OK;
}

}
}
```

navtech-radar-slam_amd/csrc/sc_window.hip:

```cpp
#include <hip/hip_runtime.h>

#include <cmath>
#include <cstdint>

#include "rsx_common.h"
#include "sc_kernels.h"
#include "sc_entry_dev.h"
#include "sc_window_dev.h"

namespace rsx {
namespace sc {

namespace {

using win::half8;
using win::floatx16;
using win::u64;
using win::kNonFinite;
using win::W_STEPS;
using win::W_TILE1;
using win::QK_COPY;
using win::QK_LO;
using win::QK_NORM;
using win::W_LDS;

#ifndef WIN_OCC
#define WIN_OCC 4
#endif
#ifndef WIN_RING
#define WIN_RING 15
#endif
__global__ __launch_bounds__(256) void sc_win_db_keys_kernel(const double *__restrict__ vkey, int64_t first, int64_t count,
                                                             _Float16 *__restrict__ vk16, float *__restrict__ vk_n) {
  const int lane = threadIdx.x & 63, wave = threadIdx.x >> 6;
  const int64_t it = (int64_t)blockIdx.x * 4 + wave;
  if (it >= count) return;
  dev::win_db_keys_entry(vkey, first + it, vk16, vk_n, lane);
}

__global__ __launch_bounds__(256) void sc_win_query_keys_kernel(const double *__restrict__ vkey, int32_t nq,
                                                                char *__restrict__ qk) {
  __shared__ _Float16 st[4][2][128];
  const int lane = threadIdx.x & 63, wave = threadIdx.x >> 6;
  const int q = blockIdx.x * 4 + wave;
  if (q >= nq) return;
  win::query_keys_image(lane < NS ? vkey[(int64_t)q * NS + lane] : 0.0, st[wave], qk + (int64_t)q * WINDOW_QK_BYTES, lane);
}

struct WindowArgs {
  const char *hnR;
  const char *vk16;
  const float *vk_n;
  const u64 *cmask;
  const char *qimg;
  const char *qkimg;
  const RescoreEntry *slist;
  const int32_t *sl_cnt;
  WindowPreview *out;
  double eps;
  int32_t k;
};

__global__ __launch_bounds__(256, WIN_OCC) void sc_window_kernel(WindowArgs a) {
  extern __shared__ __attribute__((aligned(16))) char smem[];
  __shared__ float s_ub[WINDOW_HEAD];
  __shared__ int s_pos[WINDOW_P];
  __shared__ int s_n2;
  const int lane = threadIdx.x & 63, wave = threadIdx.x >> 6;
  const int qi = blockIdx.x;
  const int sl_cnt = a.sl_cnt[qi];
  if (sl_cnt <= 0) return;
  {
    const uint4 *g0 = reinterpret_cast<const uint4 *>(a.qimg + (int64_t)qi * FILTER_QIMG_BYTES);
    const uint4 *g1 = reinterpret_cast<const uint4 *>(a.qkimg + (int64_t)qi * WINDOW_QK_BYTES);
    uint4 *l = reinterpret_cast<uint4 *>(smem);
    for (int i = threadIdx.x; i < W_LDS / 16; i += 256) l[i] = i < FILTER_QIMG_BYTES / 16 ? g0[i] : g1[i - FILTER_QIMG_BYTES / 16];
  }
  __syncthreads();
  const int n = lane & 31, hh = lane >> 5;
  const RescoreEntry *sl = a.slist + (int64_t)qi * RESCORE_SHORTLIST_CAP;
  const u64 qm = *reinterpret_cast<const u64 *>(smem + FILTER_QIMG_MASK_OFF);
  const float nq_key = *reinterpret_cast<const float *>(smem + FILTER_QIMG_BYTES + QK_NORM);
  const float uq_key = *reinterpret_cast<const float *>(smem + FILTER_QIMG_BYTES + QK_NORM + 4);
  const char *ap = smem + ((n & 1) ? (FILTER_QIMG_ODD + 40 * n - 8) : (40 * n)) + 16 * hh;
  const char *kp = smem + FILTER_QIMG_BYTES + (n & 7) * QK_COPY + ((n & ~7) + 8 * hh) * 2;

  auto do_group = [&](int pos, bool have, int pos_any) -> float {
    const int64_t slot = sl[have ? pos : pos_any].slot;

    floatx16 k0 = {0}, k1 = {0};
    {
      const char *bk = a.vk16 + slot * 256 + 16 * hh;
      half8 bh[4], bl[4];
#pragma unroll
      for (int s = 0; s < 4; s++) {
        bh[s] = *reinterpret_cast<const half8 *>(bk + 32 * s);
        bl[s] = *reinterpret_cast<const half8 *>(bk + 128 + 32 * s);
      }
#pragma unroll
      for (int s = 0; s < 4; s++) {
        const half8 ah0 = *reinterpret_cast<const half8 *>(kp + 32 * s);
        const half8 al0 = *reinterpret_cast<const half8 *>(kp + QK_LO + 32 * s);
        const half8 ah1 = *reinterpret_cast<const half8 *>(kp + 64 + 32 * s);
        const half8 al1 = *reinterpret_cast<const half8 *>(kp + QK_LO + 64 + 32 * s);
        k0 = __builtin_amdgcn_mfma_f32_32x32x16_f16(ah0, bh[s], k0, 0, 0, 0);
        k1 = __builtin_amdgcn_mfma_f32_32x32x16_f16(ah1, bh[s], k1, 0, 0, 0);
        k0 = __builtin_amdgcn_mfma_f32_32x32x16_f16(ah0, bl[s], k0, 0, 0, 0);
        k1 = __builtin_amdgcn_mfma_f32_32x32x16_f16(ah1, bl[s], k1, 0, 0, 0);
        k0 = __builtin_amdgcn_mfma_f32_32x32x16_f16(al0, bh[s], k0, 0, 0, 0);
        k1 = __builtin_amdgcn_mfma_f32_32x32x16_f16(al1, bh[s], k1, 0, 0, 0);
      }
    }
    u64 win;
    int kstar;
    win::alignment_of(k0, k1, nq_key, uq_key, reinterpret_cast<const float2 *>(a.vk_n)[slot], hh, win, kstar);

    __builtin_amdgcn_sched_barrier(0);
    floatx16 acc0 = {0}, acc1 = {0};
    {
      const char *brow = a.hnR + slot * (2 * DS) + 16 * hh;
      constexpr int R = WIN_RING;
      static_assert(W_STEPS % R == 0, "whole ring turns");
      half8 ring[R];
#pragma unroll
      for (int u = 0; u < R; u++) ring[u] = *reinterpret_cast<const half8 *>(brow + 32 * u);
#pragma unroll 1
      for (int s0 = 0; s0 < W_STEPS - R; s0 += R) {
#pragma unroll
        for (int u = 0; u < R; u++) {
          const half8 a0 = *reinterpret_cast<const half8 *>(ap + 32 * (s0 + u));
          const half8 a1 = *reinterpret_cast<const half8 *>(ap + 32 * (s0 + u + W_TILE1));
          acc0 = __builtin_amdgcn_mfma_f32_32x32x16_f16(a0, ring[u], acc0, 0, 0, 0);
          acc1 = __builtin_amdgcn_mfma_f32_32x32x16_f16(a1, ring[u], acc1, 0, 0, 0);
          ring[u] = *reinterpret_cast<const half8 *>(brow + 32 * (s0 + R + u));
        }
      }
#pragma unroll
      for (int u = 0; u < R; u++) {
        const half8 a0 = *reinterpret_cast<const half8 *>(ap + 32 * (W_STEPS - R + u));
        const half8 a1 = *reinterpret_cast<const half8 *>(ap + 32 * (W_STEPS - R + u + W_TILE1));
        acc0 = __builtin_amdgcn_mfma_f32_32x32x16_f16(a0, ring[u], acc0, 0, 0, 0);
        acc1 = __builtin_amdgcn_mfma_f32_32x32x16_f16(a1, ring[u], acc1, 0, 0, 0);
      }
    }

    __builtin_amdgcn_sched_barrier(0);
    const u64 em = a.cmask[slot];
    const float pv = win::preview_of(acc0, acc1, qm, em, win, kstar, hh);
    if (have && hh == 0) {
      WindowPreview o;
      o.pv = pv;
      o.ks = kstar;
      a.out[(int64_t)qi * WINDOW_P + pos] = o;
    }
    return (have && kstar >= 0 && pv < 3.0e38f) ? pv + WINDOW_MARGIN : INFINITY;
  };

  float tau_ub;
  {
    const int cnt1 = sl_cnt < WINDOW_HEAD ? sl_cnt : WINDOW_HEAD;
    float ub = INFINITY;
    if (wave * 32 < cnt1) ub = do_group(wave * 32 + n, wave * 32 + n < cnt1, wave * 32);
    if (hh == 0) s_ub[wave * 32 + n] = ub;
    __syncthreads();
    if (sl_cnt <= WINDOW_HEAD) return;

    {
      const float v0 = s_ub[lane], v1 = s_ub[lane + 64];
      int r0 = 0, r1 = 0;
      const float4 *u4 = reinterpret_cast<const float4 *>(s_ub);
#pragma unroll 4
      for (int j = 0; j < WINDOW_HEAD / 4; j++) {
        const float4 u = u4[j];
        const float x[4] = {u.x, u.y, u.z, u.w};
#pragma unroll
        for (int e = 0; e < 4; e++) {
          const int idx = 4 * j + e;
          r0 += (x[e] < v0 || (x[e] == v0 && idx < lane)) ? 1 : 0;
          r1 += (x[e] < v1 || (x[e] == v1 && idx < lane + 64)) ? 1 : 0;
        }
      }
      const int want = a.k - 1;
      const unsigned long long b0 = __ballot(r0 == want), b1 = __ballot(r1 == want);
      const float c0 = __shfl(v0, b0 ? __ffsll((long long)b0) - 1 : 0), c1 = __shfl(v1, b1 ? __ffsll((long long)b1) - 1 : 0);
      tau_ub = b0 ? c0 : c1;
    }
  }
  if (wave == 0) {
    int n2 = 0;
    const int lim = sl_cnt < WINDOW_P ? sl_cnt : WINDOW_P;
    for (int p0 = WINDOW_HEAD; p0 < lim; p0 += 64) {
      const int pos = p0 + lane;
      bool pass = false;
      if (pos < lim) {
        const float lb = sl[pos].lb;
        pass = !((double)lb - a.eps > (double)tau_ub);
        if (!pass) {
          WindowPreview o;
          o.pv = __builtin_nanf("");
          o.ks = -2;
          a.out[(int64_t)qi * WINDOW_P + pos] = o;
        }
      }
      const unsigned long long bal = __ballot(pass);
      if (pass) s_pos[n2 + __popcll(bal & ((1ull << lane) - 1ull))] = pos;
      n2 += __popcll(bal);
    }
    if (lane == 0) s_n2 = n2;
  }
  __syncthreads();
  const int n2 = s_n2;
  for (int g = wave; g * 32 < n2; g += 4) {
    const bool have = g * 32 + n < n2;
    (void)do_group(s_pos[have ? g * 32 + n : g * 32], have, s_pos[g * 32]);
  }
}

}

size_t window_qimg_bytes(int32_t nq) { return (size_t)nq * (FILTER_QIMG_BYTES + WINDOW_QK_BYTES) + 1024; }

int launch_window_db_keys(const double *vkey, int64_t first, int64_t count, void *vk16, float *vk_n, hipStream_t s) {
  if (count <= 0) return RSX_OK;
  hipLaunchKernelGGL(sc_win_db_keys_kernel, dim3((unsigned)((count + 3) / 4)), dim3(256), 0, s, vkey, first, count,
                     static_cast<_Float16 *>(vk16), vk_n);
  RSX_HIP(hipGetLastError());
  return RSX_OK;
}

int launch_window(const DbView &db, const QueryView &q, void *qimg, const RescoreEntry *slist, const int32_t *sl_cnt,
                  int32_t k, double eps, WindowPreview *out, hipStream_t s) {
  if (q.nq <= 0) return RSX_OK;
  char *img = static_cast<char *>(qimg);
  char *kimg = img + (size_t)q.nq * FILTER_QIMG_BYTES;
  RSX_TRY(launch_query_images(q.desc, q.norm, q.nq, img, s));
  hipLaunchKernelGGL(sc_win_query_keys_kernel, dim3((unsigned)((q.nq + 3) / 4)), dim3(256), 0, s, q.vkey, q.nq, kimg);
  RSX_HIP(hipGetLastError());
  WindowArgs a;
  a.hnR = static_cast<const char *>(db.hnR);
  a.vk16 = static_cast<const char *>(db.vk16);
  a.vk_n = db.vk_n;
  a.cmask = reinterpret_cast<const u64 *>(db.cmask);
  a.qimg = img;
  a.qkimg = kimg;
  a.slist = slist;
  a.sl_cnt = sl_cnt;
  a.out = out;
  a.eps = eps;
  a.k = k < 1 ? 1 : (k > WINDOW_HEAD ? WINDOW_HEAD : k);
  hipLaunchKernelGGL(sc_window_kernel, dim3((unsigned)q.nq), dim3(256), W_LDS, s, a);
  RSX_HIP(hipGetLastError());
  return RSX_OK;
}

const char *window_kernel_name() { return "sc_window_kernel"; }

}
}
```

Baseline: 3.263 million.

## Move window survivor filtering into window kernel and emit compact survivor list

The window kernel now computes the upper-bound tau, prunes candidates by lower bound and preview window, and writes a compact per-query survivor list (header plus entries carrying slot, shift and window low bound) into a new workspace buffer. The rescore wave kernel reads this list directly instead of rebuilding the bounds from the preview array and shortlist, re-running its top-k insertion loop and compacting through LDS. Query descriptor loading in rescore is also hoisted to kernel start. This moves work from the serial single-wave rescore kernel to the 256-thread window kernel, at the cost of extra LDS arrays and a tail pass in the window kernel. The tau used for pruning is now the float head value instead of a double recomputed from the exact top-k seed.

Result: faster. 3.301 million, median of 6 (+1.2%).

```diff
diff --git a/navtech-radar-slam_amd/csrc/sc_api.cpp b/navtech-radar-slam_amd/csrc/sc_api.cpp
--- a/navtech-radar-slam_amd/csrc/sc_api.cpp
+++ b/navtech-radar-slam_amd/csrc/sc_api.cpp
@@ -49,7 +49,7 @@
   struct QueryWs {
     DevBuf q_vkey, q_norm, q_rkey, partial;
     DevBuf f_qimg, f_lb, f_cand, f_cnt, f_thr, f_plan;
-    DevBuf f_wimg, f_win;
+    DevBuf f_wimg, f_win, f_surv;
   } ws[2];
   QueryWs *w = &ws[0];
   PairProfiler prof;
@@ -285,6 +285,7 @@
   RSX_TRY(h->w->f_thr.reserve((size_t)qb * RESCORE_THR_STRIDE * sizeof(float), s, false));
   RSX_TRY(h->w->f_wimg.reserve(window_qimg_bytes((int32_t)qb), s, false));
   RSX_TRY(h->w->f_win.reserve((size_t)qb * WINDOW_P * sizeof(WindowPreview), s, false));
+  RSX_TRY(h->w->f_surv.reserve((size_t)qb * WINDOW_LIST_STRIDE * sizeof(WindowSurvivor), s, false));
   return RSX_OK;
 }
 
@@ -301,7 +302,7 @@
   RSX_TRY(launch_select(db, lb, ld, n_items, q.nq, n_eligible, elig, first_target, h->w->f_cand.as<RescoreEntry>(),
                         h->w->f_cnt.as<int32_t>(), h->w->f_thr.as<float>(), s));
   return launch_window(db, q, h->w->f_wimg.p, h->w->f_cand.as<RescoreEntry>(), h->w->f_cnt.as<int32_t>(), k, filter_eps(),
-                       h->w->f_win.as<WindowPreview>(), s);
+                       h->w->f_win.as<WindowPreview>(), h->w->f_surv.as<WindowSurvivor>(), s);
 }
 
 int rescore(rsx_sc *h, const QueryView &q, int64_t n_items, int64_t n_eligible, const int64_t *elig, int32_t round_begin,
@@ -311,7 +312,7 @@
   return launch_rescore(db_view(h), q, h->w->f_lb.as<lb_t>(), ld, n_items, n_eligible, elig, h->w->f_cand.as<RescoreEntry>(),
                         h->w->f_cnt.as<int32_t>(), h->w->f_thr.as<float>(), filter_eps(), round_begin, round_end, tau_src,
                         seed, d_out, k, s, (h->prof.on && h->stats.p) ? h->stats.as<unsigned long long>() : nullptr,
-                        h->w->f_win.as<WindowPreview>());
+                        h->w->f_surv.as<WindowSurvivor>());
 }
 
 int32_t first_round_target() {
@@ -1257,7 +1258,7 @@
       RSX_TRY(launch_select(db, lb, ld, items, nq, elig_all, nullptr, first_round_target(), h->w->f_cand.as<RescoreEntry>(),
                             h->w->f_cnt.as<int32_t>(), h->w->f_thr.as<float>(), s));
       RSX_TRY(launch_window(db, all, h->w->f_wimg.p, h->w->f_cand.as<RescoreEntry>(), h->w->f_cnt.as<int32_t>(), k, filter_eps(),
-                            h->w->f_win.as<WindowPreview>(), s));
+                            h->w->f_win.as<WindowPreview>(), h->w->f_surv.as<WindowSurvivor>(), s));
       return rescore(h, all, items, elig_all, nullptr, 0, RESCORE_ALL_ROUNDS, nullptr, nullptr, k, h->topk.as<rsx_sc_hit>(), s);
     };
     auto all_pieces = [&]() -> int {
@@ -1349,7 +1350,7 @@
     RSX_TRY(launch_select(db, h->w->f_lb.as<lb_t>(), ld, n_items, q.nq, n_elig, nullptr, first_round_target(), h->w->f_cand.as<RescoreEntry>(),
                           h->w->f_cnt.as<int32_t>(), h->w->f_thr.as<float>(), s));
     RSX_TRY(launch_window(db, q, h->w->f_wimg.p, h->w->f_cand.as<RescoreEntry>(), h->w->f_cnt.as<int32_t>(), k, filter_eps(),
-                          h->w->f_win.as<WindowPreview>(), s));
+                          h->w->f_win.as<WindowPreview>(), h->w->f_surv.as<WindowSurvivor>(), s));
     RSX_TRY(rescore(h, q, n_items, n_elig, nullptr, 0, RESCORE_ALL_ROUNDS, nullptr, nullptr, k, d_out + b0 * k, s));
   }
   return RSX_OK;
@@ -1632,11 +1633,9 @@
       for (int i = 0; i < RESCORE_STAT_WORDS; i++) v[i] += all[(size_t)c * RESCORE_STAT_WORDS + i];
   }
   if (rsx::exp_env("RSX_RESCORE_PROF") && v[1])
-    fprintf(stderr, "[sc_rescore prof] per query (cycles of wave 0): load %.0f  phaseA %.0f  mergeA %.0f  phaseB %.0f  mergeX %.0f  gather %.0f  total %.0f\n",
+    fprintf(stderr, "[sc_rescore prof] per query (cycles): start loads %.0f  round filter + touch %.0f  pick %.0f  phaseB %.0f  align %.0f  entry wait %.0f  total %.0f\n",
             (double)v[4] / v[1], (double)v[5] / v[1], (double)v[6] / v[1], (double)v[7] / v[1], (double)v[8] / v[1], (double)v[9] / v[1],
             (double)v[10] / v[1]);
-  if (rsx::exp_env("RSX_RESCORE_PROF") && v[1] && v[13])
-    fprintf(stderr, "[sc_rescore prof] wave kernel: header %.0f  records %.0f (then tau_ub = the 'phaseA' figure)\n", (double)v[13] / v[1], (double)v[14] / v[1]);
   *candidates = (int64_t)v[0];
   *exact_evals = v[2] ? (int64_t)v[2] : (int64_t)v[0];
   *queries_rescored = (int64_t)v[1];
diff --git a/navtech-radar-slam_amd/csrc/sc_kernels.h b/navtech-radar-slam_amd/csrc/sc_kernels.h
--- a/navtech-radar-slam_amd/csrc/sc_kernels.h
+++ b/navtech-radar-slam_amd/csrc/sc_kernels.h
@@ -98,6 +98,7 @@
 static_assert(RESCORE_THR_HEAD_END < RESCORE_THR_STRIDE, "layout");
 constexpr int RESCORE_STAT_WORDS = 24, RESCORE_STAT_COPIES = 64;
 struct WindowPreview;
+struct WindowSurvivor;
 struct RescoreEntry {
   float lb;
   int32_t slot;
@@ -110,7 +111,7 @@
                    int64_t n_eligible, const int64_t *q_elig, const RescoreEntry *slist, const int32_t *sl_cnt,
                    const float *thr, double eps, int32_t round_begin, int32_t round_end, const rsx_sc_hit *tau_src,
                    const rsx_sc_hit *seed, rsx_sc_hit *d_out, int32_t k, hipStream_t s, unsigned long long *d_stats,
-                   const WindowPreview *win);
+                   const WindowSurvivor *surv);
 
 constexpr int FILTER_QIMG_BYTES = 9984;
 constexpr int FILTER_QIMG_ODD = 4960;
@@ -154,10 +155,24 @@
   float pv;
   int32_t ks;
 };
+struct WindowSurvivor {
+  float lo;
+  int32_t slot;
+  int32_t ks;
+  int32_t pos;
+};
+struct WindowListHeader {
+  int32_t count;
+  float tau_ub;
+  int32_t n_cand;
+  int32_t n_prev;
+};
+static_assert(sizeof(WindowSurvivor) == 16 && sizeof(WindowListHeader) == 16, "one 16-byte load each");
+constexpr int WINDOW_LIST_STRIDE = WINDOW_P + 1;
 size_t window_qimg_bytes(int32_t nq);
 int launch_window_db_keys(const double *vkey, int64_t first, int64_t count, void *vk16, float *vk_n, hipStream_t s);
 int launch_window(const DbView &db, const QueryView &q, void *qimg, const RescoreEntry *slist, const int32_t *sl_cnt,
-                  int32_t k, double eps, WindowPreview *out, hipStream_t s);
+                  int32_t k, double eps, WindowPreview *out, WindowSurvivor *surv, hipStream_t s);
 const char *window_kernel_name();
 
 constexpr int Q1_MAX_NQ = 16;
diff --git a/navtech-radar-slam_amd/csrc/sc_kernels.hip b/navtech-radar-slam_amd/csrc/sc_kernels.hip
--- a/navtech-radar-slam_amd/csrc/sc_kernels.hip
+++ b/navtech-radar-slam_amd/csrc/sc_kernels.hip
@@ -765,7 +765,7 @@
   int32_t k;
   int32_t round_begin, round_end;
   unsigned long long *stats;
-  const WindowPreview *win;
+  const WindowSurvivor *surv;
 };
 
 template <int B, int W, int SO>
@@ -898,8 +898,6 @@
 }
 
 
-constexpr int RW_CH = (WINDOW_P + 63) / 64;
-
 
 #ifndef RW_OCC
 #define RW_OCC 3
@@ -912,6 +910,43 @@
   const int qi = blockIdx.x;
   char *wsm = smem + WaveLds::OFF_ENT;
 
+  const int sl_cnt = a.sl_cnt[qi];
+  const float *thr = a.thr + (int64_t)qi * RESCORE_THR_STRIDE;
+  const int32_t *rcnt = reinterpret_cast<const int32_t *>(thr) + RESCORE_NUM_THR;
+  const float t_cap = thr[RESCORE_NUM_THR - 1];
+  const WindowSurvivor *sv = a.surv ? a.surv + (int64_t)qi * WINDOW_LIST_STRIDE : nullptr;
+  WindowListHeader hdr;
+  hdr.count = 0;
+  hdr.tau_ub = INFINITY;
+  hdr.n_cand = 0;
+  hdr.n_prev = 0;
+  WindowSurvivor first;
+  first.lo = INFINITY;
+  first.slot = 0;
+  first.ks = -1;
+  first.pos = 0;
+  if (sv) {
+    hdr = *reinterpret_cast<const WindowListHeader *>(sv);
+    first = sv[1 + lane];
+  }
+  {
+    const float4 *src = reinterpret_cast<const float4 *>(a.q.desc + (int64_t)qi * DS);
+    float4 *dst = reinterpret_cast<float4 *>(smem + WaveLds::OFF_QF32);
+    float4 x[5];
+#pragma unroll
+    for (int i = 0; i < 5; i++) x[i] = (lane + 64 * i < DS / 4) ? src[lane + 64 * i] : float4{0.f, 0.f, 0.f, 0.f};
+    const double kn = lane < NS ? a.q.norm[(int64_t)qi * NS + lane] : 0.0;
+    const double kv = lane < NS ? a.q.vkey[(int64_t)qi * NS + lane] : 0.0;
+#pragma unroll
+    for (int i = 0; i < 5; i++)
+      if (lane + 64 * i < DS / 4) dst[lane + 64 * i] = x[i];
+    if (lane < NS) {
+      reinterpret_cast<double *>(smem + WaveLds::OFF_QN1)[lane] = kn;
+      reinterpret_cast<double *>(smem + WaveLds::OFF_QV1)[lane] = kv;
+    }
+    wave_lds_fence();
+  }
+
   int64_t n_elig = a.n_eligible;
   if (a.q_elig) {
     const int64_t e = a.q_elig[qi];
@@ -941,9 +976,8 @@
     return t < tau_init ? t : tau_init;
   };
   double tau = kth_of(ld);
-  bool query_loaded = false;
   unsigned n_exact = 0, n_looked = 0, n_aligned = 0, n_shifts = 0, n_tail = 0;
-  unsigned nl_lane = 0, n_windowed = 0;
+  unsigned n_listed = 0, n_windowed = 0;
   bool walked_tail = false;
 
 #ifdef RSX_EXPERIMENTS
@@ -951,7 +985,7 @@
 #else
   constexpr bool timing = false;
 #endif
-  long long tacc[9] = {0, 0, 0, 0, 0, 0, 0, 0, 0};
+  long long tacc[6] = {0, 0, 0, 0, 0, 0};
   long long t_mark = timing ? clock64() : 0;
   const long long t_begin = t_mark;
   auto lap = [&](int slot_) {
@@ -973,25 +1007,6 @@
       const unsigned m7 = ((unsigned)ksm >> 8) & 0x7fu;
       if (m7) tmask = m7;
     }
-    if (!query_loaded) {
-      const float4 *src = reinterpret_cast<const float4 *>(a.q.desc + (int64_t)qi * DS);
-      float4 *dst = reinterpret_cast<float4 *>(smem + WaveLds::OFF_QF32);
-      float4 x[5];
-#pragma unroll
-      for (int i = 0; i < 5; i++) x[i] = (lane + 64 * i < DS / 4) ? src[lane + 64 * i] : float4{0.f, 0.f, 0.f, 0.f};
-      const double kn = lane < NS ? a.q.norm[(int64_t)qi * NS + lane] : 0.0;
-      const double kv = lane < NS ? a.q.vkey[(int64_t)qi * NS + lane] : 0.0;
-#pragma unroll
-      for (int i = 0; i < 5; i++)
-        if (lane + 64 * i < DS / 4) dst[lane + 64 * i] = x[i];
-      if (lane < NS) {
-        reinterpret_cast<double *>(smem + WaveLds::OFF_QN1)[lane] = kn;
-        reinterpret_cast<double *>(smem + WaveLds::OFF_QV1)[lane] = kv;
-      }
-      query_loaded = true;
-      wave_lds_fence();
-      lap(0);
-    }
     if (ks < 0) {
       ks = align_exact<SO>(reinterpret_cast<const double *>(smem + WaveLds::OFF_QV1), wsm, lane, er.v);
       n_aligned++;
@@ -1013,11 +1028,7 @@
     }
   };
 
-  const int sl_cnt = a.sl_cnt[qi];
   const RescoreEntry *sl = a.slist + (int64_t)qi * RESCORE_SHORTLIST_CAP;
-  const float *thr = a.thr + (int64_t)qi * RESCORE_THR_STRIDE;
-  const int32_t *rcnt = reinterpret_cast<const int32_t *>(thr) + RESCORE_NUM_THR;
-  const float t_cap = thr[RESCORE_NUM_THR - 1];
   const int r_end = a.round_end < RESCORE_NUM_THR ? a.round_end : RESCORE_NUM_THR;
   auto upto = [&](int r) {
     if (r <= 0) return 0;
@@ -1028,109 +1039,36 @@
   if (timing) {
     int keep = i0 + i1;
     asm volatile("" : "+s"(keep));
-    lap(7);
+    asm volatile("s_waitcnt vmcnt(0)" ::: "memory");
+    lap(0);
   }
   bool done = false;
 
   int pos_next = i0;
-  if (a.win && i0 < WINDOW_P && i0 < i1) {
-    const WindowPreview *wp = a.win + (int64_t)qi * WINDOW_P;
+  if (sv && i0 < WINDOW_P && i0 < i1) {
     const int pw = i1 < WINDOW_P ? i1 : WINDOW_P;
-    float lo[RW_CH], ub[RW_CH], flb[RW_CH];
-#pragma unroll
-    for (int j = 0; j < RW_CH; j++) {
-      const int pos = i0 + lane + 64 * j;
-      lo[j] = INFINITY;
-      ub[j] = INFINITY;
-      flb[j] = INFINITY;
-      if (pos < pw) {
-        const RescoreEntry e = sl[pos];
-        const WindowPreview w = wp[pos];
-        const int64_t gidx = a.db.idx_base + (int64_t)e.slot * a.db.idx_stride;
-        if (gidx < n_elig && !((double)e.lb - a.eps > tau)) {
-          flb[j] = e.lb;
-          if (!(w.pv == w.pv)) {
-            lo[j] = -INFINITY;
-          } else {
-            lo[j] = w.pv - WINDOW_MARGIN;
-            if (w.ks >= 0 && w.pv < 3.0e38f) ub[j] = w.pv + WINDOW_MARGIN;
-          }
-        }
-      }
-    }
-    if (timing) {
-      asm volatile("" : "+v"(lo[0]), "+v"(ub[0]));
-      lap(8);
-    }
-    double ud = ld;
-    int ui = li, us = ls;
-    for (int it = 0; it < a.k; it++) {
-      float m = ub[0];
-#pragma unroll
-      for (int j = 1; j < RW_CH; j++) m = fminf(m, ub[j]);
-      const float wm = wave_min_f32(m);
-      if (!((double)wm < __shfl(ud, a.k - 1))) break;
-      const unsigned long long bal = __ballot(m == wm);
-      const int src = __ffsll((long long)bal) - 1;
-      if (lane == src) {
-        bool gone = false;
-#pragma unroll
-        for (int j = 0; j < RW_CH; j++)
-          if (!gone && ub[j] == wm) {
-            ub[j] = INFINITY;
-            gone = true;
-          }
-      }
-      topk_insert(ud, ui, us, lane, a.k, (double)wm, 0x40000000 + it, 0);
-    }
-    const double tau_ub = kth_of(ud);
-    lap(1);
-#pragma unroll
-    for (int j = 0; j < RW_CH; j++)
-      if ((double)flb[j] - a.eps > tau_ub) lo[j] = INFINITY;
-#pragma unroll
-    for (int j = 0; j < RW_CH; j++) {
-      nl_lane += (lo[j] < INFINITY) ? 1u : 0u;
-      n_windowed += (lo[j] > -INFINITY && lo[j] < INFINITY) ? 1u : 0u;
-    }
-    struct Packed {
-      float lo;
-      int pos;
-    };
-    Packed *cbuf = reinterpret_cast<Packed *>(wsm);
-    for (;;) {
+    const int n_list = hdr.count < WINDOW_P ? hdr.count : WINDOW_P;
+    const double tau_ub = (double)hdr.tau_ub;
+    if (i0 == 0) {
+      n_listed = (unsigned)hdr.n_cand;
+      n_windowed = (unsigned)hdr.n_prev;
+    }
+    for (int base = 0; base < n_list; base += 64) {
+      WindowSurvivor e = first;
+      if (base > 0 && base + lane < n_list) e = sv[1 + base + lane];
       const double t_now = tau < tau_ub ? tau : tau_ub;
-      int nsurv = 0;
-#pragma unroll
-      for (int j = 0; j < RW_CH; j++) {
-        const bool sv = lo[j] < INFINITY && !((double)lo[j] > t_now);
-        const unsigned long long bal = __ballot(sv);
-        const int rank = nsurv + __popcll(bal & ((1ull << lane) - 1ull));
-        if (sv && rank < 64) {
-          cbuf[rank] = Packed{lo[j], i0 + lane + 64 * j};
-          lo[j] = INFINITY;
-        }
-        nsurv += __popcll(bal);
-      }
-      if (nsurv == 0) break;
-      nsurv = nsurv < 64 ? nsurv : 64;
-      wave_lds_fence();
-      float mylo = INFINITY;
-      int32_t myslot = 0;
-      int myks = -1;
-      if (lane < nsurv) {
-        const Packed c = cbuf[lane];
-        mylo = c.lo;
-        myslot = sl[c.pos].slot;
-        const int k_ = wp[c.pos].ks;
-        myks = k_ >= 0 ? k_ : -1;
-      }
-      wave_lds_fence();
+      const bool mine = base + lane < n_list && e.pos >= i0 && e.pos < pw && !((double)e.lo > t_now);
+      float mylo = mine ? e.lo : INFINITY;
+      const int32_t myslot = e.slot;
+      const int myks = e.ks;
+      unsigned long long todo = __ballot(mine);
+      if (!todo) continue;
       {
         Touch tch;
-        for (int i = 0; i < nsurv; i++) touch_entry(a.db, __shfl(myslot, i), lane, tch);
+        for (; todo; todo &= todo - 1) touch_entry(a.db, __shfl(myslot, __ffsll((long long)todo) - 1), lane, tch);
         touch_wait(tch);
       }
+      lap(1);
       auto pick = [&](int32_t &slot, int &ks) -> float {
         const float wm = wave_min_f32(mylo);
         if (wm == INFINITY) return wm;
@@ -1272,15 +1210,9 @@
     a.out[(int64_t)qi * a.k + lane] = h;
   }
   if (a.stats) {
-    unsigned lk = nl_lane, wd = n_windowed;
-#pragma unroll
-    for (int off = 32; off >= 1; off >>= 1) {
-      lk += __shfl_xor(lk, off);
-      wd += __shfl_xor(wd, off);
-    }
     if (lane == 0) {
-      atomicAdd(a.stats, (unsigned long long)(lk + n_looked));
-      atomicAdd(a.stats + 3, (unsigned long long)wd);
+      atomicAdd(a.stats, (unsigned long long)(n_listed + n_looked));
+      atomicAdd(a.stats + 3, (unsigned long long)n_windowed);
       atomicAdd(a.stats + 2, (unsigned long long)n_exact);
       atomicAdd(a.stats + 11, (unsigned long long)n_aligned);
       atomicAdd(a.stats + 12, (unsigned long long)n_shifts);
@@ -1288,8 +1220,6 @@
       if (walked_tail) atomicAdd(a.stats + 16, 1ull);
       if (timing) {
         for (int i = 0; i < 6; i++) atomicAdd(a.stats + 4 + i, (unsigned long long)tacc[i]);
-        atomicAdd(a.stats + 13, (unsigned long long)tacc[7]);
-        atomicAdd(a.stats + 14, (unsigned long long)tacc[8]);
         atomicAdd(a.stats + 10, (unsigned long long)(clock64() - t_begin));
       }
       if (n_exact) atomicAdd(a.stats + 1, 1ull);
@@ -1301,7 +1231,7 @@
                    int64_t n_eligible, const int64_t *q_elig, const RescoreEntry *slist, const int32_t *sl_cnt,
                    const float *thr, double eps, int32_t round_begin, int32_t round_end, const rsx_sc_hit *tau_src,
                    const rsx_sc_hit *seed, rsx_sc_hit *d_out, int32_t k, hipStream_t s, unsigned long long *d_stats,
-                   const WindowPreview *win) {
+                   const WindowSurvivor *surv) {
   if (q.nq <= 0) return RSX_OK;
   if (k < 1 || k > RSX_SC_MAX_TOPK) return fail(RSX_ERR_BAD_ARG, "k=%d out of range [1,%d]", k, RSX_SC_MAX_TOPK);
   RescoreArgs a;
@@ -1323,7 +1253,7 @@
   a.round_begin = round_begin;
   a.round_end = round_end;
   a.stats = d_stats;
-  a.win = win;
+  a.surv = surv;
   RSX_SO_DISPATCH(db.sum_order, hipLaunchKernelGGL(sc_rescore_wave_kernel<SO>, dim3(q.nq), dim3(64), WaveLds::SIZE, s, a));
   RSX_HIP(hipGetLastError());
   return RSX_OK;
diff --git a/navtech-radar-slam_amd/csrc/sc_window.hip b/navtech-radar-slam_amd/csrc/sc_window.hip
--- a/navtech-radar-slam_amd/csrc/sc_window.hip
+++ b/navtech-radar-slam_amd/csrc/sc_window.hip
@@ -57,6 +57,7 @@
   const RescoreEntry *slist;
   const int32_t *sl_cnt;
   WindowPreview *out;
+  WindowSurvivor *surv;
   double eps;
   int32_t k;
 };
@@ -66,10 +67,24 @@
   __shared__ float s_ub[WINDOW_HEAD];
   __shared__ int s_pos[WINDOW_P];
   __shared__ int s_n2;
-  const int lane = threadIdx.x & 63, wave = threadIdx.x >> 6;
+  __shared__ float s_tau;
+  __shared__ float s_lb[WINDOW_P], s_pv[WINDOW_P], s_cand[WINDOW_P];
+  __shared__ int s_slot[WINDOW_P], s_ks[WINDOW_P];
+  const int lane = threadIdx.x & 63, wave = __builtin_amdgcn_readfirstlane(threadIdx.x >> 6);
   const int qi = blockIdx.x;
   const int sl_cnt = a.sl_cnt[qi];
-  if (sl_cnt <= 0) return;
+  WindowSurvivor *list = a.surv + (int64_t)qi * WINDOW_LIST_STRIDE;
+  if (sl_cnt <= 0) {
+    if (threadIdx.x == 0) {
+      WindowListHeader h;
+      h.count = 0;
+      h.tau_ub = INFINITY;
+      h.n_cand = 0;
+      h.n_prev = 0;
+      *reinterpret_cast<WindowListHeader *>(list) = h;
+    }
+    return;
+  }
   {
     const uint4 *g0 = reinterpret_cast<const uint4 *>(a.qimg + (int64_t)qi * FILTER_QIMG_BYTES);
     const uint4 *g1 = reinterpret_cast<const uint4 *>(a.qkimg + (int64_t)qi * WINDOW_QK_BYTES);
@@ -85,8 +100,13 @@
   const char *ap = smem + ((n & 1) ? (FILTER_QIMG_ODD + 40 * n - 8) : (40 * n)) + 16 * hh;
   const char *kp = smem + FILTER_QIMG_BYTES + (n & 7) * QK_COPY + ((n & ~7) + 8 * hh) * 2;
 
-  auto do_group = [&](int pos, bool have, int pos_any) -> float {
-    const int64_t slot = sl[have ? pos : pos_any].slot;
+  auto lane_again = [&]() -> int {
+    int t = threadIdx.x;
+    asm volatile("" : "+v"(t));
+    return t & 31;
+  };
+  auto do_group = [&](auto pos_of, bool have, int pos_any) -> float {
+    const int64_t slot = sl[have ? pos_of() : pos_any].slot;
 
     floatx16 k0 = {0}, k1 = {0};
     {
@@ -146,24 +166,110 @@
 
     __builtin_amdgcn_sched_barrier(0);
     const u64 em = a.cmask[slot];
-    const float pv = win::preview_of(acc0, acc1, qm, em, win, kstar, hh);
+    u64 qmg = qm;
+    asm volatile("" : "+v"(qmg));
+    const float pv = win::preview_of(acc0, acc1, qmg, em, win, kstar, hh);
     if (have && hh == 0) {
+      const int pos = pos_of();
       WindowPreview o;
       o.pv = pv;
       o.ks = kstar;
       a.out[(int64_t)qi * WINDOW_P + pos] = o;
+      s_slot[pos] = (int)slot;
+      s_pv[pos] = pv;
+      s_ks[pos] = kstar;
     }
     return (have && kstar >= 0 && pv < 3.0e38f) ? pv + WINDOW_MARGIN : INFINITY;
+  };
+
+  auto write_list = [&](float tau_head, int n2) {
+    const int lim = sl_cnt < WINDOW_P ? sl_cnt : WINDOW_P;
+    const int nh = lim < WINDOW_HEAD ? lim : WINDOW_HEAD;
+    const unsigned long long below = (1ull << lane) - 1ull;
+    auto records = [&](auto f) {
+      for (int p0 = 0; p0 < nh; p0 += 64) f(p0 + lane, p0 + lane < nh);
+      for (int c0 = 0; c0 < n2; c0 += 64) f(c0 + lane < n2 ? s_pos[c0 + lane] : 0, c0 + lane < n2);
+    };
+    int nc = 0;
+    records([&](int pos, bool in) {
+      const float pv = s_pv[pos];
+      const float ub = pv + WINDOW_MARGIN;
+      const bool c = in && s_ks[pos] >= 0 && pv < 3.0e38f && ub <= tau_head;
+      const unsigned long long bal = __ballot(c);
+      if (c) s_cand[nc + __popcll(bal & below)] = ub;
+      nc += __popcll(bal);
+    });
+    dev::wave_lds_fence();
+    float tau_w = INFINITY;
+    if (nc >= a.k) {
+      for (int c0 = 0; c0 < nc; c0 += 64) {
+        const int i = c0 + lane;
+        const float v = i < nc ? s_cand[i] : INFINITY;
+        int r = 0;
+        for (int j = 0; j < nc; j++) {
+          const float x = s_cand[j];
+          r += (x < v || (x == v && j < i)) ? 1 : 0;
+        }
+        const unsigned long long b = __ballot(i < nc && r == a.k - 1);
+        if (b) {
+          tau_w = __shfl(v, __ffsll((long long)b) - 1);
+          break;
+        }
+      }
+    }
+    int ns = 0, n_cand = 0, n_prev = 0;
+    records([&](int pos, bool in) {
+      const float pv = s_pv[pos];
+      const int ks = s_ks[pos];
+      const bool none = in && !(pv == pv);
+      const bool lb_ok = !((double)s_lb[pos] - a.eps > (double)tau_w);
+      const bool cand = in && (none || (pv < INFINITY && lb_ok));
+      const float lo = none ? -INFINITY : pv - WINDOW_MARGIN;
+      const bool sv = cand && !(lo > tau_w);
+      const unsigned long long bal = __ballot(sv);
+      if (sv) {
+        WindowSurvivor e;
+        e.lo = lo;
+        e.slot = s_slot[pos];
+        e.ks = (none || ks < 0) ? -1 : ks;
+        e.pos = pos;
+        list[1 + ns + __popcll(bal & below)] = e;
+      }
+      ns += __popcll(bal);
+      n_cand += __popcll(__ballot(cand));
+      n_prev += __popcll(__ballot(cand && !none));
+    });
+    if (lane == 0) {
+      WindowListHeader h;
+      h.count = ns;
+      h.tau_ub = tau_w;
+      h.n_cand = n_cand;
+      h.n_prev = n_prev;
+      *reinterpret_cast<WindowListHeader *>(list) = h;
+    }
   };
 
   float tau_ub;
   {
     const int cnt1 = sl_cnt < WINDOW_HEAD ? sl_cnt : WINDOW_HEAD;
     float ub = INFINITY;
-    if (wave * 32 < cnt1) ub = do_group(wave * 32 + n, wave * 32 + n < cnt1, wave * 32);
+    if (wave * 32 < cnt1) ub = do_group([&] { return wave * 32 + lane_again(); }, wave * 32 + n < cnt1, wave * 32);
     if (hh == 0) s_ub[wave * 32 + n] = ub;
     __syncthreads();
-    if (sl_cnt <= WINDOW_HEAD) return;
+    float lbh0 = INFINITY, lbh1 = INFINITY;
+    if (wave == 0) {
+      if (lane < cnt1) lbh0 = sl[lane].lb;
+      if (lane + 64 < cnt1) lbh1 = sl[lane + 64].lb;
+    }
+    if (sl_cnt <= WINDOW_HEAD) {
+      if (wave == 0) {
+        s_lb[lane] = lbh0;
+        s_lb[lane + 64] = lbh1;
+        dev::wave_lds_fence();
+        write_list(INFINITY, 0);
+      }
+      return;
+    }
 
     {
       const float v0 = s_ub[lane], v1 = s_ub[lane + 64];
@@ -185,6 +291,10 @@
       const float c0 = __shfl(v0, b0 ? __ffsll((long long)b0) - 1 : 0), c1 = __shfl(v1, b1 ? __ffsll((long long)b1) - 1 : 0);
       tau_ub = b0 ? c0 : c1;
     }
+    if (wave == 0) {
+      s_lb[lane] = lbh0;
+      s_lb[lane + 64] = lbh1;
+    }
   }
   if (wave == 0) {
     int n2 = 0;
@@ -194,6 +304,7 @@
       bool pass = false;
       if (pos < lim) {
         const float lb = sl[pos].lb;
+        s_lb[pos] = lb;
         pass = !((double)lb - a.eps > (double)tau_ub);
         if (!pass) {
           WindowPreview o;
@@ -206,14 +317,19 @@
       if (pass) s_pos[n2 + __popcll(bal & ((1ull << lane) - 1ull))] = pos;
       n2 += __popcll(bal);
     }
-    if (lane == 0) s_n2 = n2;
+    if (lane == 0) {
+      s_n2 = n2;
+      s_tau = tau_ub;
+    }
   }
   __syncthreads();
   const int n2 = s_n2;
   for (int g = wave; g * 32 < n2; g += 4) {
     const bool have = g * 32 + n < n2;
-    (void)do_group(s_pos[have ? g * 32 + n : g * 32], have, s_pos[g * 32]);
-  }
+    (void)do_group([&] { return s_pos[g * 32 + lane_again()]; }, have, s_pos[g * 32]);
+  }
+  __syncthreads();
+  if (wave == 0) write_list(s_tau, n2);
 }
 
 }
@@ -229,7 +345,7 @@
 }
 
 int launch_window(const DbView &db, const QueryView &q, void *qimg, const RescoreEntry *slist, const int32_t *sl_cnt,
-                  int32_t k, double eps, WindowPreview *out, hipStream_t s) {
+                  int32_t k, double eps, WindowPreview *out, WindowSurvivor *surv, hipStream_t s) {
   if (q.nq <= 0) return RSX_OK;
   char *img = static_cast<char *>(qimg);
   char *kimg = img + (size_t)q.nq * FILTER_QIMG_BYTES;
@@ -246,6 +362,7 @@
   a.slist = slist;
   a.sl_cnt = sl_cnt;
   a.out = out;
+  a.surv = surv;
   a.eps = eps;
   a.k = k < 1 ? 1 : (k > WINDOW_HEAD ? WINDOW_HEAD : k);
   hipLaunchKernelGGL(sc_window_kernel, dim3((unsigned)q.nq), dim3(256), W_LDS, s, a);
```
